# chahuja/mix-stage

Hardware: AMD Instinct MI355X
Metric: train-step clips/sec (B=32, T=64, M=8) (higher is better)
Workload: dtype f32; 1 GPU; Mix-StAGE GAN train step (reference D/G coin flip, seed 4321: 457 G + 510 D steps), B=32 clips per GPU, T=64, 128-mel, 104-dim pose, M=S=8, audio branch pinned; fp32 arithmetic (the reference trains in fp64, trainer.py:138; held to it at 1e-4 pose L1); global_batch=32, parallelism=dp1, hip_graphs=True, bn_sync=local

## Files before the change

include/mixstage.h:

```cpp
#ifndef MIXSTAGE_H_
#define MIXSTAGE_H_

#include <stddef.h>
#include <stdint.h>

#ifdef __cplusplus
extern "C" {
#endif

#define MS_ABI_VERSION 4

enum ms_block_mode {
  MS_BARE = 0,
  MS_LRELU = 1,
  MS_BN_TRAIN = 2,
  MS_BN_EVAL = 3
};

enum ms_input_mode {
  MS_IN_PLAIN = 0,
  MS_IN_BCAST = 1,
  MS_IN_UP2ADD = 2
};

enum ms_dtype { MS_F32 = 0, MS_BF16 = 1, MS_F16 = 2 };
#define MS_DT_OUT_F32 0x100
#define MS_DT_BN_FOLDED 0x200
#define MS_DT_STAT_PAIR 0x400

typedef struct ms_conv_desc {
  int32_t B;
  int32_t Cin;
  int32_t H, W;
  int32_t Cout;
  int32_t groups;
  int32_t KH, KW, SH, SW, PH, PW;
  int32_t OH, OW;
  int32_t mode;
  int32_t in_mode;
  float slope;
  float eps;
  float momentum;
  int32_t dtype;
} ms_conv_desc;

const char* ms_last_error(void);
int ms_abi_version(void);
int ms_stat_pair_ok(const ms_conv_desc* d);

size_t ms_conv_block_fwd_workspace(const ms_conv_desc* d);
size_t ms_conv_block_bwd_workspace(const ms_conv_desc* d);

int ms_conv_block_fwd(const ms_conv_desc* d, const float* x, const float* x2, const float* w,
                      const float* bias, const float* gamma, const float* beta, float* running_mean,
                      float* running_var, float* y_raw, float* y, float* save, void* workspace,
                      size_t workspace_bytes, void* stream);

typedef struct ms_fwd_options {
  const void* w_planes;
  int32_t* bn_sync;
  int32_t bn_sync_words;
} ms_fwd_options;
int ms_conv_block_fwd_ex(const ms_conv_desc* d, const float* x, const float* x2, const float* w,
                         const float* bias, const float* gamma, const float* beta, float* running_mean,
                         float* running_var, float* y_raw, float* y, float* save, void* workspace,
                         size_t workspace_bytes, void* stream, const ms_fwd_options* opt);
int ms_clip_hold(void* stream);
int ms_clip_hold_flush(void* stream);
int ms_clip_hold_discard(void* stream);
int ms_clip_grid(const ms_conv_desc* d);
int ms_clip_pair_ok(const ms_conv_desc* host, const ms_conv_desc* guest);
size_t ms_fwd_weights_bytes(const ms_conv_desc* d);
int ms_fwd_weights_prepare(int n, const ms_conv_desc* descs, const float* const* w, void* const* planes, void* stream);

int ms_conv_block_bwd(const ms_conv_desc* d, const float* x, const float* x2, const float* w,
                      const float* gamma, const float* running_mean, const float* running_var,
                      const float* y_raw, const float* y, const float* save, const float* dy, float* dyr,
                      float* dx, float* dx2, float* dw, float* dbias, float* dgamma, float* dbeta,
                      void* workspace, size_t workspace_bytes, void* stream);

typedef struct ms_bwd_options {
  void* side_stream;
  void* side_workspace;
  size_t side_workspace_bytes;
  const float* wt_prepared;
  float* wgrad_partials;
  int defer_wgrad_launch;
  const float* prev_y;
  const float* prev_y_raw;
  const float* prev_save;
  const float* prev_gamma;
  float* prev_dgamma;
  float* prev_dbeta;
  float* prev_dbias;
  float prev_slope;
  int32_t* bn_sync;
  int32_t bn_sync_words;
  int dy_is_dyr;
  const float* dx_accum;
} ms_bwd_options;
int ms_dgrad_takes_accum(const ms_conv_desc* d);
int ms_dgrad_fuses_prev_bn(const ms_conv_desc* d);
int ms_conv_block_bwd_ex(const ms_conv_desc* d, const float* x, const float* x2, const float* w,
                         const float* gamma, const float* running_mean, const float* running_var,
                         const float* y_raw, const float* y, const float* save, const float* dy, float* dyr,
                         float* dx, float* dx2, float* dw, float* dbias, float* dgamma, float* dbeta,
                         void* workspace, size_t workspace_bytes, void* stream, const ms_bwd_options* opt);

typedef struct ms_prep16_item {
  const ms_conv_desc* desc;
  const float* w;
  const float* bias;
  const float* gamma;
  const float* beta;
  const float* running_mean;
  const float* running_var;
  void* fwd;
  void* dgrad;
} ms_prep16_item;
size_t ms_weights16_bytes(const ms_conv_desc* d, int which);
int ms_weights16_prepare(int n, const ms_prep16_item* items, void* stream);

int ms_set_bn_sync_buffer(int32_t* zeroed_words, int n);

int ms_cb8_from_plain(int dtype, const float* x, void* y, int B, int C, int HW, void* stream);
int ms_cb8_to_plain(int dtype, const void* x, float* y, int B, int C, int HW, void* stream);
int ms_cb8_from_btc(int dtype, const float* x, void* y, int B, int T, int C, int velocity, void* stream);
int ms_cb8_to_btc(int dtype, const void* x, float* y, int B, int T, int C, int velocity_bwd, void* stream);

size_t ms_dgrad_weights_elems(const ms_conv_desc* d, const float* w);
int ms_set_precision(int mode);
int ms_get_precision(void);
int ms_tuning_epoch(void);
int ms_dgrad_weights_prepare(int n, const ms_conv_desc* descs, const float* const* w, float* const* wt, void* stream);

size_t ms_wgrad_partials_elems(const ms_conv_desc* d, int* splits);
int ms_set_wgrad_batched(int on, int tiles_per_workgroup);
int ms_wgrad_flush(void* stream);
int ms_wgrad_discard(void);
int ms_wgrad_reduce_multi(int n, const float* const* partials, float* const* dw, const int* elems, const int* splits,
                          void* stream);

int ms_bn_stats(const float* y_raw, float* stats, int B, int C, int HW, void* stream);
int ms_bn_train_apply(const float* stats_all, int world, int n_local, const float* gamma, const float* beta, float* running_mean,
                      float* running_var, const float* y_raw, float* y, float* save, int B, int C, int HW, float eps,
                      float momentum, float slope, void* stream);
size_t ms_bn_bwd_workspace(int B, int C);
int ms_bn_bwd_sums(const float* dy, const float* y_raw, const float* save, float* sums, int B, int C, int HW, float slope,
                   void* workspace, size_t workspace_bytes, void* stream);
int ms_bn_bwd_apply(const float* dy, const float* y_raw, const float* save, const float* gamma, const float* sums_global,
                    double n_global, float* dyr, int B, int C, int HW, float slope, void* stream);

int ms_lerp_time_fwd(const float* x, float* y, int B, int C, int Tin, int F, int Tout, void* stream);
int ms_lerp_time_bwd(const float* dy, float* dx, int B, int C, int Tin, int F, int Tout, void* stream);

int ms_softmax_mix_fwd(const float* z, const float* score, float* soft, float* out, int B, int M, int P,
                       int T, void* stream);
int ms_softmax_mix_bwd(const float* z, const float* soft, const float* dout, float* dz, float* dscore,
                       int B, int M, int P, int T, void* stream);

#define MS_CHAIN_MAX_BLOCKS 4
typedef struct ms_chain_desc {
  int32_t B, M, T, cin0, C, P, n_blocks;
  int32_t mode;
  int32_t dtype;
  int32_t sync_first_word;
  int32_t keep_all_raw;
  float slope, eps, momentum;
} ms_chain_desc;
typedef struct ms_chain_tensors {
  const void* x;
  const float* score;
  const float* w[MS_CHAIN_MAX_BLOCKS];
  const float* bias[MS_CHAIN_MAX_BLOCKS];
  const float* gamma[MS_CHAIN_MAX_BLOCKS];
  const float* beta[MS_CHAIN_MAX_BLOCKS];
  float* running_mean[MS_CHAIN_MAX_BLOCKS];
  float* running_var[MS_CHAIN_MAX_BLOCKS];
  void* y_raw[MS_CHAIN_MAX_BLOCKS];
  void* y[MS_CHAIN_MAX_BLOCKS];
  float* save[MS_CHAIN_MAX_BLOCKS];
  const float* w_logits;
  const float* bias_logits;
  float* z;
  float* soft;
  float* out;
  const void* prepared;
  int32_t* sync;
  int32_t sync_words;
} ms_chain_tensors;
int ms_decoder_chain_supported(const ms_chain_desc* d);
size_t ms_decoder_chain_prepared_bytes(const ms_chain_desc* d);
size_t ms_decoder_chain_workspace(const ms_chain_desc* d);
int ms_decoder_chain_sync_words(const ms_chain_desc* d);
int ms_decoder_chain_prepare(const ms_chain_desc* d, const float* const* w, const float* w_logits, void* prepared, void* stream);
int ms_decoder_chain_fwd(const ms_chain_desc* d, const ms_chain_tensors* t, void* workspace, size_t workspace_bytes, void* stream);

int ms_decoder_chain_eval_supported(const ms_chain_desc* d);
size_t ms_decoder_chain_eval_workspace(const ms_chain_desc* d);
int ms_decoder_chain_eval_sync_words(const ms_chain_desc* d);
int ms_decoder_chain_eval_plan(const ms_chain_desc* d, int32_t* n_tiles, int32_t* groups_per_workgroup, int32_t* tile_first,
                               int32_t* own_lo, int32_t* own_hi, int32_t cap);
int ms_decoder_chain_eval_fwd(const ms_chain_desc* d, const ms_chain_tensors* t, void* workspace, size_t workspace_bytes, void* stream);

int ms_kmeans_labels(const float* pose, const int32_t* keep, const double* centers, int64_t* labels, int B, int T, int P,
                     int PK, int M, int feats, void* stream);
int ms_znorm_select(const float* x, const int32_t* keep, const double* mean, const double* inv_std, float* y, size_t rows,
                    int P, int PK, void* stream);

int ms_step_metrics(const float* ycap, const float* gt, const int32_t* keep, const int32_t* slot_of, const double* mean,
                    const double* stdv, const float* alphas, int n_alpha, double* out, int B, int T, int P, int PK,
                    void* stream);
int ms_eval_accumulate(const float* ycap, const float* gt, const int32_t* keep, const double* mean, const double* stdv,
                       double* fid_sums, double* fid_gram, unsigned long long* w1_hist, int B, int T, int P, int PK,
                       double bin_width, int nbins, void* stream);

int ms_concat_style_fwd(const float* x, const float* emb, const int64_t* ids, int ids_stride_b, int ids_stride_t, float* out,
                        int B, int C, int D, int T, void* stream);
int ms_concat_style_bwd(const float* dout, const int64_t* ids, int ids_stride_b, int ids_stride_t, float* dx, float* demb,
                        int B, int C, int D, int T, int S, void* stream);

int ms_concat_style_soft_fwd(const float* x, const float* emb, const float* w, int w_stride_b, int w_stride_t, float* out,
                             int B, int C, int D, int T, int S, void* stream);
int ms_concat_style_soft_bwd(const float* dout, const float* emb, const float* w, int w_stride_b, int w_stride_t, float* dx,
                             float* demb, float* dw, int B, int C, int D, int T, int S, void* stream);

int ms_cross_entropy_fwd(const float* score, const int64_t* target, float* loss, float* row_scratch,
                         int n_outer, int n_inner, int C, int stride_outer, int stride_c,
                         int stride_inner, void* stream);
int ms_cross_entropy_bwd(const float* score, const int64_t* target, const float* gscale, float* dscore,
                         int n_outer, int n_inner, int C, int stride_outer, int stride_c,
                         int stride_inner, int accumulate, void* stream);

typedef struct ms_loss_scale {
  float scale;
  const float* scale_dev;
} ms_loss_scale;
int ms_cross_entropy_fwd_ex(const float* score, const int64_t* target, float* loss, int n_outer, int n_inner, int C,
                            int stride_outer, int stride_c, int stride_inner, void* stream, const ms_loss_scale* ls);
int ms_cross_entropy_bwd_ex(const float* score, const int64_t* target, const float* gscale, float* dscore, int n_outer,
                            int n_inner, int C, int stride_outer, int stride_c, int stride_inner, int accumulate, void* stream,
                            const ms_loss_scale* ls);

int ms_velocity_fwd(const float* x, float* v, int B, int T, int P, void* stream);
int ms_velocity_bwd(const float* dv, float* dx, int B, int T, int P, void* stream);

int ms_transpose_btc(const float* x, float* y, int B, int T, int C, void* stream);
int ms_transpose_bct(const float* x, float* y, int B, int C, int T, void* stream);

int ms_l1_mean_fwd(const float* a, const float* b, float target, float* loss, float* partials, size_t n,
                   void* stream);
int ms_l1_mean_bwd(const float* a, const float* b, float target, const float* gscale, float* da, size_t n,
                   void* stream);
int ms_l2_mean_fwd(const float* a, const float* b, float target, float* loss, float* partials, size_t n, void* stream);
int ms_l2_mean_bwd(const float* a, const float* b, float target, const float* gscale, float* da, size_t n, void* stream);

int ms_lp_mean_fwd_ex(int squared, const float* a, const float* b, float target, float* loss, float* partials, size_t n,
                      void* stream, const ms_loss_scale* ls);
int ms_lp_mean_bwd_ex(int squared, const float* a, const float* b, float target, const float* gscale, float* da, size_t n,
                      void* stream, const ms_loss_scale* ls);

int ms_lp_mean_pair_fwd(int squared, const float* a, const float* targets, float* loss, size_t n, void* stream, const ms_loss_scale* ls);
int ms_lp_mean_pair_bwd(int squared, const float* a, const float* targets, const float* gscale0, const float* gscale1, float* da, size_t n,
                        void* stream, const ms_loss_scale* ls);

int ms_copy_multi(int n, const void* const* src, void* const* dst, const size_t* bytes, void* stream);

int ms_write_floats(float* dst, const float* host_values, int n, void* stream);

int ms_sqnorm(const float* g, size_t n, float* norm_out, float* partials, void* stream);
int ms_adam_step(float* p, const float* g, float* m, float* v, size_t n, const float* norm, float max_norm,
                 float lr, float beta1, float beta2, float eps, int32_t* step_state, void* stream);
int ms_adam_step_segmented(float* p, const float* g, float* m, float* v, size_t n, const float* norm, float max_norm,
                           float lr, float beta1, float beta2, float eps, int32_t* step_state,
                           const int32_t* seg_of_chunk, const int32_t* seg_first_step, float* seg_scratch, int n_seg,
                           void* stream);
int ms_adam_step_segmented_scaled(float* p, const float* g, float* m, float* v, size_t n, float* norm, float max_norm,
                                  float lr, float beta1, float beta2, float eps, int32_t* step_state,
                                  const int32_t* seg_of_chunk, const int32_t* seg_first_step, float* seg_scratch, int n_seg,
                                  int32_t* loss_scale_state, int32_t growth_interval, float min_scale, float max_scale,
                                  const int32_t* const* meeting_words, int n_meeting_words, void* stream);
int ms_adam_step_segmented_lr(float* p, const float* g, float* m, float* v, size_t n, const float* norm, float max_norm,
                              const float* lr_dev, float beta1, float beta2, float eps, int32_t* step_state,
                              const int32_t* seg_of_chunk, const int32_t* seg_first_step, float* seg_scratch, int n_seg,
                              void* stream);
int ms_adam_step_segmented_scaled_lr(float* p, const float* g, float* m, float* v, size_t n, float* norm, float max_norm,
                                     const float* lr_dev, float beta1, float beta2, float eps, int32_t* step_state,
                                     const int32_t* seg_of_chunk, const int32_t* seg_first_step, float* seg_scratch, int n_seg,
                                     int32_t* loss_scale_state, int32_t growth_interval, float min_scale, float max_scale,
                                     const int32_t* const* meeting_words, int n_meeting_words, void* stream);
size_t ms_reduce_partials_count(size_t n);

#ifdef __cplusplus
}
#endif
#endif
```

include/mixstage_aux.h:

```cpp
#ifndef MIXSTAGE_AUX_H_
#define MIXSTAGE_AUX_H_

#include "mixstage.h"

#ifdef __cplusplus
extern "C" {
#endif

int ms_set_counter_buffer(int32_t* zeroed_counters, int n);

int ms_conv_block_bwd_overlap(const ms_conv_desc* d, const float* x, const float* x2, const float* w,
                              const float* gamma, const float* running_mean, const float* running_var,
                              const float* y_raw, const float* y, const float* save, const float* dy, float* dyr,
                              float* dx, float* dx2, float* dw, float* dbias, float* dgamma, float* dbeta,
                              void* workspace, size_t workspace_bytes, void* stream, void* side_stream,
                              void* side_workspace, size_t side_workspace_bytes);

int ms_timing_enable(int on);
size_t ms_timing_report(char* buf, size_t cap);

int ms_debug_set_patch_min_workgroups(int n);
int ms_debug_set_patch_tuning(int intra_split, int force_splitk);

int ms_debug_set_conv16_tile(int wm, int wn);
int ms_debug_set_conv16_ring(int nstg, int wide8);
int ms_debug_set_wgrad16_target(int workgroups);
int ms_debug_set_wgrad16_ring(int buffers);
int ms_debug_set_wgrad_target(int workgroups);
int ms_debug_set_wgrad_wave(int on);
int ms_debug_set_conv_tile(int on);
int ms_debug_set_bn_fused(int on);
int ms_debug_set_bn_fused_min_workgroups(int n);
int ms_debug_set_skip(const char* patterns);

int ms_debug_set_clip32(int on);

int ms_debug_set_clip_corun(int on);

int ms_selftest_mfma(const float* A, const float* B, float* C, int K, void* stream);
int ms_probe_peak(int kind, long iters, void* a, void* b, double* work, void* stream);

#ifdef __cplusplus
}
#endif
#endif
```

mix_stage_amd/_lib.py:

```python
import ctypes
import os

_HERE = os.path.dirname(os.path.abspath(__file__))
LIB_PATH = os.path.join(_HERE, 'libmixstage_hip.so')
_ALT_LIB = os.environ.get('MS_LIB_PATH')
if _ALT_LIB:
  LIB_PATH = _ALT_LIB

c_void_p, c_int, c_float, c_size_t = ctypes.c_void_p, ctypes.c_int, ctypes.c_float, ctypes.c_size_t


class BwdOptions(ctypes.Structure):
  _fields_ = [('side_stream', ctypes.c_void_p), ('side_workspace', ctypes.c_void_p), ('side_workspace_bytes', ctypes.c_size_t),
              ('wt_prepared', ctypes.c_void_p), ('wgrad_partials', ctypes.c_void_p), ('defer_wgrad_launch', ctypes.c_int),
              ('prev_y', ctypes.c_void_p), ('prev_y_raw', ctypes.c_void_p), ('prev_save', ctypes.c_void_p), ('prev_gamma', ctypes.c_void_p),
              ('prev_dgamma', ctypes.c_void_p), ('prev_dbeta', ctypes.c_void_p), ('prev_dbias', ctypes.c_void_p), ('prev_slope', ctypes.c_float),
              ('bn_sync', ctypes.c_void_p), ('bn_sync_words', ctypes.c_int32), ('dy_is_dyr', ctypes.c_int),
              ('dx_accum', ctypes.c_void_p)]


class LossScale(ctypes.Structure):
  _fields_ = [('scale', ctypes.c_float), ('scale_dev', ctypes.c_void_p)]


class FwdOptions(ctypes.Structure):
  _fields_ = [('w_planes', ctypes.c_void_p), ('bn_sync', ctypes.c_void_p), ('bn_sync_words', ctypes.c_int32)]


class ConvDesc(ctypes.Structure):
  _fields_ = [(n, ctypes.c_int32) for n in
              ('B', 'Cin', 'H', 'W', 'Cout', 'groups', 'KH', 'KW', 'SH', 'SW', 'PH', 'PW', 'OH', 'OW',
               'mode', 'in_mode')] + \
             [('slope', c_float), ('eps', c_float), ('momentum', c_float), ('dtype', ctypes.c_int32)]


class ChainDesc(ctypes.Structure):
  _fields_ = [(n, ctypes.c_int32) for n in ('B', 'M', 'T', 'cin0', 'C', 'P', 'n_blocks', 'mode', 'dtype', 'sync_first_word', 'keep_all_raw')] + \
             [('slope', c_float), ('eps', c_float), ('momentum', c_float)]


class ChainTensors(ctypes.Structure):
  _fields_ = [('x', ctypes.c_void_p), ('score', ctypes.c_void_p)] + \
             [(n, ctypes.c_void_p * 4) for n in ('w', 'bias', 'gamma', 'beta', 'running_mean', 'running_var', 'y_raw', 'y', 'save')] + \
             [(n, ctypes.c_void_p) for n in ('w_logits', 'bias_logits', 'z', 'soft', 'out', 'prepared', 'sync')] + \
             [('sync_words', ctypes.c_int32)]


class Prep16Item(ctypes.Structure):
  _fields_ = [('desc', ctypes.POINTER(ConvDesc))] + [(n, ctypes.c_void_p) for n in
             ('w', 'bias', 'gamma', 'beta', 'running_mean', 'running_var', 'fwd', 'dgrad')]


MS_BARE, MS_LRELU, MS_BN_TRAIN, MS_BN_EVAL = 0, 1, 2, 3
MS_IN_PLAIN, MS_IN_BCAST, MS_IN_UP2ADD = 0, 1, 2
MS_F32, MS_BF16, MS_F16, MS_DT_OUT_F32, MS_DT_BN_FOLDED = 0, 1, 2, 0x100, 0x200
MS_DT_STAT_PAIR = 0x400

_P = c_void_p
_DESC = ctypes.POINTER(ConvDesc)

SIGNATURES = {
    'ms_last_error': (ctypes.c_char_p, []),
    'ms_abi_version': (c_int, []),
    'ms_set_counter_buffer': (c_int, [_P, c_int]),
    'ms_set_bn_sync_buffer': (c_int, [_P, c_int]),
    'ms_debug_set_bn_fused': (c_int, [c_int]),
    'ms_debug_set_bn_fused_min_workgroups': (c_int, [c_int]),
    'ms_conv_block_fwd_workspace': (c_size_t, [_DESC]),
    'ms_conv_block_bwd_workspace': (c_size_t, [_DESC]),
    'ms_conv_block_fwd': (c_int, [_DESC] + [_P] * 11 + [_P, c_size_t, _P]),
    'ms_conv_block_bwd': (c_int, [_DESC] + [_P] * 17 + [_P, c_size_t, _P]),
    'ms_conv_block_bwd_overlap': (c_int, [_DESC] + [_P] * 17 + [_P, c_size_t, _P, _P, _P, c_size_t]),
    'ms_conv_block_bwd_ex': (c_int, [_DESC] + [_P] * 17 + [_P, c_size_t, _P, _P]),
    'ms_dgrad_weights_elems': (c_size_t, [_DESC, _P]),
    'ms_dgrad_weights_prepare': (c_int, [c_int, _P, _P, _P, _P]),
    'ms_tuning_epoch': (c_int, []),
    'ms_conv_block_fwd_ex': (c_int, [_DESC] + [_P] * 11 + [_P, c_size_t, _P, _P]),
    'ms_fwd_weights_bytes': (c_size_t, [_DESC]),
    'ms_fwd_weights_prepare': (c_int, [c_int, _P, _P, _P, _P]),
    'ms_set_precision': (c_int, [c_int]),
    'ms_get_precision': (c_int, []),
    'ms_wgrad_partials_elems': (c_size_t, [_DESC, _P]),
    'ms_wgrad_reduce_multi': (c_int, [c_int, _P, _P, _P, _P, _P]),
    'ms_wgrad_flush': (c_int, [_P]),
    'ms_wgrad_discard': (c_int, []),
    'ms_weights16_bytes': (c_size_t, [_DESC, c_int]),
    'ms_weights16_prepare': (c_int, [c_int, _P, _P]),
    'ms_cb8_from_plain': (c_int, [c_int, _P, _P, c_int, c_int, c_int, _P]),
    'ms_cb8_to_plain': (c_int, [c_int, _P, _P, c_int, c_int, c_int, _P]),
    'ms_cb8_from_btc': (c_int, [c_int, _P, _P, c_int, c_int, c_int, c_int, _P]),
    'ms_cb8_to_btc': (c_int, [c_int, _P, _P, c_int, c_int, c_int, c_int, _P]),
    'ms_bn_stats': (c_int, [_P, _P, c_int, c_int, c_int, _P]),
    'ms_bn_train_apply': (c_int, [_P, c_int, c_int, _P, _P, _P, _P, _P, _P, _P, c_int, c_int, c_int, c_float, c_float, c_float, _P]),
    'ms_bn_bwd_workspace': (c_size_t, [c_int, c_int]),
    'ms_bn_bwd_sums': (c_int, [_P, _P, _P, _P, c_int, c_int, c_int, c_float, _P, c_size_t, _P]),
    'ms_bn_bwd_apply': (c_int, [_P, _P, _P, _P, _P, ctypes.c_double, _P, c_int, c_int, c_int, c_float, _P]),
    'ms_lerp_time_fwd': (c_int, [_P, _P, c_int, c_int, c_int, c_int, c_int, _P]),
    'ms_lerp_time_bwd': (c_int, [_P, _P, c_int, c_int, c_int, c_int, c_int, _P]),
    'ms_softmax_mix_fwd': (c_int, [_P, _P, _P, _P, c_int, c_int, c_int, c_int, _P]),
    'ms_softmax_mix_bwd': (c_int, [_P, _P, _P, _P, _P, c_int, c_int, c_int, c_int, _P]),
    'ms_kmeans_labels': (c_int, [_P, _P, _P, _P, c_int, c_int, c_int, c_int, c_int, c_int, _P]),
    'ms_znorm_select': (c_int, [_P, _P, _P, _P, _P, c_size_t, c_int, c_int, _P]),
    'ms_step_metrics': (c_int, [_P] * 7 + [c_int, _P, c_int, c_int, c_int, c_int, _P]),
    'ms_eval_accumulate': (c_int, [_P] * 8 + [c_int, c_int, c_int, c_int, ctypes.c_double, c_int, _P]),
    'ms_concat_style_fwd': (c_int, [_P, _P, _P, c_int, c_int, _P, c_int, c_int, c_int, c_int, _P]),
    'ms_concat_style_bwd': (c_int, [_P, _P, c_int, c_int, _P, _P, c_int, c_int, c_int, c_int, c_int, _P]),
    'ms_concat_style_soft_fwd': (c_int, [_P, _P, _P, c_int, c_int, _P, c_int, c_int, c_int, c_int, c_int, _P]),
    'ms_concat_style_soft_bwd': (c_int, [_P, _P, _P, c_int, c_int, _P, _P, _P, c_int, c_int, c_int, c_int, c_int, _P]),
    'ms_cross_entropy_fwd': (c_int, [_P, _P, _P, _P] + [c_int] * 6 + [_P]),
    'ms_cross_entropy_bwd': (c_int, [_P, _P, _P, _P] + [c_int] * 7 + [_P]),
    'ms_cross_entropy_fwd_ex': (c_int, [_P, _P, _P] + [c_int] * 6 + [_P, _P]),
    'ms_cross_entropy_bwd_ex': (c_int, [_P, _P, _P, _P] + [c_int] * 7 + [_P, _P]),
    'ms_lp_mean_fwd_ex': (c_int, [c_int, _P, _P, c_float, _P, _P, c_size_t, _P, _P]),
    'ms_lp_mean_bwd_ex': (c_int, [c_int, _P, _P, c_float, _P, _P, c_size_t, _P, _P]),
    'ms_lp_mean_pair_fwd': (c_int, [c_int, _P, _P, _P, c_size_t, _P, _P]),
    'ms_lp_mean_pair_bwd': (c_int, [c_int, _P, _P, _P, _P, _P, c_size_t, _P, _P]),
    'ms_velocity_fwd': (c_int, [_P, _P, c_int, c_int, c_int, _P]),
    'ms_velocity_bwd': (c_int, [_P, _P, c_int, c_int, c_int, _P]),
    'ms_transpose_btc': (c_int, [_P, _P, c_int, c_int, c_int, _P]),
    'ms_transpose_bct': (c_int, [_P, _P, c_int, c_int, c_int, _P]),
    'ms_l1_mean_fwd': (c_int, [_P, _P, c_float, _P, _P, c_size_t, _P]),
    'ms_l1_mean_bwd': (c_int, [_P, _P, c_float, _P, _P, c_size_t, _P]),
    'ms_l2_mean_fwd': (c_int, [_P, _P, c_float, _P, _P, c_size_t, _P]),
    'ms_l2_mean_bwd': (c_int, [_P, _P, c_float, _P, _P, c_size_t, _P]),
    'ms_copy_multi': (c_int, [c_int, _P, _P, _P, _P]),
    'ms_write_floats': (c_int, [_P, _P, c_int, _P]),
    'ms_decoder_chain_supported': (c_int, [_P]),
    'ms_decoder_chain_prepared_bytes': (c_size_t, [_P]),
    'ms_decoder_chain_workspace': (c_size_t, [_P]),
    'ms_decoder_chain_sync_words': (c_int, [_P]),
    'ms_decoder_chain_prepare': (c_int, [_P, _P, _P, _P, _P]),
    'ms_decoder_chain_fwd': (c_int, [_P, _P, _P, c_size_t, _P]),
    'ms_decoder_chain_eval_supported': (c_int, [_P]),
    'ms_decoder_chain_eval_workspace': (c_size_t, [_P]),
    'ms_decoder_chain_eval_sync_words': (c_int, [_P]),
    'ms_decoder_chain_eval_plan': (c_int, [_P, _P, _P, _P, _P, _P, c_int]),
    'ms_decoder_chain_eval_fwd': (c_int, [_P, _P, _P, c_size_t, _P]),
    'ms_sqnorm': (c_int, [_P, c_size_t, _P, _P, _P]),
    'ms_adam_step': (c_int, [_P, _P, _P, _P, c_size_t, _P, c_float, c_float, c_float, c_float, c_float, _P, _P]),
    'ms_adam_step_segmented': (c_int, [_P, _P, _P, _P, c_size_t, _P, c_float, c_float, c_float, c_float, c_float, _P, _P, _P, _P,
                                       c_int, _P]),
    'ms_adam_step_segmented_scaled': (c_int, [_P, _P, _P, _P, c_size_t, _P, c_float, c_float, c_float, c_float, c_float, _P, _P, _P, _P,
                                              c_int, _P, ctypes.c_int32, c_float, c_float, _P, c_int, _P]),
    'ms_adam_step_segmented_lr': (c_int, [_P, _P, _P, _P, c_size_t, _P, c_float, _P, c_float, c_float, c_float, _P, _P, _P, _P,
                                          c_int, _P]),
    'ms_adam_step_segmented_scaled_lr': (c_int, [_P, _P, _P, _P, c_size_t, _P, c_float, _P, c_float, c_float, c_float, _P, _P, _P, _P,
                                                 c_int, _P, ctypes.c_int32, c_float, c_float, _P, c_int, _P]),
    'ms_reduce_partials_count': (c_size_t, [c_size_t]),
    'ms_timing_enable': (c_int, [c_int]),
    'ms_timing_report': (c_size_t, [ctypes.c_char_p, c_size_t]),
    'ms_debug_set_patch_min_workgroups': (c_int, [c_int]),
    'ms_debug_set_patch_tuning': (c_int, [c_int, c_int]),
    'ms_debug_set_conv16_tile': (c_int, [c_int, c_int]),
    'ms_debug_set_conv16_ring': (c_int, [c_int, c_int]),
    'ms_debug_set_skip': (c_int, [ctypes.c_char_p]),
    'ms_debug_set_clip32': (c_int, [c_int]),
    'ms_debug_set_clip_corun': (c_int, [c_int]),
    'ms_clip_hold': (c_int, [_P]),
    'ms_clip_hold_flush': (c_int, [_P]),
    'ms_clip_hold_discard': (c_int, [_P]),
    'ms_clip_grid': (c_int, [_DESC]),
    'ms_clip_pair_ok': (c_int, [_DESC, _DESC]),
    'ms_debug_set_wgrad16_target': (c_int, [c_int]),
    'ms_debug_set_wgrad16_ring': (c_int, [c_int]),
    'ms_debug_set_wgrad_target': (c_int, [c_int]),
    'ms_debug_set_wgrad_wave': (c_int, [c_int]),
    'ms_debug_set_conv_tile': (c_int, [c_int]),
    'ms_set_wgrad_batched': (c_int, [c_int, c_int]),
    'ms_dgrad_fuses_prev_bn': (c_int, [_P]),
    'ms_dgrad_takes_accum': (c_int, [_P]),
    'ms_stat_pair_ok': (c_int, [_P]),
    'ms_selftest_mfma': (c_int, [_P, _P, _P, c_int, _P]),
    'ms_probe_peak': (c_int, [c_int, ctypes.c_long, _P, _P, ctypes.POINTER(ctypes.c_double), _P]),
}

_lib = None


class MixStageLibError(RuntimeError):
  pass


def lib():
  global _lib
  if _lib is None:
    if not os.path.isfile(LIB_PATH):
      raise MixStageLibError('%s not built: run `make -C mix_stage_amd/csrc` (or __graft_entry__.build()); '
                             'there is no CPU fallback' % LIB_PATH)
    handle = ctypes.CDLL(LIB_PATH)
    for name, (res, args) in SIGNATURES.items():
      if _ALT_LIB and name.startswith('ms_debug_') and not hasattr(handle, name):
        continue
      fn = getattr(handle, name)
      fn.restype, fn.argtypes = res, args
    mode = os.environ.get('MS_PRECISION', '')
    if mode:
      if mode not in ('fp32', 'bf16x6'):
        raise MixStageLibError('MS_PRECISION=%s: expected fp32 or bf16x6' % mode)
      handle.ms_set_precision(1 if mode == 'bf16x6' else 0)
    if os.environ.get('MS_BN_FUSED'):
      handle.ms_debug_set_bn_fused(int(os.environ['MS_BN_FUSED']))
    if os.environ.get('MS_BN_FUSED_MIN_WGS'):
      handle.ms_debug_set_bn_fused_min_workgroups(int(os.environ['MS_BN_FUSED_MIN_WGS']))
    if os.environ.get('MS_CLIP32'):
      handle.ms_debug_set_clip32(int(os.environ['MS_CLIP32']))
    if os.environ.get('MS_CONV_TILE'):
      handle.ms_debug_set_conv_tile(int(os.environ['MS_CONV_TILE']))
    if os.environ.get('MS_WGRAD_WAVE'):
      handle.ms_debug_set_wgrad_wave(int(os.environ['MS_WGRAD_WAVE']))
    if os.environ.get('MS_PATCH_MIN_WGS'):
      handle.ms_debug_set_patch_min_workgroups(int(os.environ['MS_PATCH_MIN_WGS']))
    _lib = handle
  return _lib


def check(rc, what):
  if rc != 0:
    raise MixStageLibError('%s failed: %s' % (what, lib().ms_last_error().decode()))
```

mix_stage_amd/csrc/api.hip:

```cpp
#include "block_geom.h"

namespace ms {
extern int g_clip32;

static int validate(const ms_conv_desc* d, const char* who) {
  if (!d) return set_error("%s: null descriptor", who);
  if (d->B < 1 || d->Cin < 1 || d->Cout < 1 || d->groups < 1 || d->H < 1 || d->W < 1 || d->KH < 1 || d->KW < 1 ||
      d->SH < 1 || d->SW < 1 || d->PH < 0 || d->PW < 0)
    return set_error("%s: bad geometry", who);
  const int oh = (d->H + 2 * d->PH - d->KH) / d->SH + 1, ow = (d->W + 2 * d->PW - d->KW) / d->SW + 1;
  if (d->H + 2 * d->PH < d->KH || d->W + 2 * d->PW < d->KW || oh != d->OH || ow != d->OW)
    return set_error("%s: output size (%d,%d) does not match geometry (expected %d,%d)", who, d->OH, d->OW, oh, ow);
  if (d->mode < MS_BARE || d->mode > MS_BN_EVAL) return set_error("%s: bad mode %d", who, d->mode);
  if (d->in_mode < MS_IN_PLAIN || d->in_mode > MS_IN_UP2ADD) return set_error("%s: bad in_mode %d", who, d->in_mode);
  if (d->in_mode == MS_IN_UP2ADD && (d->H != 1 || d->KH != 1 || (d->W & 1)))
    return set_error("%s: UP2ADD needs a 1-D block with even W", who);
  if (dt_of(d) > DT_F16 || (d->dtype & ~(0xff | MS_DT_OUT_F32 | MS_DT_BN_FOLDED | MS_DT_STAT_PAIR))) return set_error("%s: bad dtype 0x%x", who, d->dtype);
  if (dt_of(d) == DT_F32 && (d->dtype & ~(0xff | MS_DT_STAT_PAIR))) return set_error("%s: MS_DT_OUT_F32 is a flag of the 16-bit modes", who);
  if ((d->dtype & MS_DT_STAT_PAIR) && (d->B & 1)) return set_error("%s: MS_DT_STAT_PAIR needs an even batch", who);
  const double out_elems = (double)d->B * d->groups * d->Cout * d->OH * d->OW;
  const double in_elems = (double)d->B * d->groups * d->Cin * d->H * d->W;
  const double lim = dt_of(d) == DT_F32 ? 536870912.0 : 1073741824.0;
  if (out_elems >= lim || in_elems >= lim) return set_error("%s: tensor of 2 GiB or more (%.0f elements)", who, std::max(out_elems, in_elems));
  return 0;
}

static inline bool conv_c1_of(const ms_conv_desc* d) {
  return conv_c1_ok(d->groups, d->Cin, d->Cout, d->KH, d->KW, d->SH, d->SW, d->PH, d->PW, d->H, d->in_mode == MS_IN_PLAIN);
}
static inline bool wgrad_c1_of(const ms_conv_desc* d) {
  return dt_of(d) == DT_F32 && g_precision == 0 &&
         wgrad_c1_ok(d->groups, d->Cin, d->Cout, d->KH, d->KW, d->SH, d->SW, d->PH, d->PW, d->H, d->W, d->in_mode == MS_IN_PLAIN);
}

struct FwdPlan {
  BlockGeo g;
  bool clip, c1;
  int c1_tiles;
  PatchPlan pp;
  GatherPlan pl;
  bool pair_epilogue;
  size_t w_bytes;
  struct { size_t stats, part, counts, clip_w, planes, total; } ws;
};
static FwdPlan fwd_plan(const ms_conv_desc* d) {
  FwdPlan p;
  const BlockGeo g = p.g = geo_of(d);
  const bool train = d->mode == MS_BN_TRAIN;
  p.clip = g_precision == 0 && clip32_fwd_ok(d);
  p.c1 = conv_c1_of(d);
  p.c1_tiles = p.c1 ? conv_c1_tiles(d->B, d->H, d->W) : 0;
  p.pp = plan_patch(g.nd, d->Cout, d->groups, d->Cin, d->KH, d->KW, d->SH, d->SW, d->B, d->OH, d->OW, 1, d->W);
  p.pl = plan_gather(d->Cout, g.npix, d->groups, d->Cin * g.khw);
  const PatchPlan& pp = p.pp;
  const bool patch_slab = pp.ok && (pp.splitk > 1 || pp.ksi > 1);
  p.pair_epilogue = !train || ((long)d->B / 2 * g.hw <= 4096 && !p.c1 && (pp.ok ? patch_slab : p.pl.splitk > 1));
  const size_t planes_bytes = (pp.ok && pp.p6) ? (size_t)3 * g.C * patch6_row_elems(d->Cin, d->KH, d->KW) * 2 : 0;
  p.w_bytes = p.clip ? clip32_fwd_weight_bytes(d) : planes_bytes;

  const size_t slab = (size_t)g.npix * g.C * sizeof(float);
  auto tile_stats = [&](int n_tiles) { return align_up((size_t)n_tiles * g.C * 2 * sizeof(float), 256); };
  p.ws.stats = p.ws.part = 0;
  p.ws.counts = p.c1 ? tile_stats(p.c1_tiles) : pp.ok ? tile_stats(pp.n_tiles) : 0;
  size_t front = 256;
  if (train) front = std::max(front, (size_t)p.pl.n_tiles * g.C * 2 * sizeof(float));
  if (pp.ok && train) front = std::max(front, tile_stats(pp.n_tiles) + (size_t)pp.n_tiles * sizeof(float));
  if (patch_slab) front = std::max(front, pp.splitk * slab);
  if (p.pl.splitk > 1) front = std::max(front, p.pl.splitk * slab);
  if (p.c1) front = std::max(front, tile_stats(p.c1_tiles) + (size_t)p.c1_tiles * sizeof(float));
  p.ws.total = align_up(front, 256) + 256;
  p.ws.planes = carve(p.ws.total, align_up(planes_bytes, 256));
  p.ws.clip_w = p.clip ? clip32_part_bytes(d->Cout, d->B * d->OW / 32) : 0;
  if (p.clip) p.ws.total = std::max(p.ws.total, p.ws.clip_w + align_up(p.w_bytes, 256) + 256);
  return p;
}

struct BwdPlan {
  BlockGeo g;
  DgradGeo dg;
  int nchunk;
  bool dg_clip, dg_grouped;
  PatchPlan dpp;
  GatherPlan dpl;
  size_t wt_elems;
  size_t dg_planes_bytes;
  bool wg_c1;
  WgradPatchPlan wp;
  int wg_splits;
  int wg_splits_reserved;
  struct { size_t fuse_part, bn_part, colpart, wt, wg_part, dg_part, dg_planes, total; } ws;
};
static BwdPlan bwd_plan(const ms_conv_desc* d) {
  BwdPlan p;
  const BlockGeo g = p.g = geo_of(d);
  const DgradGeo dg = p.dg = dgrad_geo_of(d);
  int bpc;
  p.nchunk = bwd_chunks(d->B, g.C, &bpc);
  p.dg_clip = g_precision == 0 && clip32_dgrad_ok(d);
  p.dg_grouped = g_precision == 0 && g_clip32 && gdgrad32_ok(d);
  p.dpp = plan_patch(g.nd, d->Cin, dg.tg, dg.tcog, dg.jh, dg.jw, 1, 1, d->B, cdiv(d->H, d->SH), cdiv(d->W, d->SW), dg.ncls, d->OW);
  p.dpl = plan_gather(d->Cin, d->B * cdiv(d->H, d->SH) * cdiv(d->W, d->SW), dg.tg * dg.ncls, dg.tcog * dg.jh * dg.jw);
  p.wt_elems = dgrad_weight_elems(d->groups, d->Cout, d->Cin, d->KH, d->KW, d->SH, d->SW);
  p.dg_planes_bytes = (p.dpp.ok && p.dpp.p6) ? (size_t)3 * dg.ncls * dg.tg * d->Cin * patch6_row_elems(dg.tcog, dg.jh, dg.jw) * 2 : 0;
  p.wg_c1 = wgrad_c1_of(d);
  p.wp = WgradPatchPlan{};
  if (p.wg_c1) {
    p.wg_splits = p.wg_splits_reserved = wgrad_c1_splits(d->B, d->H);
  } else {
    p.wp = plan_wgrad_patch(g.nd, d->Cout, d->Cin * g.khw, d->groups, d->KH, d->KW, d->SH, d->SW, d->B, d->OH, d->OW, d->W, g.up2 != 0);
    const int gather_splits = wgrad_splits(d->Cout, d->Cin * g.khw, d->groups, g.npix);
    p.wg_splits = p.wp.ok ? p.wp.splits : gather_splits;
    p.wg_splits_reserved = std::max(p.wp.ok ? p.wp.splits : 1, gather_splits);
  }

  const size_t dx_bytes = (size_t)d->B * g.cin_tot * d->H * d->W * sizeof(float);
  p.ws.total = 0;
  p.ws.fuse_part = carve(p.ws.total, clip32_dgrad_bn_part_bytes(d));
  p.ws.bn_part = carve(p.ws.total, align_up((size_t)g.C * p.nchunk * 2 * sizeof(float), 256));
  p.ws.colpart = carve(p.ws.total, align_up((size_t)g.C * p.nchunk * sizeof(float), 256));
  p.ws.wt = carve(p.ws.total, align_up(std::max(p.wt_elems, std::max(clip32_dgrad_weight_floats(d), gdgrad32_weight_floats(d))) * sizeof(float), 256));
  p.ws.wg_part = carve(p.ws.total, align_up(wsize_of(d) * sizeof(float) * (p.wg_splits_reserved > 1 ? p.wg_splits_reserved : 0), 256));
  p.ws.dg_part = carve(p.ws.total, (p.dpp.ok && p.dpp.splitk > 1) ? align_up(p.dpp.splitk * dx_bytes, 256) : 0);
  p.ws.dg_planes = carve(p.ws.total, align_up(p.dg_planes_bytes, 256));
  if (p.dpl.splitk > 1) p.ws.total += align_up(p.dpl.splitk * dx_bytes, 256);
  p.ws.total += 256;
  return p;
}

enum { DW_NONE = 0, DW_TRANSPOSED = 1, DW_CLIP = 2, DW_GROUPED = 3 };
static int dgrad_weights_of(const ms_conv_desc* d, const BwdPlan& p, const float* w) {
  if (p.dg_clip) return DW_CLIP;
  if (p.dg_grouped) return DW_GROUPED;
  const bool direct = p.dpp.ok && !p.dpp.p6 && patch_dgrad_direct_ok(w, d->Cin, d->KH, d->KW, d->SH, d->SW, p.g.bcast != 0);
  return direct ? DW_NONE : DW_TRANSPOSED;
}
static size_t dgrad_weights_elems(const ms_conv_desc* d, const BwdPlan& p, int kind) {
  return kind == DW_CLIP ? clip32_dgrad_weight_floats(d) : kind == DW_GROUPED ? gdgrad32_weight_floats(d) : p.wt_elems;
}

}

using namespace ms;

extern "C" {

size_t ms_conv_block_fwd_workspace(const ms_conv_desc* d) {
  if (!d) return 256;
  return dt_of(d) != DT_F32 ? block_fwd16_workspace(d) : fwd_plan(d).ws.total;
}

size_t ms_conv_block_bwd_workspace(const ms_conv_desc* d) {
  if (!d) return 256;
  return dt_of(d) != DT_F32 ? block_bwd16_workspace(d) : bwd_plan(d).ws.total;
}

int ms_conv_block_fwd(const ms_conv_desc* d, const float* x, const float* x2, const float* w, const float* bias,
                      const float* gamma, const float* beta, float* running_mean, float* running_var, float* y_raw, float* y,
                      float* save, void* workspace, size_t workspace_bytes, void* stream) {
  return ms_conv_block_fwd_ex(d, x, x2, w, bias, gamma, beta, running_mean, running_var, y_raw, y, save, workspace,
                              workspace_bytes, stream, nullptr);
}

static int conv_block_fwd_impl(const ms_conv_desc* d, const float* x, const float* x2, const float* w, const float* bias,
                               const float* gamma, const float* beta, float* running_mean, float* running_var, float* y_raw,
                               float* y, float* save, void* workspace, size_t workspace_bytes, void* stream,
                               const ms_fwd_options* opt);

int ms_conv_block_fwd_ex(const ms_conv_desc* d, const float* x, const float* x2, const float* w, const float* bias,
                         const float* gamma, const float* beta, float* running_mean, float* running_var, float* y_raw,
                         float* y, float* save, void* workspace, size_t workspace_bytes, void* stream,
                         const ms_fwd_options* opt) {
  const bool clip_path = d && dt_of(d) == DT_F32 && g_precision == 0 && !validate(d, "ms_conv_block_fwd") && clip32_fwd_ok(d);
  int rc = clip32_fwd_call_begin((hipStream_t)stream, clip_path, workspace, workspace_bytes);
  if (!rc) rc = conv_block_fwd_impl(d, x, x2, w, bias, gamma, beta, running_mean, running_var, y_raw, y, save, workspace, workspace_bytes, stream, opt);
  clip32_fwd_call_end((hipStream_t)stream);
  return rc;
}

static int conv_block_fwd_impl(const ms_conv_desc* d, const float* x, const float* x2, const float* w, const float* bias,
                               const float* gamma, const float* beta, float* running_mean, float* running_var, float* y_raw,
                               float* y, float* save, void* workspace, size_t workspace_bytes, void* stream,
                               const ms_fwd_options* opt) {
  const unsigned short* w_planes = opt ? (const unsigned short*)opt->w_planes : nullptr;
  int rc = validate(d, "ms_conv_block_fwd");
  if (rc) return rc;
  if (!x || !w || !y) return set_error("ms_conv_block_fwd: null tensor");
  const bool bn = d->mode == MS_BN_TRAIN || d->mode == MS_BN_EVAL;
  if (bn && (!gamma || !beta || !running_mean || !running_var)) return set_error("ms_conv_block_fwd: BN tensors missing");
  if (d->mode == MS_BN_TRAIN && (!y_raw || !save || !workspace)) return set_error("ms_conv_block_fwd: y_raw/save/workspace missing");
  if (d->in_mode == MS_IN_UP2ADD && !x2) return set_error("ms_conv_block_fwd: UP2ADD needs x2");
  if (dt_of(d) != DT_F32)
    return block_fwd16(d, x, x2, w, bias, gamma, beta, running_mean, running_var, y_raw, y, save, workspace, workspace_bytes,
                       (hipStream_t)stream, w_planes, opt ? opt->bn_sync : nullptr, opt ? opt->bn_sync_words : 0);
  const FwdPlan p = fwd_plan(d);
  if (workspace_bytes < p.ws.total) return set_error("ms_conv_block_fwd: workspace too small");
  hipStream_t s = (hipStream_t)stream;
  const BlockGeo& g = p.g;
  const int C = g.C, npix = g.npix, hw = g.hw, Kg = d->Cin * g.khw;
  float* stats = ws_at<float>(workspace, p.ws.stats);
  float* counts = ws_at<float>(workspace, p.ws.counts);
  float* part = ws_at<float>(workspace, p.ws.part);

  if (p.clip) {
    const float* wp = (const float*)w_planes;
    if (!wp) {
      float* mine = ws_at<float>(workspace, p.ws.clip_w);
      rc = clip32_prep_queue(w, mine, d->Cout, d->Cin, d->KW, 0, d->Cin, s);
      if (!rc) rc = clip32_prep_flush(s);
      if (rc) return rc;
      wp = mine;
    }
    rc = clip32_block_fwd(d, x, x2, wp, bias, gamma, beta, running_mean, running_var, y_raw, y, save, stats, opt ? opt->bn_sync : nullptr,
                          opt ? opt->bn_sync_words : 0, s);
    if (rc != -2) return rc;
    rc = clip32_hold_flush(s);
    if (rc) return rc;
  }

  float* out = d->mode == MS_BN_TRAIN ? y_raw : y;
  const int a_vec = (Kg % 4 == 0) && (((uintptr_t)w & 15) == 0);
  const int ep = d->mode == MS_BARE ? EP_BARE : d->mode == MS_LRELU ? EP_LRELU : d->mode == MS_BN_EVAL ? EP_BN_EVAL : EP_RAW_STATS;
  const int sg = d->mode == MS_BN_TRAIN ? sg_of(d) : 1;
  if (sg > 1 && !p.pair_epilogue)
    return set_error("ms_conv_block_fwd: MS_DT_STAT_PAIR is not implemented for this block's kernels (ms_stat_pair_ok)");
  if (p.c1) {
    rc = launch_conv_c1(x, w, bias, out, gamma, beta, running_mean, running_var, stats, counts, d->B, d->H, d->W, ep, d->slope,
                        d->eps, s);
    if (rc) return rc;
    if (d->mode == MS_BN_TRAIN) {
      rc = launch_bn_finalize_apply(stats, counts, p.c1_tiles, 0, npix, C, gamma, beta, running_mean, running_var, save, d->eps,
                                    d->momentum, y_raw, y, d->B, hw, d->slope, s);
    }
    return rc;
  }
  if (p.pp.ok) {
    const PatchPlan& pp = p.pp;
    PatchArgs q = {};
    q.A = w; q.src = x; q.src2 = x2; q.out = out;
    q.bias = bias; q.bn_g = gamma; q.bn_b = beta; q.bn_m = running_mean; q.bn_v = running_var;
    q.stats = stats; q.counts = counts;
    q.Mg = d->Cout; q.Kg = Kg; q.groups = d->groups; q.Kc = d->Cin; q.bcast = g.bcast; q.a_vec = a_vec; q.ep = ep;
    fill_src(q, plane_strides(g.one_d, d->B, g.cin_tot, d->H, d->W));
    fill_out(q, plane_strides(g.one_d, d->B, C, d->OH, d->OW));
    q.PH = g.one_d ? 0 : d->PH;
    q.PW = d->PW; q.tiles_x = pp.tiles_x; q.tiles_y = pp.tiles_y; q.slope = d->slope; q.eps = d->eps;
    q.o_sh = 1; q.o_sw = 1; q.o_ry = 0; q.o_rx = 0;
    q.splitk = pp.splitk; q.chunks_per_split = pp.chunks_per_split;
    q.src_elems = (size_t)d->B * g.cin_tot * d->H * d->W; q.a_elems = (size_t)C * Kg;
    const bool raw_out = pp.splitk > 1 || (pp.ksi > 1 && d->mode == MS_BN_TRAIN);
    if (raw_out) { q.part = part; q.part_stride = (size_t)npix * C; }
    const double flops = 2.0 * d->Cout * Kg * (double)npix * d->groups;
    const double bytes = 4.0 * ((double)C * Kg + (double)d->B * g.cin_tot * d->H * d->W + (double)npix * C);
    if (pp.p6) {
      const int re = patch6_row_elems(d->Cin, d->KH, d->KW);
      const unsigned short* planes = w_planes;
      if (!planes) {
        unsigned short* mine = ws_at<unsigned short>(workspace, p.ws.planes);
        rc = launch_split_weights(w, mine, C, d->Cin, d->KH, d->KW, s);
        if (rc) return rc;
        planes = mine;
      }
      q.Aplanes = planes; q.plane_stride = (unsigned)((size_t)C * re); q.a_row_elems = re;
      rc = launch_patch6(q, pp, d->KH, d->KW, d->SW, g.up2 != 0, flops, bytes, s);
    } else {
      rc = launch_patch(q, pp, d->KH, d->KW, d->SW, g.up2 != 0, flops, bytes, s);
    }
    if (rc) return rc;
    if (raw_out)
      return launch_splitk_fwd_epilogue(q.part, pp.splitk, q.part_stride, bias, gamma, beta, running_mean, running_var, y_raw,
                                        y, save, d->B, C, hw, ep, d->slope, d->eps, d->momentum, s, sg);
    if (d->mode == MS_BN_TRAIN) {
      rc = launch_bn_finalize_apply(stats, counts, pp.n_tiles, 0, npix, C, gamma, beta, running_mean, running_var, save, d->eps,
                                    d->momentum, y_raw, y, d->B, hw, d->slope, s);
    }
    return rc;
  }
  const GatherPlan& pl = p.pl;
  GatherArgs a = {};
  a.A = w; a.src = x; a.src2 = x2; a.out = out;
  a.bias = bias; a.bn_g = gamma; a.bn_b = beta; a.bn_m = running_mean; a.bn_v = running_var;
  a.stats = stats;
  a.Mg = d->Cout; a.Kg = Kg; a.groups = d->groups; a.Kc = d->Cin;
  a.bcast = g.bcast; a.src_ctotal = g.cin_tot;
  a.SRCH = d->H; a.SRCW = d->W; a.OUTH = d->OH; a.OUTW = d->OW; a.Npix = npix;
  a.KH = d->KH; a.KW = d->KW; a.SH = d->SH; a.SW = d->SW; a.PH = d->PH; a.PW = d->PW;
  a.a_vec = a_vec; a.ep = ep;
  a.slope = d->slope; a.eps = d->eps;
  if (pl.splitk > 1) {
    a.part = part;
    a.part_stride = (size_t)npix * C;
  }
  rc = launch_gather(a, false, g.up2 != 0, pl, s);
  if (rc) return rc;
  if (pl.splitk > 1) {
    return launch_splitk_fwd_epilogue(a.part, pl.splitk, a.part_stride, bias, gamma, beta, running_mean, running_var, y_raw, y,
                                      save, d->B, C, hw, ep, d->slope, d->eps, d->momentum, s, sg);
  }
  if (d->mode == MS_BN_TRAIN) {
    rc = launch_bn_finalize_apply(stats, nullptr, pl.n_tiles, 64 * pl.tn, npix, C, gamma, beta, running_mean, running_var, save,
                                  d->eps, d->momentum, y_raw, y, d->B, hw, d->slope, s);
  }
  return rc;
}

size_t ms_wgrad_partials_elems(const ms_conv_desc* d, int* splits) {
  if (validate(d, "ms_wgrad_partials_elems")) return 0;
  const int sp = dt_of(d) != DT_F32 ? wgrad16_splits(d) : bwd_plan(d).wg_splits;
  if (splits) *splits = sp;
  return sp > 1 ? (size_t)sp * wsize_of(d) : 0;
}

int ms_wgrad_reduce_multi(int n, const float* const* partials, float* const* dw, const int* elems, const int* splits,
                          void* stream) {
  if (n < 0 || (n && (!partials || !dw || !elems || !splits))) return set_error("ms_wgrad_reduce_multi: null argument");
  for (int i = 0; i < n; ++i)
    if (!partials[i] || !dw[i] || elems[i] <= 0 || splits[i] < 1) return set_error("ms_wgrad_reduce_multi: bad job %d", i);
  ReduceBatch rb;
  rb.n = 0;
  for (int i = 0; i < n; ++i) {
    ReduceJob jb = {partials[i], dw[i], elems[i], splits[i], 0, 0};
    rb.job[rb.n++] = jb;
    if (rb.n == REDUCE_BATCH_MAX) {
      const int rc = launch_reduce_splits_multi(rb, (hipStream_t)stream);
      if (rc) return rc;
      rb.n = 0;
    }
  }
  return rb.n ? launch_reduce_splits_multi(rb, (hipStream_t)stream) : 0;
}

size_t ms_dgrad_weights_elems(const ms_conv_desc* d, const float* w) {
  if (validate(d, "ms_dgrad_weights_elems")) return 0;
  if (dt_of(d) != DT_F32) return 0;
  const BwdPlan p = bwd_plan(d);
  const int kind = dgrad_weights_of(d, p, w);
  if (kind == DW_NONE) return 0;
  return align_up(dgrad_weights_elems(d, p, kind), 64) + (p.dg_planes_bytes + 3) / 4;
}

size_t ms_fwd_weights_bytes(const ms_conv_desc* d) {
  if (validate(d, "ms_fwd_weights_bytes")) return 0;
  if (dt_of(d) != DT_F32) return 0;
  return fwd_plan(d).w_bytes;
}

int ms_fwd_weights_prepare(int n, const ms_conv_desc* descs, const float* const* w, void* const* planes, void* stream) {
  if (n < 0 || (n && (!descs || !w || !planes))) return set_error("ms_fwd_weights_prepare: null argument");
  PrepQueueGuard queue_guard;
  SplitBatch sb;
  sb.n = 0;
  for (int i = 0; i < n; ++i) {
    const ms_conv_desc* d = descs + i;
    int rc = validate(d, "ms_fwd_weights_prepare");
    if (rc) return rc;
    if (dt_of(d) != DT_F32) continue;
    const FwdPlan p = fwd_plan(d);
    if (!p.w_bytes) continue;
    if (!planes[i]) return set_error("ms_fwd_weights_prepare: block %d needs a buffer of ms_fwd_weights_bytes bytes", i);
    if (p.clip) {
      rc = clip32_prep_queue(w[i], (float*)planes[i], d->Cout, d->Cin, d->KW, 0, d->Cin, (hipStream_t)stream);
      if (rc) return rc;
      continue;
    }
    SplitJob jb = {w[i], (unsigned short*)planes[i], p.g.C, d->Cin, p.g.khw, 0, 0, 0};
    sb.job[sb.n++] = jb;
    if (sb.n == SPLIT_BATCH_MAX) {
      rc = launch_split_weights_multi(sb, (hipStream_t)stream);
      if (rc) return rc;
      sb.n = 0;
    }
  }
  { const int rcq = clip32_prep_flush((hipStream_t)stream); if (rcq) return rcq; }
  return sb.n ? launch_split_weights_multi(sb, (hipStream_t)stream) : 0;
}

int ms_dgrad_weights_prepare(int n, const ms_conv_desc* descs, const float* const* w, float* const* wt, void* stream) {
  if (n < 0 || (n && (!descs || !w || !wt))) return set_error("ms_dgrad_weights_prepare: null argument");
  PrepQueueGuard queue_guard;
  TransposeBatch tb;
  tb.n = 0;
  for (int i = 0; i < n; ++i) {
    const ms_conv_desc* d = descs + i;
    int rc = validate(d, "ms_dgrad_weights_prepare");
    if (rc) return rc;
    const BwdPlan p = bwd_plan(d);
    const int kind = dgrad_weights_of(d, p, w[i]);
    if (kind == DW_NONE) continue;
    if (!wt[i]) return set_error("ms_dgrad_weights_prepare: block %d needs a buffer of ms_dgrad_weights_elems floats", i);
    if (kind == DW_CLIP) {
      rc = clip32_prep_queue(w[i], wt[i], d->Cin, d->Cout, d->KW, d->KW == 4 ? 2 : 1, d->Cin, (hipStream_t)stream);
      if (rc) return rc;
      continue;
    }
    if (kind == DW_GROUPED) {
      rc = gdgrad32_prepare(d, w[i], wt[i], (hipStream_t)stream);
      if (rc) return rc;
      continue;
    }
    TransposeJob jb = {w[i], wt[i], p.dg.tg, p.dg.tcog, d->Cin, d->KH, d->KW, d->SH, d->SW, d->PH, d->PW, p.dpp.ok ? 1 : 0, 0};
    tb.job[tb.n++] = jb;
    if (tb.n == TRANSPOSE_BATCH_MAX) {
      rc = launch_transpose_weight_multi(tb, (hipStream_t)stream);
      if (rc) return rc;
      tb.n = 0;
    }
  }
  if (tb.n) {
    const int rc = launch_transpose_weight_multi(tb, (hipStream_t)stream);
    if (rc) return rc;
  }
  { int rcq = clip32_prep_flush((hipStream_t)stream); if (!rcq) rcq = gdgrad32_prep_flush((hipStream_t)stream); if (rcq) return rcq; }
  SplitBatch sb;
  sb.n = 0;
  for (int i = 0; i < n; ++i) {
    const ms_conv_desc* d = descs + i;
    const BwdPlan p = bwd_plan(d);
    if (!p.dg_planes_bytes || dgrad_weights_of(d, p, w[i]) != DW_TRANSPOSED) continue;
    SplitJob jb = {wt[i], (unsigned short*)(wt[i] + align_up(p.wt_elems, 64)), p.dg.ncls * p.dg.tg * d->Cin, p.dg.tcog, p.dg.jh * p.dg.jw, 0, 0, 0};
    sb.job[sb.n++] = jb;
    if (sb.n == SPLIT_BATCH_MAX) {
      const int rc = launch_split_weights_multi(sb, (hipStream_t)stream);
      if (rc) return rc;
      sb.n = 0;
    }
  }
  return sb.n ? launch_split_weights_multi(sb, (hipStream_t)stream) : 0;
}

int ms_stat_pair_ok(const ms_conv_desc* d) {
  if (!d || (d->B & 1) || validate(d, "ms_stat_pair_ok")) return 0;
  if (d->mode != MS_BN_TRAIN) return 1;
  if (dt_of(d) != DT_F32) return stat_pair16_ok(d) ? 1 : 0;
  if (g_precision != 0) return 0;
  if ((long)d->B / 2 * d->OH * d->OW > BN_BWD32_FUSED_MAX) return 0;
  const FwdPlan p = fwd_plan(d);
  if (p.clip) {
    const int npx = d->SW == 2 ? 32 : 64, npw = d->B * d->OW / npx, cus = current_device_cus();
    if (npw % 2 == 0 && cus > 0 && cdiv(d->Cout, 32) * npw <= cus) return 1;
  }
  return p.pair_epilogue ? 1 : 0;
}

int ms_dgrad_fuses_prev_bn(const ms_conv_desc* d) {
  if (!d || validate(d, "ms_dgrad_fuses_prev_bn") || (d->dtype & MS_DT_STAT_PAIR)) return 0;
  return (dt_of(d) == DT_F32 && g_precision == 0 && clip32_dgrad_bn_ok(d)) ? 1 : 0;
}

int ms_dgrad_takes_accum(const ms_conv_desc* d) {
  if (!d || validate(d, "ms_dgrad_takes_accum")) return 0;
  if (dt_of(d) != DT_F32) return dgrad16_takes_accum(d) ? 1 : 0;
  return (g_precision == 0 && d->in_mode == MS_IN_PLAIN && clip32_dgrad_ok(d)) ? 1 : 0;
}

int ms_conv_block_bwd(const ms_conv_desc* d, const float* x, const float* x2, const float* w, const float* gamma,
                      const float* running_mean, const float* running_var, const float* y_raw, const float* y,
                      const float* save, const float* dy, float* dyr, float* dx, float* dx2, float* dw, float* dbias,
                      float* dgamma, float* dbeta, void* workspace, size_t workspace_bytes, void* stream) {
  ms_bwd_options o = {};
  return ms_conv_block_bwd_ex(d, x, x2, w, gamma, running_mean, running_var, y_raw, y, save, dy, dyr, dx, dx2, dw, dbias,
                              dgamma, dbeta, workspace, workspace_bytes, stream, &o);
}

static hipEvent_t fork_event() {
  static thread_local hipEvent_t ev = nullptr;
  if (!ev && hipEventCreateWithFlags(&ev, hipEventDisableTiming) != hipSuccess) ev = nullptr;
  return ev;
}

int ms_conv_block_bwd_overlap(const ms_conv_desc* d, const float* x, const float* x2, const float* w, const float* gamma,
                              const float* running_mean, const float* running_var, const float* y_raw, const float* y,
                              const float* save, const float* dy, float* dyr, float* dx, float* dx2, float* dw,
                              float* dbias, float* dgamma, float* dbeta, void* workspace, size_t workspace_bytes,
                              void* stream, void* side_stream, void* side_workspace, size_t side_workspace_bytes) {
  ms_bwd_options o = {};
  o.side_stream = side_stream; o.side_workspace = side_workspace; o.side_workspace_bytes = side_workspace_bytes;
  return ms_conv_block_bwd_ex(d, x, x2, w, gamma, running_mean, running_var, y_raw, y, save, dy, dyr, dx, dx2, dw, dbias,
                              dgamma, dbeta, workspace, workspace_bytes, stream, &o);
}

int ms_conv_block_bwd_ex(const ms_conv_desc* d, const float* x, const float* x2, const float* w, const float* gamma,
                         const float* running_mean, const float* running_var, const float* y_raw, const float* y,
                         const float* save, const float* dy, float* dyr, float* dx, float* dx2, float* dw, float* dbias,
                         float* dgamma, float* dbeta, void* workspace, size_t workspace_bytes, void* stream,
                         const ms_bwd_options* opt) {
  (void)running_mean; (void)running_var;
  ms_bwd_options none = {};
  if (!opt) opt = &none;
  void* side_stream = opt->side_stream;
  const float* wt_prepared = opt->wt_prepared;
  const bool defer_wgrad = opt->wgrad_partials != nullptr;
  int rc = validate(d, "ms_conv_block_bwd");
  if (rc) return rc;
  if (d->mode == MS_BN_EVAL) return set_error("ms_conv_block_bwd: BN_EVAL blocks are never differentiated on the path");
  if (!dy || !w || !workspace) return set_error("ms_conv_block_bwd: null tensor");
  if (d->mode == MS_BN_TRAIN && !opt->dy_is_dyr && (!y_raw || !save || !gamma || !dyr)) return set_error("ms_conv_block_bwd: BN_TRAIN needs y_raw/save/gamma/dyr");
  if ((opt->dy_is_dyr || opt->prev_y) && (dt_of(d) != DT_F32 || side_stream)) return set_error("ms_conv_block_bwd: the fused producer-BatchNorm backward is an fp32, single-stream form");
  if (d->mode == MS_LRELU && (!y || !dyr)) return set_error("ms_conv_block_bwd: LRELU needs y/dyr");
  if (dw && !x) return set_error("ms_conv_block_bwd: dw needs x");
  if (opt->dx_accum && !(dx && ms_dgrad_takes_accum(d))) return set_error("ms_conv_block_bwd: dx_accum on a block ms_dgrad_takes_accum() declines");
  if (d->in_mode == MS_IN_UP2ADD && ((dw && !x2) || (dx && !dx2))) return set_error("ms_conv_block_bwd: UP2ADD needs x2/dx2");
  if (dt_of(d) != DT_F32) {
    if (side_stream) return set_error("ms_conv_block_bwd: no side-stream form in the 16-bit modes");
    if (d->mode == MS_BARE && out_f32_of(d) && !dyr) return set_error("ms_conv_block_bwd: fp32 dy needs the dyr scratch");
    return block_bwd16(d, x, x2, w, gamma, y_raw, y, save, dy, dyr, dx, dx2, dw, dbias, dgamma, dbeta, workspace, workspace_bytes,
                       (hipStream_t)stream, wt_prepared, opt->wgrad_partials, opt->defer_wgrad_launch, opt->dx_accum);
  }
  const BwdPlan p = bwd_plan(d);
  if (workspace_bytes < p.ws.total) return set_error("ms_conv_block_bwd: workspace too small");
  hipStream_t s = (hipStream_t)stream;
  const BlockGeo& g = p.g;
  const DgradGeo& dg = p.dg;
  const int C = g.C, npix = g.npix, hw = g.hw, Kg = d->Cin * g.khw;
  const bool up2 = g.up2 != 0, bcast = g.bcast != 0;

  float* fuse_part = ws_at<float>(workspace, p.ws.fuse_part);
  float* bn_part = ws_at<float>(workspace, p.ws.bn_part);
  float* colpart = ws_at<float>(workspace, p.ws.colpart);
  float* wt = ws_at<float>(workspace, p.ws.wt);
  float* wg_part = ws_at<float>(workspace, p.ws.wg_part);
  float* dg_part = ws_at<float>(workspace, p.ws.dg_part);
  if (defer_wgrad) wg_part = opt->wgrad_partials;
  hipStream_t ws_stream = s;
  if (side_stream && side_stream != stream && dw) {
    if (defer_wgrad) return set_error("ms_conv_block_bwd_ex: wgrad_partials and side_stream are exclusive");
    if (!opt->side_workspace || opt->side_workspace_bytes < p.ws.total)
      return set_error("ms_conv_block_bwd_overlap: side workspace too small");
    ws_stream = (hipStream_t)side_stream;
    wg_part = ws_at<float>(opt->side_workspace, p.ws.wg_part);
  }

  const float* gr = dy;
  int bias_done = 0;
  const bool have_prev = opt->prev_y != nullptr;
  if (have_prev && !(dx && g_precision == 0 && clip32_dgrad_bn_ok(d)))
    return set_error("ms_conv_block_bwd: this block's data gradient cannot carry the producer's BatchNorm backward (ms_dgrad_fuses_prev_bn)");
  if (opt->dy_is_dyr) {
    if (d->mode != MS_BN_TRAIN) return set_error("ms_conv_block_bwd: dy_is_dyr is the BN_TRAIN form");
    bias_done = 1;
  } else if (d->mode == MS_BN_TRAIN) {
    rc = launch_bn_bwd(dy, y_raw, y, save, gamma, bn_part, dyr, colpart, dbias, dgamma, dbeta, d->B, C, hw, d->slope, &bias_done, s, sg_of(d));
    gr = dyr;
  } else if (d->mode == MS_LRELU) {
    rc = launch_act_bwd(dy, y, dyr, colpart, dbias, d->B, C, hw, 1, d->slope, &bias_done, s);
    gr = dyr;
  } else if (dbias) {
    rc = launch_act_bwd(dy, nullptr, nullptr, colpart, dbias, d->B, C, hw, 0, 0.f, &bias_done, s);
  }
  if (rc) return rc;
  if (dbias && !bias_done && !opt->dy_is_dyr) {
    rc = launch_colsum_finalize(colpart, dbias, d->B, C, s);
    if (rc) return rc;
  }

  if (ws_stream != s) {
    hipEvent_t ev = fork_event();
    if (!ev || hipEventRecord(ev, s) != hipSuccess || hipStreamWaitEvent(ws_stream, ev, 0) != hipSuccess)
      return set_error("ms_conv_block_bwd_overlap: stream fork failed");
  }

  bool dx_done = false;
  if (dx && p.dg_clip) {
    const float* wp = wt_prepared;
    if (!wp) {
      rc = clip32_prep_queue(w, wt, d->Cin, d->Cout, d->KW, d->KW == 4 ? 2 : 1, d->Cin, s);
      if (!rc) rc = clip32_prep_flush(s);
      if (rc) return rc;
      wp = wt;
    }
    if (have_prev) {
      const Clip32PrevBN pv = {opt->prev_y, opt->prev_y_raw, opt->prev_save, opt->prev_gamma, opt->prev_dgamma, opt->prev_dbeta, opt->prev_dbias, opt->prev_slope};
      rc = clip32_block_dgrad(d, gr, wp, dx, dx2, s, &pv, fuse_part, opt->bn_sync, opt->bn_sync_words, opt->dx_accum);
      if (rc == -2) return set_error("ms_conv_block_bwd: the fused data gradient is not resident at once on this device");
    } else {
      rc = clip32_block_dgrad(d, gr, wp, dx, dx2, s, nullptr, nullptr, nullptr, 0, opt->dx_accum);
    }
    if (rc && rc != -2) return rc;
    if (rc == -2 && opt->dx_accum) return set_error("ms_conv_block_bwd: the clip-resident data gradient declined a launch with dx_accum");
    dx_done = rc == 0;
    rc = 0;
  }
  if (dx && !dx_done && p.dg_grouped) {
    const float* wp = wt_prepared;
    if (!wp) {
      rc = gdgrad32_prepare(d, w, wt, s);
      if (!rc) rc = gdgrad32_prep_flush(s);
      if (rc) return rc;
      wp = wt;
    }
    rc = gdgrad32_launch(d, gr, wp, dx, s);
    if (rc) return rc;
    dx_done = true;
  }
  if (dx && !dx_done) {
    const PatchPlan& pp0 = p.dpp;
    const int Kg2 = dg.tcog * dg.jh * dg.jw;
    const size_t dx_elems = (size_t)d->B * g.cin_tot * d->H * d->W;
    const bool direct = pp0.ok && !pp0.p6 && patch_dgrad_direct_ok(w, d->Cin, d->KH, d->KW, d->SH, d->SW, bcast);
    if (wt_prepared) {
      wt = const_cast<float*>(wt_prepared);
    } else if (!direct) {
      rc = launch_transpose_weight(w, wt, dg.tg, dg.tcog, d->Cin, d->KH, d->KW, d->SH, d->SW, d->PH, d->PW, pp0.ok ? 1 : 0, s);
      if (rc) return rc;
    }
    if (pp0.ok) {
      PatchArgs q = {};
      q.A = wt; q.src = gr; q.out = dx; q.out2 = dx2;
      q.Mg = d->Cin; q.Kg = Kg2; q.groups = dg.tg; q.Kc = dg.tcog; q.bcast = 0; q.a_vec = (Kg2 % 4 == 0);
      if (direct) { q.A = w; q.a_vec = 2; }
      q.ep = up2 ? EP_DGRAD_UP2 : EP_BARE; q.is_dgrad = 1;
      q.cls_a_stride = (unsigned)((size_t)dg.tg * d->Cin * Kg2);
      fill_src(q, plane_strides(g.one_d, d->B, C, d->OH, d->OW));
      fill_out(q, plane_strides(g.one_d, d->B, g.cin_tot, d->H, d->W));
      const double flops = fill_parity_classes(q, d, dg, g.one_d);
      const double bytes = 4.0 * ((double)dg.ncls * dg.tg * d->Cin * Kg2 + (double)d->B * C * hw) + 4.0 * (double)dx_elems;
      q.tiles_x = pp0.tiles_x; q.tiles_y = pp0.tiles_y;
      q.splitk = pp0.splitk; q.chunks_per_split = pp0.chunks_per_split;
      q.src_elems = (size_t)d->B * C * hw; q.a_elems = (size_t)dg.ncls * dg.tg * d->Cin * Kg2;
      if (pp0.splitk > 1) {
        q.part = dg_part; q.part_stride = dx_elems;
        q.ep = EP_BARE;
      }
      if (pp0.p6) {
        const int re = patch6_row_elems(dg.tcog, dg.jh, dg.jw), rows = dg.ncls * dg.tg * d->Cin;
        const unsigned short* planes;
        if (wt_prepared) {
          planes = (const unsigned short*)(wt_prepared + align_up(p.wt_elems, 64));
        } else {
          unsigned short* mine = ws_at<unsigned short>(workspace, p.ws.dg_planes);
          rc = launch_split_weights(wt, mine, rows, dg.tcog, dg.jh, dg.jw, s);
          if (rc) return rc;
          planes = mine;
        }
        q.Aplanes = planes; q.plane_stride = (unsigned)((size_t)rows * re); q.a_row_elems = re;
        q.cls_a_stride = (unsigned)(dg.tg * d->Cin);
        rc = launch_patch6(q, pp0, dg.jh, dg.jw, 1, false, flops, bytes, s);
      } else {
        rc = launch_patch(q, pp0, dg.jh, dg.jw, 1, false, flops, bytes, s);
      }
      if (rc) return rc;
      if (pp0.splitk > 1) {
        rc = launch_splitk_dgrad_epilogue(dg_part, pp0.splitk, dx_elems, dx, dx2, dx_elems, d->W, up2 ? 1 : 0, s);
        if (rc) return rc;
      }
    } else {
      const GatherPlan& pl = p.dpl;
      GatherArgs a = {};
      a.A = wt; a.src = gr; a.out = dx; a.out2 = dx2;
      a.Mg = d->Cin; a.Kg = Kg2; a.groups = dg.tg; a.Kc = dg.tcog; a.src_ctotal = C;
      a.SRCH = d->OH; a.SRCW = d->OW; a.OUTH = d->H; a.OUTW = d->W; a.Npix = d->B * d->H * d->W; a.batch = d->B;
      a.KH = dg.jh; a.KW = dg.jw; a.SH = d->SH; a.SW = d->SW; a.PH = d->PH; a.PW = d->PW;
      a.bcast = 0;
      a.a_vec = (a.Kg % 4 == 0);
      a.ep = up2 ? EP_DGRAD_UP2 : EP_DGRAD;
      if (pl.splitk > 1) {
        a.part = dg_part;
        a.part_stride = dx_elems;
        a.ep = EP_DGRAD;
      }
      rc = launch_gather(a, true, up2, pl, s);
      if (rc) return rc;
      if (pl.splitk > 1) {
        rc = launch_splitk_dgrad_epilogue(dg_part, pl.splitk, dx_elems, dx, dx2, dx_elems, d->W, up2 ? 1 : 0, s);
        if (rc) return rc;
      }
    }
  }

  if (dw && p.wg_c1) {
    rc = launch_wgrad_c1(gr, x, wg_part, d->B, d->H, d->W, ws_stream);
    if (!rc && !defer_wgrad) rc = launch_reduce_splits(wg_part, dw, C * Kg, p.wg_splits, ws_stream);
    return rc;
  }
  if (dw && p.wp.ok) {
    const WgradPatchPlan& wp = p.wp;
    WgradPatchArgs q = {};
    q.dyr = gr; q.src = x; q.src2 = x2;
    q.out = wp.splits > 1 ? wg_part : dw;
    q.Cog = d->Cout; q.Cig = d->Cin; q.Kg = Kg; q.groups = d->groups; q.bcast = bcast;
    fill_src(q, plane_strides(g.one_d, d->B, g.cin_tot, d->H, d->W));
    fill_out(q, plane_strides(g.one_d, d->B, C, d->OH, d->OW));
    q.PH = g.one_d ? 0 : d->PH;
    q.PW = d->PW; q.tiles_x = wp.tiles_x; q.tiles_y = wp.tiles_y; q.n_tiles = wp.n_tiles;
    q.tiles_per_split = wp.tiles_per_split; q.splits = wp.splits;
    const double flops = 2.0 * d->Cout * q.Kg * (double)npix * d->groups;
    const double bytes = 4.0 * ((double)npix * C + (double)d->B * g.cin_tot * d->H * d->W + (double)C * q.Kg);
    if (wp.splits > 1 && !defer_wgrad && !wp.p6) {
      q.counters = counter_region(CNT_WGRAD, cdiv(q.Kg, 64) * cdiv(d->Cout, 64) * d->groups);
      q.final_out = dw;
    }
    if (opt->defer_wgrad_launch && !wp.p6 && ws_stream == s && (wp.splits == 1 || defer_wgrad))
      return queue_wgrad_patch(q, wp, d->KH, d->KW, d->SW, up2, flops, bytes);
    rc = wp.p6 ? launch_wgrad_patch6(q, wp, d->KH, d->KW, d->SW, up2, flops, bytes, ws_stream)
               : launch_wgrad_patch(q, wp, d->KH, d->KW, d->SW, up2, flops, bytes, ws_stream);
    if (rc) return rc;
    if (wp.splits > 1 && !q.counters && !defer_wgrad) rc = launch_reduce_splits(wg_part, dw, C * q.Kg, wp.splits, ws_stream);
  } else if (dw) {
    WgradArgs a = {};
    a.dyr = gr; a.src = x; a.src2 = x2;
    a.Cog = d->Cout; a.Cig = d->Cin; a.Kg = Kg; a.groups = d->groups;
    a.src_ctotal = g.cin_tot;
    a.H = d->H; a.W = d->W; a.OH = d->OH; a.OW = d->OW; a.Npix = npix;
    a.KH = d->KH; a.KW = d->KW; a.SH = d->SH; a.SW = d->SW; a.PH = d->PH; a.PW = d->PW;
    a.bcast = bcast;
    rc = launch_wgrad(a, up2, dw, wg_part, defer_wgrad, ws_stream, opt->defer_wgrad_launch && ws_stream == s);
  }
  return rc;
}

int ms_clip_hold(void* stream) { return clip32_hold_arm((hipStream_t)stream); }
int ms_clip_hold_flush(void* stream) { return clip32_hold_flush((hipStream_t)stream); }
int ms_clip_hold_discard(void* stream) { clip32_hold_discard((hipStream_t)stream); return 0; }
int ms_clip_grid(const ms_conv_desc* d) {
  if (validate(d, "ms_clip_grid") || dt_of(d) != DT_F32 || g_precision != 0) return 0;
  return clip32_fwd_grid(d);
}
int ms_clip_pair_ok(const ms_conv_desc* host, const ms_conv_desc* guest) {
  if (validate(host, "ms_clip_pair_ok") || validate(guest, "ms_clip_pair_ok") || dt_of(host) != DT_F32 || dt_of(guest) != DT_F32 || g_precision != 0) return 0;
  return clip32_fwd_pair_ok(host, guest) ? 1 : 0;
}
int ms_debug_set_clip_corun(int on) {
  const int prev = g_clip_corun < 0 ? 1 : g_clip_corun;
  g_clip_corun = on ? 1 : 0;
  return prev;
}

}
```

mix_stage_amd/csrc/clip32.hip:

```cpp
#include <stdio.h>
#include <stdlib.h>

#include <algorithm>
#include <map>
#include <mutex>
#include <vector>

#include "kernels.h"
#include "conv16.h"

namespace ms {

typedef unsigned int cl_u32x4 __attribute__((ext_vector_type(4)));
typedef unsigned int cl_u32x2 __attribute__((ext_vector_type(2)));
constexpr int CL_SPIN_LIMIT = 1 << 21;
constexpr int CL_MAXK8W = 9;

struct Clip32Args {
  const float* x;
  const float* x2;
  const float* wp;
  const float* bias;
  const float* gamma;
  const float* beta;
// ... 260 lines not shown
            acc[nb] = __builtin_amdgcn_mfma_f32_32x32x2f32(cl_f4e(wr[u], j), cl_f4e(bf[u & 1][nb], j), acc[nb], 0, 0, 0);
        __builtin_amdgcn_sched_barrier(0);
      }
    } else {
#pragma unroll
      for (int i = 0; i < CL_MAXK8W; ++i) {
        if (i < k8w) {
#pragma unroll
          for (int tap = 0; tap < KW; ++tap) {
            if constexpr (DG2) {
              const float4 b1 = *reinterpret_cast<const float4*>(img + ((size_t)i * 2 * pslots + bbase[0] + ((4 - tap) >> 1)) * 4);
#pragma unroll
              for (int j = 0; j < 4; ++j)
                acc[(tap + 1) & 1] = __builtin_amdgcn_mfma_f32_32x32x2f32(cl_f4e(wr[i * KW + tap], j), cl_f4e(b1, j), acc[(tap + 1) & 1], 0, 0, 0);
              continue;
            }
            float4 bf[NB];
#pragma unroll
            for (int nb = 0; nb < NB; ++nb) bf[nb] = *reinterpret_cast<const float4*>(img + ((size_t)i * 2 * pslots + bbase[nb] + cl_pos<SPLIT>(tap, half)) * 4);
#pragma unroll
            for (int j = 0; j < 4; ++j)
#pragma unroll
              for (int nb = 0; nb < NB; ++nb)
                acc[nb] = __builtin_amdgcn_mfma_f32_32x32x2f32(cl_f4e(wr[i * KW + tap], j), cl_f4e(bf[nb], j), acc[nb], 0, 0, 0);
          }
        }
      }
    }
  }
  CL_STAMP(3);
  __syncthreads();
  CL_STAMP(4);

  constexpr int RP = NPX + 4;
  float* red = cl_smem;
#pragma unroll
  for (int nb = 0; nb < NB; ++nb)
#pragma unroll
    for (int q = 0; q < 16; ++q) red[(w * 32 + 8 * (q >> 2) + 4 * h + (q & 3)) * RP + (DG2 ? 2 * n0 + nb : 32 * nb + n0)] = acc[nb][q];
  __syncthreads();

  constexpr int FPT = NPX / 8;
  float v[FPT];
  {
    const float* rp = red + chl * RP + FPT * pq;
#pragma unroll
    for (int k = 0; k < FPT; k += 4) {
      float4 s = *reinterpret_cast<const float4*>(rp + k);
#pragma unroll
      for (int ww = 1; ww < 4; ++ww) {
        const float4 u = *reinterpret_cast<const float4*>(rp + ww * 32 * RP + k);
        s.x += u.x; s.y += u.y; s.z += u.z; s.w += u.w;
      }
      v[k] = s.x + bias_c; v[k + 1] = s.y + bias_c; v[k + 2] = s.z + bias_c; v[k + 3] = s.w + bias_c;
    }
    if constexpr (!UP2) {
#pragma unroll
      for (int k = 0; k < FPT; ++k) v[k] += av[k];
    }
  }
  const int f0 = FPT * pq;
  auto store_frames = [&](float* dst, const float (&val)[FPT]) {
    if (To >= FPT) {
      const int cl = f0 / To, tt = f0 - cl * To;
      float* d = dst + ((size_t)(b0 + cl) * p.Cout + cgl) * To + tt;
#pragma unroll
      for (int k = 0; k < FPT; k += 4) *reinterpret_cast<float4*>(d + k) = float4{val[k], val[k + 1], val[k + 2], val[k + 3]};
    } else {
#pragma unroll
      for (int k = 0; k < FPT; ++k) {
        const int f = f0 + k, cl = f / To, tt = f - cl * To;
        dst[((size_t)(b0 + cl) * p.Cout + cgl) * To + tt] = val[k];
      }
    }
  };

  float sc = 1.f, sh = 0.f;
  if (p.ep == EP_RAW_STATS) {
    float s = 0.f;
#pragma unroll
    for (int k = 0; k < FPT; ++k) s += v[k];
    const float mean_w = cl_sum8(s) * (1.0f / NPX);
    float q = 0.f;
#pragma unroll
    for (int k = 0; k < FPT; ++k) { const float d = v[k] - mean_w; q = fmaf(d, d, q); }
    const float m2_w = cl_sum8(q);
    double mean = (double)mean_w, m2 = (double)m2_w;
    const int npg = p.npw / p.sg, sgi = pw / npg, pw0 = sgi * npg;
    const double n = (double)npg * NPX;
    const __amdgpu_buffer_rsrc_t rsPart = buf_rsrc(p.part);
    auto group_stats = [&](int first, double& gmean, double& gm2) {
      float2 pv[4];
      const unsigned base = 8u * (unsigned)((ct * p.npw + first) * 32 + chl);
      double ms = 0.0, qs = 0.0, dv = 0.0;
      for (int i0 = pq; i0 < npg; i0 += 32) {
#pragma unroll
        for (int u = 0; u < 4; ++u) {
          const int i = min(i0 + 8 * u, npg - 1);
          pv[u] = __builtin_bit_cast(float2, __builtin_amdgcn_raw_buffer_load_b64(rsPart, (int)(base + 8u * (unsigned)(i * 32)), 0, 16));
        }
#pragma unroll
        for (int u = 0; u < 4; ++u)
          if (i0 + 8 * u < npg) { ms += (double)pv[u].x; qs += (double)pv[u].y; }
      }
      gmean = cl_sum8_d(ms) / (double)npg;
      for (int i0 = pq; i0 < npg; i0 += 32) {
#pragma unroll
        for (int u = 0; u < 4; ++u) {
          const int i = min(i0 + 8 * u, npg - 1);
          pv[u] = __builtin_bit_cast(float2, __builtin_amdgcn_raw_buffer_load_b64(rsPart, (int)(base + 8u * (unsigned)(i * 32)), 0, 16));
        }
#pragma unroll
        for (int u = 0; u < 4; ++u)
          if (i0 + 8 * u < npg) { const double dl = (double)pv[u].x - gmean; dv += dl * dl; }
      }
      gm2 = cl_sum8_d(qs) + (double)NPX * cl_sum8_d(dv);
    };
    bool expired = false;
    if (p.npw > 1) {
      if (pq == 0)
        __builtin_amdgcn_raw_buffer_store_b64(__builtin_bit_cast(cl_u32x2, float2{mean_w, m2_w}), rsPart,
                                              (int)(8u * (unsigned)((ct * p.npw + pw) * 32 + chl)), 0, 16);
      asm volatile("s_waitcnt vmcnt(0)" ::: "memory");
      __syncthreads();
      CL_STAMP(5);
      int* lflag = reinterpret_cast<int*>(cl_smem + 4 * 32 * RP);
      if (t == 0) {
        int* counter = p.sync + p.cnt_base + 32 * ct;
        const int prior = __hip_atomic_load(p.sync, __ATOMIC_RELAXED, __HIP_MEMORY_SCOPE_AGENT);
        const unsigned old = (unsigned)__hip_atomic_fetch_add(counter, 1, __ATOMIC_RELAXED, __HIP_MEMORY_SCOPE_AGENT);
        const unsigned target = (old / (unsigned)p.npw + 1u) * (unsigned)p.npw;
        int spins = 0, bad = 0;
        while ((int)((unsigned)__hip_atomic_load(counter, __ATOMIC_RELAXED, __HIP_MEMORY_SCOPE_AGENT) - target) < 0) {
          __builtin_amdgcn_s_sleep(2);
          if (++spins > CL_SPIN_LIMIT) { __hip_atomic_store(p.sync, 20, __ATOMIC_RELAXED, __HIP_MEMORY_SCOPE_AGENT); bad = 1; break; }
        }
        lflag[0] = bad | (prior != 0);
      }
      __syncthreads();
      CL_STAMP(6);
      group_stats(pw0, mean, m2);
      expired = lflag[0] != 0;
      if (expired) { mean = __builtin_nan(""); }
    }
    const float var = (float)(m2 / n), fmean = (float)mean;
    const float invstd = 1.0f / sqrtf(var + p.eps);
    sc = gam * invstd;
    sh = bet - fmean * sc;
    if (pw == pw0 && pq == 0 && rowok && fmean == fmean && p.save) {
      float* sv = p.save + (size_t)sgi * 4 * p.Cout;
      sv[cgl] = fmean; sv[p.Cout + cgl] = invstd; sv[2 * p.Cout + cgl] = sc; sv[3 * p.Cout + cgl] = sh;
    }
    if (pw == (p.sg - 1) * npg && !expired) {
      float rmc = rmo, rvc = rvo;
      for (int gi = 0; gi + 1 < p.sg; ++gi) {
        double gmean, gm2;
        group_stats(gi * npg, gmean, gm2);
        if (pq == 0 && rowok) {
          const float ub = n > 1.0 ? (float)(gm2 / (n - 1.0)) : (float)(gm2 / n);
          running_stats_update(&p.rm[cgl], &p.rv[cgl], rmc, rvc, p.momentum, (float)gmean, ub);
          rmc = p.rm[cgl]; rvc = p.rv[cgl];
        }
      }
      if (pq == 0 && rowok && fmean == fmean) {
        const float unbiased = n > 1.0 ? (float)(m2 / (n - 1.0)) : var;
        running_stats_update(&p.rm[cgl], &p.rv[cgl], rmc, rvc, p.momentum, fmean, unbiased);
      }
    }
    if (p.y_raw && rowok && (p.raw_all || bn_inv_unsafe(fmean, invstd, sc, sh, p.slope))) store_frames(p.y_raw, v);
  } else if (p.ep == EP_BN_EVAL) {
    sc = gam * (1.0f / sqrtf(rvo + p.eps));
    sh = bet - rmo * sc;
  } else if (p.ep == EP_DGRAD_BN) {
    const int C = p.Cout;
    const float mean = p.pv_save[cgc], invstd = p.pv_save[C + cgc], scp = p.pv_save[2 * C + cgc], shp = p.pv_save[3 * C + cgc];
    const float gm = p.pv_gamma[cgc];
    const bool from_y = !bn_inv_unsafe(mean, invstd, scp, shp, p.slope);
    const float* src = from_y ? p.pv_y : p.pv_y_raw;
    float yv[FPT];
    if (To >= FPT) {
      const int cl = f0 / To, tt = f0 - cl * To;
      const float* sp = src + ((size_t)(b0 + cl) * C + cgc) * To + tt;
#pragma unroll
      for (int k = 0; k < FPT; k += 4) {
        const float4 u = *reinterpret_cast<const float4*>(sp + k);
        yv[k] = u.x; yv[k + 1] = u.y; yv[k + 2] = u.z; yv[k + 3] = u.w;
      }
    } else {
#pragma unroll
      for (int k = 0; k < FPT; ++k) {
        const int f = f0 + k, cl = f / To, tt = f - cl * To;
        yv[k] = src[((size_t)(b0 + cl) * C + cgc) * To + tt];
      }
    }
    const float beta_c = fmaf(mean, scp, shp), inv_sl = 1.0f / p.slope, inv_g = invstd / scp;
    float dz[FPT], xh[FPT];
    float s1 = 0.f, s2 = 0.f, s3 = 0.f;
#pragma unroll
    for (int k = 0; k < FPT; ++k) {
      bool pos;
      float xv;
      if (from_y) {
        pos = yv[k] > 0.f;
        xv = ((pos ? yv[k] : yv[k] * inv_sl) - beta_c) * inv_g;
      } else {
        pos = fmaf(yv[k], scp, shp) > 0.f;
        xv = (yv[k] - mean) * invstd;
      }
      dz[k] = v[k] * (pos ? 1.f : p.slope);
      xh[k] = xv;
      s1 += dz[k];
      s2 = fmaf(dz[k], xv, s2);
      s3 += xv;
    }
    s1 = cl_sum8(s1); s2 = cl_sum8(s2); s3 = cl_sum8(s3);
    double S1 = (double)s1, S2 = (double)s2, S3 = (double)s3;
    if (p.npw > 1) {
      const __amdgpu_buffer_rsrc_t rsPart = buf_rsrc(p.part);
      if (pq == 0)
        __builtin_amdgcn_raw_buffer_store_b128(__builtin_bit_cast(cl_u32x4, float4{s1, s2, s3, 0.f}), rsPart,
                                               (int)(16u * (unsigned)((ct * p.npw + pw) * 32 + chl)), 0, 16);
      asm volatile("s_waitcnt vmcnt(0)" ::: "memory");
      __syncthreads();
      int* lflag = reinterpret_cast<int*>(cl_smem + 4 * 32 * RP);
      if (t == 0) {
        int* counter = p.sync + p.cnt_base + 32 * ct;
        const int prior = __hip_atomic_load(p.sync, __ATOMIC_RELAXED, __HIP_MEMORY_SCOPE_AGENT);
        const unsigned old = (unsigned)__hip_atomic_fetch_add(counter, 1, __ATOMIC_RELAXED, __HIP_MEMORY_SCOPE_AGENT);
        const unsigned target = (old / (unsigned)p.npw + 1u) * (unsigned)p.npw;
        int spins = 0, bad = 0;
        while ((int)((unsigned)__hip_atomic_load(counter, __ATOMIC_RELAXED, __HIP_MEMORY_SCOPE_AGENT) - target) < 0) {
          __builtin_amdgcn_s_sleep(2);
          if (++spins > CL_SPIN_LIMIT) { __hip_atomic_store(p.sync, 21, __ATOMIC_RELAXED, __HIP_MEMORY_SCOPE_AGENT); bad = 1; break; }
        }
        lflag[0] = bad | (prior != 0);
      }
      __syncthreads();
      const unsigned base = 16u * (unsigned)(ct * p.npw * 32 + chl);
      double a1 = 0.0, a2 = 0.0, a3 = 0.0;
      float4 pv4[4];
      for (int i0 = pq; i0 < p.npw; i0 += 32) {
#pragma unroll
        for (int u = 0; u < 4; ++u) {
          const int i = min(i0 + 8 * u, p.npw - 1);
          pv4[u] = __builtin_bit_cast(float4, __builtin_amdgcn_raw_buffer_load_b128(rsPart, (int)(base + 16u * (unsigned)(i * 32)), 0, 16));
        }
#pragma unroll
        for (int u = 0; u < 4; ++u)
          if (i0 + 8 * u < p.npw) { a1 += (double)pv4[u].x; a2 += (double)pv4[u].y; a3 += (double)pv4[u].z; }
      }
      S1 = cl_sum8_d(a1); S2 = cl_sum8_d(a2); S3 = cl_sum8_d(a3);
      if (lflag[0]) S1 = __builtin_nan("");
    }
    const double n = (double)p.npw * NPX;
    const float m1 = (float)(S1 / n), m2 = (float)(S2 / n), gi = gm * invstd;
#pragma unroll
    for (int k = 0; k < FPT; ++k) v[k] = gi * (dz[k] - m1 - xh[k] * m2);
    if (pw == 0 && pq == 0 && rowok) {
      if (p.pv_dgamma) { p.pv_dgamma[cgl] = (float)S2; p.pv_dbeta[cgl] = (float)S1; }
      if (p.pv_dbias) p.pv_dbias[cgl] = -gi * m2 * (float)S3;
    }
    if (rowok) store_frames(p.y, v);
    return;
  }
  if (!rowok) return;
  if (p.ep == EP_DGRAD_UP2) {
    store_frames(p.y2, v);
    float hv[FPT / 2];
#pragma unroll
    for (int k = 0; k < FPT / 2; ++k) hv[k] = v[2 * k] + v[2 * k + 1];
    const int Th = To / 2, fh = f0 / 2;
    if (Th >= FPT / 2) {
      const int cl = fh / Th, tt = fh - cl * Th;
      float* d = p.y + ((size_t)(b0 + cl) * p.Cout + cgl) * Th + tt;
#pragma unroll
      for (int k = 0; k < FPT / 2; ++k) d[k] = hv[k];
    } else {
#pragma unroll
      for (int k = 0; k < FPT / 2; ++k) {
        const int f = fh + k, cl = f / Th, tt = f - cl * Th;
        p.y[((size_t)(b0 + cl) * p.Cout + cgl) * Th + tt] = hv[k];
      }
    }
    return;
  }
  if (p.ep != EP_BARE) {
#pragma unroll
    for (int k = 0; k < FPT; ++k) v[k] = lrelu(p.ep == EP_LRELU ? v[k] : fmaf(v[k], sc, sh), p.slope);
  }
  store_frames(p.y, v);
  CL_STAMP(7);
}

template <int KW, int S, int NB, bool UP2, int K8W, bool DG2 = false>
__global__ __launch_bounds__(256, 1) void clip32_kernel(const Clip32Args p) {
  prefetch_kernargs<sizeof(Clip32Args)>();
  clip32_body<KW, S, NB, UP2, K8W, DG2>(p, blockIdx.x);
}

struct ClipPairArgs {
  int nA;
  Clip32Args a, b;
};
template <int KWA, int SA, int NBA, bool UP2A, int K8WA, int KWB, int SB, int NBB, bool UP2B, int K8WB>
__global__ __launch_bounds__(256, 1) void clip32_pair_kernel(const ClipPairArgs pp) {
  const unsigned bid = blockIdx.x;
  if (bid < (unsigned)pp.nA) {
    prefetch_kernargs<sizeof(Clip32Args)>();
    clip32_body<KWA, SA, NBA, UP2A, K8WA>(pp.a, bid);
  } else {
    prefetch_kernargs<384>((int)offsetof(ClipPairArgs, b));
    clip32_body<KWB, SB, NBB, UP2B, K8WB>(pp.b, bid - (unsigned)pp.nA);
  }
}

struct ClipPrepJob {
  const float* w;
  float* out;
  int rows, red, KW, k8w, transposed, w_rows, w_cols, block_end;
};
enum { CLIP_PREP_MAX = 40 };
struct ClipPrepBatch { int n; ClipPrepJob job[CLIP_PREP_MAX]; };

constexpr int CLP_LDS = 32 * 289;
__global__ __launch_bounds__(256) void clip32_prep_kernel(const ClipPrepBatch pb) {
  __shared__ float lds[CLP_LDS];
  int j = 0;
  while (j + 1 < pb.n && (int)blockIdx.x >= pb.job[j].block_end) ++j;
  const ClipPrepJob& jb = pb.job[j];
  const int blk = blockIdx.x - (j ? pb.job[j - 1].block_end : 0);
  const int wv = blk & 3, ct = blk >> 2, t = threadIdx.x;
  const int KW = jb.KW, k8w = jb.k8w;
  const int c_lo = wv * k8w * 8, nc = min(k8w * 8, max(0, jb.red - c_lo));
  const int r_lo = 32 * ct, nr = min(32, jb.rows - r_lo);
  int pitch;
  if (!jb.transposed) {
    const int seg = nc * KW;
    pitch = (k8w * 8 * KW) | 1;
    for (int k = t; k < seg; k += 256) {
      const float* src = jb.w + ((size_t)r_lo * jb.w_cols + c_lo) * KW + k;
      const size_t rstride = (size_t)jb.w_cols * KW;
      float v[32];
#pragma unroll
      for (int rr = 0; rr < 32; ++rr) v[rr] = src[(size_t)min(rr, nr - 1) * rstride];
#pragma unroll
      for (int rr = 0; rr < 32; ++rr)
        if (rr < nr) lds[rr * pitch + k] = v[rr];
    }
  } else {
    const int seg = nr * KW;
    pitch = (32 * KW) | 1;
    const int n = nc * seg;
    for (int e0 = t; e0 < n; e0 += 8 * 256) {
      float v[8];
      int dst[8];
#pragma unroll
      for (int u = 0; u < 8; ++u) {
        const int e = min(e0 + 256 * u, n - 1);
        const int cc = e / seg, k = e - cc * seg;
        dst[u] = cc * pitch + k;
        v[u] = jb.w[((size_t)(c_lo + cc) * jb.w_cols + r_lo) * KW + k];
      }
#pragma unroll
      for (int u = 0; u < 8; ++u)
        if (e0 + 256 * u < n) lds[dst[u]] = v[u];
    }
  }
  __syncthreads();
  float4* dst = reinterpret_cast<float4*>(jb.out) + ((size_t)(ct * 4 + wv) * k8w * KW) * 64;
  const int lane = t & 63, rr = lane & 31, h = lane >> 5;
  for (int u = t >> 6; u < k8w * KW; u += 4) {
    const int k8l = u / KW, tap = u - k8l * KW;
    float vv[4];
#pragma unroll
    for (int q = 0; q < 4; ++q) {
      const int cl = 8 * k8l + 4 * h + q;
      float val = 0.f;
      if (rr < nr && cl < nc) val = jb.transposed ? lds[cl * pitch + rr * KW + (jb.transposed == 1 ? KW - 1 - tap : tap)] : lds[rr * pitch + cl * KW + tap];
      vv[q] = val;
    }
    dst[(size_t)u * 64 + lane] = float4{vv[0], vv[1], vv[2], vv[3]};
  }
}

int g_clip32 = 1;

static int clip_k8w(int red) { return (cdiv(red, 8) + 3) / 4; }

static bool clip_geom_ok(int B, int rows, int red, int To, int KW, int S, int groups, int nb) {
  if (!g_clip32 || groups != 1) return false;
  if (!((KW == 3 && S == 1) || (KW == 4 && S == 2))) return false;
  if (To < 1 || To > 32 * nb || (To & (To - 1))) return false;
  if ((B * To) % (32 * nb)) return false;
  if (red > 8 * 4 * CL_MAXK8W || rows < 1) return false;
  return true;
}

bool clip32_fwd_ok(const ms_conv_desc* d) {
  if ((d->dtype & 0xff) != 0) return false;
  if (!(d->H == 1 && d->KH == 1 && d->PW == 1 && d->in_mode != MS_IN_BCAST)) return false;
  const int nb = d->SW == 2 ? 1 : 2;
  if (d->in_mode == MS_IN_UP2ADD && !(d->KW == 3 && d->SW == 1)) return false;
  if (d->OW * d->SW != d->W) return false;
  return clip_geom_ok(d->B, d->Cout, d->Cin, d->OW, d->KW, d->SW, d->groups, nb);
}

bool clip32_dgrad_ok(const ms_conv_desc* d) {
  if ((d->dtype & 0xff) != 0) return false;
  if (!(d->H == 1 && d->KH == 1 && d->PW == 1 && d->in_mode != MS_IN_BCAST)) return false;
  if (d->KW == 4 && d->SW == 2) return d->in_mode == 0 && 2 * d->OW == d->W && clip_geom_ok(d->B, d->Cin, d->Cout, d->W, 4, 2, d->groups, 2);
  if (!(d->KW == 3 && d->SW == 1)) return false;
  return clip_geom_ok(d->B, d->Cin, d->Cout, d->W, 3, 1, d->groups, 2);
}

size_t clip32_weight_floats(int rows, int red, int KW) { return (size_t)cdiv(rows, 32) * 4 * clip_k8w(red) * KW * 256; }

size_t clip32_fwd_weight_bytes(const ms_conv_desc* d) { return clip32_fwd_ok(d) ? clip32_weight_floats(d->Cout, d->Cin, d->KW) * 4 : 0; }
size_t clip32_dgrad_weight_floats(const ms_conv_desc* d) { return clip32_dgrad_ok(d) ? clip32_weight_floats(d->Cin, d->Cout, d->KW) : 0; }

static ClipPrepBatch g_prep;
static int g_prep_blocks = 0;
int clip32_prep_queue(const float* w, float* out, int rows, int red, int KW, int transposed, int w_cols, hipStream_t s) {
  if (g_prep.n == CLIP_PREP_MAX) { const int rc = clip32_prep_flush(s); if (rc) return rc; }
  ClipPrepJob jb = {w, out, rows, red, KW, clip_k8w(red), transposed, 0, w_cols, 0};
  g_prep_blocks += cdiv(rows, 32) * 4;
  jb.block_end = g_prep_blocks;
  g_prep.job[g_prep.n++] = jb;
  return 0;
}
void clip32_prep_discard() { g_prep.n = 0; g_prep_blocks = 0; }
int clip32_prep_flush(hipStream_t s) {
  if (!g_prep.n) return 0;
  TimingScope ts(s, 0, 0, "clip32_prep_kernel|clip_prep jobs%d", g_prep.n);
  const int blocks = g_prep_blocks;
  ClipPrepBatch pb = g_prep;
  g_prep.n = 0; g_prep_blocks = 0;
  if (ts.skip()) return 0;
  hipLaunchKernelGGL(clip32_prep_kernel, dim3(blocks), dim3(256), 0, s, pb);
  return check_launch("clip32_prep_kernel");
}

size_t clip32_part_bytes(int rows, int npw) { return align_up((size_t)cdiv(rows, 32) * npw * 32 * 2 * sizeof(float), 256); }
int clip32_sync_words(int rows) { return 32 * (cdiv(rows, 32) + 1); }

template <int KW, int S, int NB, bool UP2, int K8W, bool DG2 = false>
static int clip32_launch_k(const Clip32Args& a, int nwg, int lds_bytes, hipStream_t s) {
  auto fn = clip32_kernel<KW, S, NB, UP2, K8W, DG2>;
  static unsigned long long attr_done = 0;
  if (first_time_on_device(attr_done)) {
    if (hipFuncSetAttribute(reinterpret_cast<const void*>(fn), hipFuncAttributeMaxDynamicSharedMemorySize, 160 * 1024) != hipSuccess)
      return set_error("clip32: cannot raise the dynamic LDS limit");
    done_on_device(attr_done);
  }
  hipLaunchKernelGGL(fn, dim3(nwg), dim3(256), lds_bytes, s, a);
  return check_launch("clip32_kernel");
}
template <int KW, int S, int NB, bool UP2, bool DG2 = false>
static int clip32_launch_t(const Clip32Args& a, int nwg, int lds_bytes, hipStream_t s) {
  switch (a.k8w) {
    case 2: return clip32_launch_k<KW, S, NB, UP2, 2, DG2>(a, nwg, lds_bytes, s);
    case 4: return clip32_launch_k<KW, S, NB, UP2, 4, DG2>(a, nwg, lds_bytes, s);
    case 8: return clip32_launch_k<KW, S, NB, UP2, 8, DG2>(a, nwg, lds_bytes, s);
    case 9: return clip32_launch_k<KW, S, NB, UP2, 9, DG2>(a, nwg, lds_bytes, s);
    default: return clip32_launch_k<KW, S, NB, UP2, 0, DG2>(a, nwg, lds_bytes, s);
  }
}

struct ClipJob {
  Clip32Args a;
  int KW, S, nb, nwg, lds;
  bool up2, dg2;
  const char* what;
  double flops, bytes;
};

enum { CLIP_HOST_DOWN8 = 0, CLIP_HOST_UP8 = 1, CLIP_HOSTS = 2 };
enum { CLIP_GUEST_K3_4 = 0, CLIP_GUEST_DOWN2 = 1, CLIP_GUEST_DOWN4 = 2, CLIP_GUEST_DOWN8 = 3, CLIP_GUESTS = 4 };
static int clip_host_kind(const ClipJob& j) {
  if (j.dg2 || j.a.k8w != 8) return -1;
  if (j.KW == 4 && j.S == 2 && !j.up2) return CLIP_HOST_DOWN8;
  if (j.KW == 3 && j.S == 1 && j.up2) return CLIP_HOST_UP8;
  return -1;
}
static int clip_guest_kind(const ClipJob& j) {
  if (j.dg2 || j.up2) return -1;
  if (j.KW == 3 && j.S == 1) return j.a.k8w == 4 ? CLIP_GUEST_K3_4 : -1;
  if (j.KW == 4 && j.S == 2) return j.a.k8w == 2 ? CLIP_GUEST_DOWN2 : j.a.k8w == 4 ? CLIP_GUEST_DOWN4 : j.a.k8w == 8 ? CLIP_GUEST_DOWN8 : -1;
  return -1;
}
template <int KWA, int SA, int NBA, bool UP2A, int K8WA, int KWB, int SB, int NBB, bool UP2B, int K8WB>
static int clip32_pair_launch_k(const ClipPairArgs& pp, int nwg, int lds_bytes, hipStream_t s) {
  auto fn = clip32_pair_kernel<KWA, SA, NBA, UP2A, K8WA, KWB, SB, NBB, UP2B, K8WB>;
  static unsigned long long attr_done = 0;
  if (first_time_on_device(attr_done)) {
    if (hipFuncSetAttribute(reinterpret_cast<const void*>(fn), hipFuncAttributeMaxDynamicSharedMemorySize, 160 * 1024) != hipSuccess)
      return set_error("clip32: cannot raise the dynamic LDS limit");
    done_on_device(attr_done);
  }
  hipLaunchKernelGGL(fn, dim3(nwg), dim3(256), lds_bytes, s, pp);
  return check_launch("clip32_pair_kernel");
}
template <int KWA, int SA, int NBA, bool UP2A>
static int clip32_pair_launch_g(int guest, const ClipPairArgs& pp, int nwg, int lds_bytes, hipStream_t s) {
  switch (guest) {
    case CLIP_GUEST_K3_4: return clip32_pair_launch_k<KWA, SA, NBA, UP2A, 8, 3, 1, 2, false, 4>(pp, nwg, lds_bytes, s);
    case CLIP_GUEST_DOWN2: return clip32_pair_launch_k<KWA, SA, NBA, UP2A, 8, 4, 2, 1, false, 2>(pp, nwg, lds_bytes, s);
    case CLIP_GUEST_DOWN4: return clip32_pair_launch_k<KWA, SA, NBA, UP2A, 8, 4, 2, 1, false, 4>(pp, nwg, lds_bytes, s);
    default: return clip32_pair_launch_k<KWA, SA, NBA, UP2A, 8, 4, 2, 1, false, 8>(pp, nwg, lds_bytes, s);
  }
}

static int clip32_issue(ClipJob& j, hipStream_t s) {
  Clip32Args& a = j.a;
  const int nwg = j.nwg;
  TimingScope ts(s, j.flops, j.bytes, "clip32_kernel<%d,%d,%d,%d>|conv_%s_clip k1x%d s%d rows%d red%d T%d B%d ep%d", j.KW, j.S, j.nb, j.up2 ? 1 : 0, j.what,
                 j.KW, j.S, a.rows_valid, a.Cin, a.To, a.B, a.ep);
  if (ts.skip()) return 0;
  static int dbg = -1;
  if (dbg < 0) { const char* e = getenv("MS_CLIP_DBG"); dbg = e ? atoi(e) : 0; }
  static unsigned long long* g_stamps = nullptr;
  if (dbg & 32) {
    if (!g_stamps && hipMalloc(&g_stamps, 4096 * 8 * 8) != hipSuccess) g_stamps = nullptr;
    if (g_stamps) (void)hipMemsetAsync(g_stamps, 0, 4096 * 8 * 8, s);
    a.stamps = nwg <= 4096 ? g_stamps : nullptr;
  }
  int rc;
  if (j.dg2) rc = clip32_launch_t<4, 1, 2, false, true>(a, nwg, j.lds, s);
  else if (j.KW == 3 && j.S == 1) rc = j.up2 ? clip32_launch_t<3, 1, 2, true>(a, nwg, j.lds, s) : clip32_launch_t<3, 1, 2, false>(a, nwg, j.lds, s);
  else rc = clip32_launch_t<4, 2, 1, false>(a, nwg, j.lds, s);
  if (a.stamps) {
    std::vector<unsigned long long> h((size_t)nwg * 8);
    if (hipStreamSynchronize(s) == hipSuccess && hipMemcpy(h.data(), g_stamps, h.size() * 8, hipMemcpyDeviceToHost) == hipSuccess) {
      unsigned long long t0 = ~0ull;
      for (int i = 0; i < nwg; ++i) t0 = std::min(t0, h[(size_t)i * 8]);
      fprintf(stderr, "clip32 %s k%d s%d rows%d red%d ep%d: stamps (us after the first workgroup's entry; min / median / max over %d workgroups)\n", j.what, j.KW, j.S,
              a.rows_valid, a.Cin, a.ep, nwg);
      for (int k = 0; k < 8; ++k) {
        std::vector<double> v;
        for (int i = 0; i < nwg; ++i) if (h[(size_t)i * 8 + k]) v.push_back((double)(h[(size_t)i * 8 + k] - t0) * 0.01);
        if (v.empty()) continue;
        std::sort(v.begin(), v.end());
        fprintf(stderr, "  stamp %d: %7.2f %7.2f %7.2f\n", k, v.front(), v[v.size() / 2], v.back());
      }
    }
    a.stamps = nullptr;
  }
  return rc;
}

int g_clip_corun = -1;
enum { HOLD_IDLE = 0, HOLD_ARMED = 1, HOLD_PENDING = 2 };
struct ClipHold {
  int state = HOLD_IDLE;
  ClipJob job;
  const char* ws_lo = nullptr;
  const char* ws_hi = nullptr;
};
static std::mutex g_hold_mu;
static std::map<hipStream_t, ClipHold> g_hold;
static thread_local bool t_in_fwd = false;
static thread_local const char* t_ws_lo = nullptr;
static thread_local const char* t_ws_hi = nullptr;

static bool clip_corun_on() {
  if (g_clip_corun < 0) { const char* e = getenv("MS_CLIP_CORUN"); g_clip_corun = e ? (atoi(e) != 0) : 1; }
  return g_clip_corun != 0;
}

int clip32_hold_arm(hipStream_t s) {
  std::lock_guard<std::mutex> lk(g_hold_mu);
  ClipHold& h = g_hold[s];
  if (h.state == HOLD_PENDING) return set_error("ms_clip_hold: a held block is pending on this stream (flush or discard it first)");
  h.state = HOLD_ARMED;
  return 0;
}
void clip32_hold_discard(hipStream_t s) {
  std::lock_guard<std::mutex> lk(g_hold_mu);
  auto it = g_hold.find(s);
  if (it != g_hold.end()) it->second.state = HOLD_IDLE;
}
int clip32_hold_flush(hipStream_t s) {
  ClipJob job;
  {
    std::lock_guard<std::mutex> lk(g_hold_mu);
    auto it = g_hold.find(s);
    if (it == g_hold.end()) return 0;
    const int st = it->second.state;
    it->second.state = HOLD_IDLE;
    if (st != HOLD_PENDING) return 0;
    job = it->second.job;
  }
  return clip32_issue(job, s);
}
int clip32_fwd_call_begin(hipStream_t s, bool clip_path, const void* ws, size_t ws_bytes) {
  t_in_fwd = true;
  t_ws_lo = (const char*)ws; t_ws_hi = t_ws_lo + (ws ? ws_bytes : 0);
  bool flush = false;
  {
    std::lock_guard<std::mutex> lk(g_hold_mu);
    auto it = g_hold.find(s);
    if (it != g_hold.end() && it->second.state == HOLD_PENDING)
      flush = !clip_path || (t_ws_lo < it->second.ws_hi && it->second.ws_lo < t_ws_hi);
  }
  return flush ? clip32_hold_flush(s) : 0;
}
void clip32_fwd_call_end(hipStream_t s) {
  t_in_fwd = false;
  std::lock_guard<std::mutex> lk(g_hold_mu);
  auto it = g_hold.find(s);
  if (it != g_hold.end() && it->second.state == HOLD_ARMED) it->second.state = HOLD_IDLE;
}

static bool clip_pair_fits(const ClipJob& A, const ClipJob& B) {
  if (!clip_corun_on()) return false;
  if (clip_host_kind(A) < 0 || clip_guest_kind(B) < 0) return false;
  if (A.nwg % 8) return false;
  int cus = current_device_cus();
  if (cus <= 0) cus = 256;
  return A.nwg + B.nwg <= cus;
}
static bool clip_pair_ok(const ClipJob& A, const ClipJob& B) {
  if (!clip_pair_fits(A, B)) return false;
  const bool meetA = A.a.ep == EP_RAW_STATS && A.a.npw > 1, meetB = B.a.ep == EP_RAW_STATS && B.a.npw > 1;
  if (meetA && meetB && (A.a.part == B.a.part || A.a.sync == B.a.sync)) return false;
  return true;
}
static int clip32_issue_pair(ClipJob& A, ClipJob& B, hipStream_t s) {
  char da[96], db[96];
  snprintf(da, sizeof(da), "conv_%s_clip k1x%d s%d rows%d red%d T%d B%d ep%d", A.what, A.KW, A.S, A.a.rows_valid, A.a.Cin, A.a.To, A.a.B, A.a.ep);
  snprintf(db, sizeof(db), "conv_%s_clip k1x%d s%d rows%d red%d T%d B%d ep%d", B.what, B.KW, B.S, B.a.rows_valid, B.a.Cin, B.a.To, B.a.B, B.a.ep);
  TimingScope ts(s, A.flops + B.flops, A.bytes + B.bytes, "clip32_kernel<%d,%d,%d,%d>+<%d,%d,%d,%d>|%s + %s", A.KW, A.S, A.nb, A.up2 ? 1 : 0, B.KW, B.S,
                 B.nb, B.up2 ? 1 : 0, da, db);
  if (ts.skip()) return 0;
  ClipPairArgs pp;
  pp.nA = A.nwg; pp.a = A.a; pp.b = B.a;
  pp.a.stamps = pp.b.stamps = nullptr;
  const int nwg = A.nwg + B.nwg, lds = std::max(A.lds, B.lds), guest = clip_guest_kind(B);
  return clip_host_kind(A) == CLIP_HOST_DOWN8 ? clip32_pair_launch_g<4, 2, 1, false>(guest, pp, nwg, lds, s)
                                              : clip32_pair_launch_g<3, 1, 2, true>(guest, pp, nwg, lds, s);
}

int clip32_launch(Clip32Args a, int KW, int S, bool up2, const char* what, hipStream_t s, bool dg2 = false, ClipJob* plan = nullptr) {
  const int nb = (S == 2 && !dg2) ? 1 : 2, npx = 32 * nb;
  a.k8w = clip_k8w(a.Cin);
  a.npw = a.B * a.To / npx;
  if (a.sg < 1) a.sg = 1;
  if (a.npw % a.sg) return -2;
  const int nct = cdiv(a.Cout, 32);
  a.nct = nct;
  const int ncl = npx / a.To, pslots = cl_pslots(ncl * (a.Ti + 2));
  const int img = 4 * a.k8w * 2 * pslots * 16, red = (4 * 32 * (npx + 4) + 4) * 4;
  const int lds = std::max(img, red);
  if (lds > 160 * 1024) return set_error("clip32: image of %d bytes", lds);
  const int nwg = nct * a.npw;
  static int xcd_on = -1;
  if (xcd_on < 0) { const char* e = getenv("MS_CLIP_XCD"); xcd_on = e ? atoi(e) : 1; }
  a.cx = a.px = 0;
  if (xcd_on && nwg % 8 == 0) {
    const double wct = 32.0 * a.Cin * KW, imgb = (double)a.Cin * ncl * a.Ti * (up2 ? 1.5 : 1.0);
    double best = nct % 8 == 0 ? wct * (nct / 8) + imgb * a.npw : 1e30;
    for (int cx = 4; cx >= 1; cx >>= 1) {
      const int px = 8 / cx;
      if (nct % cx || a.npw % px) continue;
      const double cost = wct * (nct / cx) + imgb * (a.npw / px);
      if (cost < best) { best = cost; a.cx = cx; a.px = px; }
    }
  }
  int cus = 256;
  cus = current_device_cus();
  if (!cus) cus = 256;
  if ((a.ep == EP_RAW_STATS || a.ep == EP_DGRAD_BN) && a.npw > 1 && nwg > cus) return -2;
  ClipJob job;
  job.a = a; job.KW = KW; job.S = S; job.nb = nb; job.nwg = nwg; job.lds = lds; job.up2 = up2; job.dg2 = dg2; job.what = what;
  job.flops = 2.0 * a.rows_valid * a.Cin * (dg2 ? 2 : KW) * (double)a.B * a.To;
  job.bytes = 4.0 * ((double)a.rows_valid * a.Cin * KW + (double)a.B * a.Cin * a.Ti + (double)a.B * a.rows_valid * a.To);
  if (plan) { *plan = job; return 0; }
  if (t_in_fwd) {
    ClipJob held;
    int st;
    {
      std::lock_guard<std::mutex> lk(g_hold_mu);
      auto it = g_hold.find(s);
      st = it == g_hold.end() ? HOLD_IDLE : it->second.state;
      if (st == HOLD_ARMED) {
        it->second.state = HOLD_PENDING;
        it->second.job = job;
        it->second.ws_lo = t_ws_lo; it->second.ws_hi = t_ws_hi;
      } else if (st == HOLD_PENDING) {
        it->second.state = HOLD_IDLE;
        held = it->second.job;
      }
    }
    if (st == HOLD_ARMED) return 0;
    if (st == HOLD_PENDING) {
      if (clip_pair_ok(job, held)) return clip32_issue_pair(job, held, s);
      const int rc = clip32_issue(held, s);
      if (rc) return rc;
    }
  }
  return clip32_issue(job, s);
}

static int clip32_fwd_plan(const ms_conv_desc* d, ClipJob* plan) {
  if (!clip32_fwd_ok(d)) return 0;
  Clip32Args a = {};
  a.B = d->B; a.Cin = d->Cin; a.Cout = d->Cout; a.rows_valid = d->Cout; a.To = d->OW; a.Ti = d->W;
  a.ep = d->mode == MS_BARE ? EP_BARE : d->mode == MS_LRELU ? EP_LRELU : d->mode == MS_BN_EVAL ? EP_BN_EVAL : EP_RAW_STATS;
  a.sg = a.ep == EP_RAW_STATS ? sg_of(d) : 1;
  plan->nwg = 0;
  if (clip32_launch(a, d->KW, d->SW, d->in_mode == MS_IN_UP2ADD, "fwd", nullptr, false, plan) != 0) return 0;
  return plan->nwg;
}
int clip32_fwd_grid(const ms_conv_desc* d) {
  ClipJob plan;
  return clip32_fwd_plan(d, &plan);
}
bool clip32_fwd_pair_ok(const ms_conv_desc* host, const ms_conv_desc* guest) {
  ClipJob A, B;
  return clip32_fwd_plan(host, &A) > 0 && clip32_fwd_plan(guest, &B) > 0 && clip_pair_fits(A, B);
}

int clip32_block_fwd(const ms_conv_desc* d, const float* x, const float* x2, const float* wp, const float* bias, const float* gamma,
                     const float* beta, float* rm, float* rv, float* y_raw, float* y, float* save, float* part, int* sync,
                     int sync_words, hipStream_t s) {
  Clip32Args a = {};
  a.x = x; a.x2 = x2; a.wp = wp; a.bias = bias; a.gamma = gamma; a.beta = beta; a.rm = rm; a.rv = rv;
  a.y_raw = d->mode == MS_BN_TRAIN ? y_raw : nullptr; a.y = y; a.save = save; a.part = part; a.sync = sync; a.cnt_base = 32;
  a.B = d->B; a.Cin = d->Cin; a.Cout = d->Cout; a.rows_valid = d->Cout; a.To = d->OW; a.Ti = d->W;
  a.ep = d->mode == MS_BARE ? EP_BARE : d->mode == MS_LRELU ? EP_LRELU : d->mode == MS_BN_EVAL ? EP_BN_EVAL : EP_RAW_STATS;
  a.slope = d->slope; a.eps = d->eps; a.momentum = d->momentum;
  if (a.ep == EP_RAW_STATS && (!sync || sync_words < 32 + clip32_sync_words(d->Cout) || !part)) return -2;
  a.sg = a.ep == EP_RAW_STATS ? sg_of(d) : 1;
  a.raw_all = (long)d->B / a.sg * d->OW > BN_BWD32_FUSED_MAX ? 1 : 0;
  return clip32_launch(a, d->KW, d->SW, d->in_mode == MS_IN_UP2ADD, "fwd", s);
}

bool clip32_dgrad_bn_ok(const ms_conv_desc* d) {
  if (!clip32_dgrad_ok(d) || d->in_mode != MS_IN_PLAIN) return false;
  const int cus = current_device_cus();
  return cus > 0 && cdiv(d->Cin, 32) * (d->B * d->W / 64) <= cus;
}
size_t clip32_dgrad_bn_part_bytes(const ms_conv_desc* d) {
  return clip32_dgrad_ok(d) && d->in_mode == MS_IN_PLAIN ? align_up((size_t)cdiv(d->Cin, 32) * (d->B * d->W / 64) * 32 * 4 * sizeof(float), 256) : 0;
}

int clip32_block_dgrad(const ms_conv_desc* d, const float* g, const float* wp, float* dx, float* dx2, hipStream_t s,
                       const Clip32PrevBN* pv, float* part, int* sync, int sync_words, const float* accum) {
  Clip32Args a = {};
  const bool up2 = d->in_mode == MS_IN_UP2ADD;
  if (accum && up2) return set_error("clip32 data gradient: dx_accum with an upsample-add input");
  a.acc = accum;
  a.x = g; a.wp = wp;
  a.y = dx; a.y2 = dx2;
  a.B = d->B; a.Cin = d->Cout; a.Cout = d->Cin; a.rows_valid = d->Cin; a.To = d->W; a.Ti = d->W;
  a.ep = up2 ? EP_DGRAD_UP2 : EP_BARE;
  if (pv) {
    if (up2 || !part || !sync || sync_words < 32 + clip32_sync_words(d->Cin) || !pv->y || !pv->y_raw || !pv->save || !pv->gamma)
      return set_error("clip32 data gradient with the producer's BatchNorm backward: missing buffer");
    a.ep = EP_DGRAD_BN;
    a.pv_y = pv->y; a.pv_y_raw = pv->y_raw; a.pv_save = pv->save; a.pv_gamma = pv->gamma;
    a.pv_dgamma = pv->dgamma; a.pv_dbeta = pv->dbeta; a.pv_dbias = pv->dbias;
    a.slope = pv->slope; a.part = part; a.sync = sync; a.cnt_base = 32;
  }
  if (d->KW == 4) {
    a.Ti = d->OW;
    return clip32_launch(a, 4, 2, false, "dgrad", s, true);
  }
  return clip32_launch(a, 3, 1, false, "dgrad", s);
}

}
```

mix_stage_amd/csrc/kernels.h:

```cpp
#pragma once
#include "common.h"

namespace ms {

enum { EP_BARE = 0, EP_LRELU = 1, EP_BN_EVAL = 2, EP_RAW_STATS = 3, EP_DGRAD = 4, EP_DGRAD_UP2 = 5, EP_BN_FUSED = 6, EP_DGRAD_BN = 7, EP_DGRAD_ACC = 8 };

struct GatherArgs {
  const float* A;
  const float* src;
  const float* src2;
  float* out;
  float* out2;
  const float* bias;
  const float* bn_g;
  const float* bn_b;
  const float* bn_m;
  const float* bn_v;
  float* stats;
  int Mg, Kg, groups, Kc, src_ctotal, SRCH, SRCW, OUTH, OUTW, Npix;
  int KH, KW, SH, SW, PH, PW;
  int bcast, a_vec, ep;
  int batch;
  int splitk, k_per_split;
  float* part;
  size_t part_stride;
  float slope, eps;
};

struct WgradArgs {
  const float* dyr;
  const float* src;
  const float* src2;
  float* out;
  int Cog, Cig, Kg, groups, src_ctotal, H, W, OH, OW, Npix;
  int KH, KW, SH, SW, PH, PW;
  int bcast, splits, r_per_split;
  int accumulate;
};
constexpr int WG_MAX_JOBS = 24;
struct WgradBatch {
  int n;
  int block_end[WG_MAX_JOBS];
  WgradArgs job[WG_MAX_JOBS];
};

struct TimingScope {
  TimingScope(hipStream_t s, double flops, double bytes, const char* fmt, ...);
  ~TimingScope();
  bool skip() const { return skip_; }
  int idx_;
  hipStream_t s_;
  bool skip_;
};

struct PatchArgs {
  const float* A;
  const float* src;
  const float* src2;
  float* out;
  const float* bias;
  const float* bn_g;
  const float* bn_b;
  const float* bn_m;
  const float* bn_v;
  float* stats;
  float* counts;
  int Mg, Kg, groups, Kc, bcast, a_vec, ep;
  int SRCH, SRCW, s_img, s_chan, s_row;
  int OUTH, OUTW, o_img, o_chan, o_row;
  int o_sh, o_sw, o_ry, o_rx;
  float* out2;
  int is_dgrad;
  int gx, gy, gz;
  int splitk, chunks_per_split;
  float* part;
  size_t part_stride;
  int PH, PW, tiles_x, tiles_y;
  float slope, eps;
  size_t src_elems, a_elems;
  int ncls, cls_PH[4], cls_PW[4], cls_OUTH[4], cls_OUTW[4], cls_ry[4], cls_rx[4];
  unsigned cls_a_stride;
  int cls_fast;
  const unsigned short* Aplanes;
  unsigned plane_stride;
  int a_row_elems;
};
struct PatchPlan { int ok, tm, tw, tiles_y, tiles_x, n_tiles, splitk, chunks_per_split, tn, wm, ksi, p6, tile; };
PatchPlan plan_patch(int nd, int Mg, int groups, int Kc, int KH, int KW, int SH, int SW, int B, int OH, int OW, int zmul = 1, int in_w = 0);
extern int g_conv_tile;
bool conv_tile_shape_ok(int KH, int KW, int S);
int launch_tile(const PatchArgs& a, const PatchPlan& pl, int KH, int KW, int S, double flops, double bytes, hipStream_t s);
int patch_chunk_channels(int KH, int KW);
bool patch_dgrad_direct_ok(const float* w, int Cin_g, int KH, int KW, int SH, int SW, bool up2_or_bcast);
int launch_patch(const PatchArgs& a, const PatchPlan& pl, int KH, int KW, int S, bool up2, double flops, double bytes,
                 hipStream_t s);

bool conv_c1_ok(int groups, int Cin, int Cout, int KH, int KW, int SH, int SW, int PH, int PW, int H, int in_plain);
int conv_c1_tiles(int B, int H, int W);
bool wgrad_c1_ok(int groups, int Cin, int Cout, int KH, int KW, int SH, int SW, int PH, int PW, int H, int W, int in_plain);
int wgrad_c1_splits(int B, int H);
int launch_wgrad_c1(const float* dyr, const float* x, float* part, int B, int H, int W, hipStream_t s);
int launch_conv_c1(const float* x, const float* w, const float* bias, float* out, const float* bn_g, const float* bn_b,
                   const float* bn_m, const float* bn_v, float* stats, float* counts, int B, int H, int W, int ep, float slope,
                   float eps, hipStream_t s);
extern int g_patch_intra;
extern int g_precision;
bool patch6_supported(int KH, int KW, int S);
int patch6_row_elems(int Kc, int KH, int KW);
int launch_split_weights(const float* w, unsigned short* planes, int rows, int Kc, int KH, int KW, hipStream_t s);
struct SplitJob {
  const float* w;
  unsigned short* planes;
  int rows, Kc, KHW, CK, row_elems, block_end;
};
enum { SPLIT_BATCH_MAX = 64 };
struct SplitBatch { int n; SplitJob job[SPLIT_BATCH_MAX]; };
int launch_split_weights_multi(SplitBatch& sb, hipStream_t s);
int launch_patch6(const PatchArgs& a, const PatchPlan& pl, int KH, int KW, int S, bool up2, double flops, double bytes,
                  hipStream_t s);
extern int g_patch_min_wgs;

struct WgradPatchArgs {
  const float* dyr;
  const float* src;
  const float* src2;
  float* out;
  int Cog, Cig, Kg, groups, bcast;
  int SRCH, SRCW, s_img, s_chan, s_row, PH, PW;
  int OUTH, OUTW, o_img, o_chan, o_row;
  int tiles_x, tiles_y, n_tiles, tiles_per_split, splits;
  int gx, gy, gz;
  int accumulate;
  int n_steps, steps_per_split;
  int wave_kind;
  int KH, KW, w4, nx4, xrp, xcp, xbuf;
  int* counters;
  float* final_out;
};
struct WgradPatchPlan { int ok, tw, tiles_y, tiles_x, n_tiles, splits, tiles_per_split, p6, wave; };
constexpr int WGP_MAX_JOBS = 48;
struct WgradPatchBatch {
  int n;
  int block_end[WGP_MAX_JOBS];
  WgradPatchArgs job[WGP_MAX_JOBS];
};
int queue_wgrad_patch(const WgradPatchArgs& a, const WgradPatchPlan& pl, int KH, int KW, int S, bool up2, double flops, double bytes);
int wgrad_patch_flush(hipStream_t s);
void wgrad_patch_discard();
bool wgrad6_supported(int KH, int KW, int S);
int launch_wgrad_patch6(const WgradPatchArgs& a, const WgradPatchPlan& pl, int KH, int KW, int S, bool up2, double flops,
                        double bytes, hipStream_t s);
WgradPatchPlan plan_wgrad_patch(int nd, int Cog, int Kg, int groups, int KH, int KW, int SH, int SW, int B, int OH, int OW, int W = 0,
                                bool up2 = false);
int launch_wgrad_patch(const WgradPatchArgs& a, const WgradPatchPlan& pl, int KH, int KW, int S, bool up2, double flops,
                       double bytes, hipStream_t s);
int launch_reduce_splits(const float* part, float* out, int n, int splits, hipStream_t s);

struct Clip32Args;
bool clip32_fwd_ok(const ms_conv_desc* d);
bool clip32_dgrad_ok(const ms_conv_desc* d);
size_t clip32_fwd_weight_bytes(const ms_conv_desc* d);
size_t clip32_dgrad_weight_floats(const ms_conv_desc* d);
size_t clip32_weight_floats(int rows, int red, int KW);
int clip32_prep_queue(const float* w, float* out, int rows, int red, int KW, int transposed, int w_cols, hipStream_t s);
int clip32_prep_flush(hipStream_t s);
void clip32_prep_discard();
void gdgrad32_prep_discard();
struct PrepQueueGuard { ~PrepQueueGuard() { clip32_prep_discard(); gdgrad32_prep_discard(); } };
size_t clip32_part_bytes(int rows, int npw);
int clip32_sync_words(int rows);
int clip32_block_fwd(const ms_conv_desc* d, const float* x, const float* x2, const float* wp, const float* bias, const float* gamma,
                     const float* beta, float* rm, float* rv, float* y_raw, float* y, float* save, float* part, int* sync,
                     int sync_words, hipStream_t s);
extern int g_clip_corun;
int clip32_hold_arm(hipStream_t s);
int clip32_hold_flush(hipStream_t s);
void clip32_hold_discard(hipStream_t s);
int clip32_fwd_call_begin(hipStream_t s, bool clip_path, const void* ws, size_t ws_bytes);
void clip32_fwd_call_end(hipStream_t s);
int clip32_fwd_grid(const ms_conv_desc* d);
bool clip32_fwd_pair_ok(const ms_conv_desc* host, const ms_conv_desc* guest);
struct Clip32PrevBN { const float* y; const float* y_raw; const float* save; const float* gamma; float* dgamma; float* dbeta; float* dbias; float slope; };
size_t clip32_dgrad_bn_part_bytes(const ms_conv_desc* d);
bool clip32_dgrad_bn_ok(const ms_conv_desc* d);
int clip32_block_dgrad(const ms_conv_desc* d, const float* g, const float* wp, float* dx, float* dx2, hipStream_t s,
                       const Clip32PrevBN* pv = nullptr, float* part = nullptr, int* sync = nullptr, int sync_words = 0,
                       const float* accum = nullptr);

bool gdgrad32_ok(const ms_conv_desc* d);
size_t gdgrad32_weight_floats(const ms_conv_desc* d);
int gdgrad32_prepare(const ms_conv_desc* d, const float* w, float* out, hipStream_t s);
int gdgrad32_prep_flush(hipStream_t s);
int gdgrad32_launch(const ms_conv_desc* d, const float* g, const float* wp, float* dx, hipStream_t s);

int chain32_supported(const ms_chain_desc* d);
size_t chain32_prepared_bytes(const ms_chain_desc* d);
size_t chain32_workspace(const ms_chain_desc* d);
int chain32_sync_words(const ms_chain_desc* d);
int chain32_prepare(const ms_chain_desc* d, const float* const* w, const float* wl, void* prepared, hipStream_t s);
int chain32_fwd(const ms_chain_desc* d, const ms_chain_tensors* tn, void* workspace, size_t workspace_bytes, hipStream_t s);
int chain16_supported(const ms_chain_desc* d);
size_t chain16_prepared_bytes(const ms_chain_desc* d);
size_t chain16_workspace(const ms_chain_desc* d);
int chain16_sync_words(const ms_chain_desc* d);
int chain16_prepare(const ms_chain_desc* d, const float* const* w, const float* wl, void* prepared, hipStream_t s);
int chain16_fwd(const ms_chain_desc* d, const ms_chain_tensors* tn, void* workspace, size_t workspace_bytes, hipStream_t s);
constexpr int CHAIN_EVAL_TILE = 64, CHAIN_EVAL_HALO = 4, CHAIN_EVAL_STEP = CHAIN_EVAL_TILE - 2 * CHAIN_EVAL_HALO, CHAIN_EVAL_FILL = 256,
              CHAIN_EVAL_MAX_PARTS = 2048;
struct ChainEvalPlan { int n_tiles, gpw, ngw; long units; };
ChainEvalPlan chain_eval_plan(const ms_chain_desc* d);
int chain_eval_shape_ok(const ms_chain_desc* d);
size_t chain_eval_workspace(const ms_chain_desc* d);
int chain_eval_sync_words(const ms_chain_desc* d);
int chain16_eval_fwd(const ms_chain_desc* d, const ms_chain_tensors* tn, void* workspace, size_t workspace_bytes, hipStream_t s);

struct GatherPlan { int tm, tn, splitk, k_per_split, n_tiles; };
GatherPlan plan_gather(int Mg, int npix, int zcount, int Kg);
int launch_gather(GatherArgs a, bool transposed, bool up2, const GatherPlan& plan, hipStream_t s);
int launch_splitk_fwd_epilogue(const float* part, int splitk, size_t part_stride, const float* bias, const float* gamma,
                               const float* beta, float* rm, float* rv, float* y_raw, float* y, float* save, int B, int C,
                               int HW, int ep, float slope, float eps, float momentum, hipStream_t s, int sg = 1);
int launch_splitk_dgrad_epilogue(const float* part, int splitk, size_t part_stride, float* dx, float* dx2, size_t n, int W,
                                 int up2, hipStream_t s);
int wgrad_splits(int Cog, int Kg, int groups, int Npix);
int launch_wgrad(WgradArgs a, bool up2, float* dw, float* partial_ws, bool defer_reduce, hipStream_t s, bool queue = false);
int wgrad_gather_flush(hipStream_t s);
void wgrad_gather_discard();
struct ReduceJob {
  const float* part;
  float* out;
  int n, splits, wave, block_end;
};
enum { REDUCE_BATCH_MAX = 96 };
struct ReduceBatch { int n; ReduceJob job[REDUCE_BATCH_MAX]; };
int launch_reduce_splits_multi(ReduceBatch& rb, hipStream_t s);
struct TransposeJob {
  const float* w;
  float* wt;
  int groups, Cog, Cig, KH, KW, SH, SW, PH, PW, flip;
  int block_end;
};
enum { TRANSPOSE_BATCH_MAX = 48 };
struct TransposeBatch { int n; TransposeJob job[TRANSPOSE_BATCH_MAX]; };
int launch_transpose_weight_multi(TransposeBatch& tb, hipStream_t s);
int launch_transpose_weight(const float* w, float* wt, int groups, int Cog, int Cig, int KH, int KW, int SH, int SW,
                            int PH, int PW, int flip, hipStream_t s);
size_t dgrad_weight_elems(int groups, int Cog, int Cig, int KH, int KW, int SH, int SW);
int launch_bn_finalize(const float* stats, const float* counts, int n_tiles, int tile_n, int N, int C, const float* gamma,
                       const float* beta, float* rm, float* rv, float* save, float eps, float momentum, hipStream_t s);
int launch_bn_apply(const float* y_raw, float* y, const float* save, int C, int HW, size_t total, float slope, hipStream_t s);
int launch_bn_finalize_apply(const float* stats, const float* counts, int n_tiles, int tile_n, int N, int C, const float* gamma,
                             const float* beta, float* rm, float* rv, float* save, float eps, float momentum, const float* y_raw,
                             float* y, int B, int HW, float slope, hipStream_t s);
int bwd_chunks(int B, int C, int* b_per_chunk);
constexpr int BN_BWD32_FUSED_MAX = 256 * 16;
int launch_bn_bwd(const float* dy, const float* y_raw, const float* y, const float* save, const float* gamma, float* partial, float* dyr,
                  float* colpart, float* dbias, float* dgamma, float* dbeta, int B, int C, int HW, float slope, int* fused,
                  hipStream_t s, int sg = 1);
int launch_act_bwd(const float* dy, const float* y, float* dyr, float* colpart, float* dbias, int B, int C, int HW, int mode, float slope, int* fused,
                   hipStream_t s);
int launch_colsum_finalize(const float* colpart, float* out, int B, int C, hipStream_t s);
int launch_adam_seg(float* p, const float* g, float* m, float* v, size_t n, const int32_t* step_state, const int32_t* seg_of_chunk,
                    const float* seg_scratch, float beta1, float beta2, float eps, hipStream_t s);

__device__ inline float adam_seg_step_size(float lr, float beta1, double t) { return (float)((double)lr / (1.0 - pow((double)beta1, t))); }
__device__ inline float adam_seg_bc2(float beta2, double t) { return (float)sqrt(1.0 - pow((double)beta2, t)); }
__device__ inline float adam_clip_coef(float max_norm, float n) {
  const float coef = max_norm / (n + 1e-6f);
  return coef > 1.f ? 1.f : coef;
}
__device__ inline bool adam_norm_finite(float n) { return fabsf(n) <= 3.0e38f; }
__device__ inline bool adam_lr_bad(float lr) { return !(lr > 0.f && lr <= 3.0e38f); }
__device__ inline void adam_flag_step(int32_t* state, bool bad) {
  state[2] = bad ? 1 : 0;
  if (bad) state[3] += 1;
}
__device__ inline int adam_meeting_raised(bool finite, const int32_t* const* __restrict__ meeting_words, int n_meeting_words) {
  int raised = 0;
  if (!finite)
    for (int i = threadIdx.x; i < n_meeting_words; i += blockDim.x)
      if (meeting_words[i] && meeting_words[i][0] != 0) raised = 1;
  return raised;
}
__device__ inline void adam_scaled_tail(int32_t* state, float* norm, float raw, bool finite, bool meeting, bool bad_lr, int step,
                                        float max_norm, int32_t* ls, int growth_interval, float min_scale, float max_scale) {
  float* lf = reinterpret_cast<float*>(ls);
  float S = lf[0];
  const float inv_S = lf[1];
  int good = ls[2];
  state[0] = step;
  const float n = raw * inv_S;
  norm[0] = n;
  reinterpret_cast<float*>(state)[1] = adam_clip_coef(max_norm, n) * inv_S;
  int skipped = 0;
  if (bad_lr) {
    state[2] = 1;
    state[3] += 1;
  } else if (finite) {
    state[2] = 0;
    if (good < 0x7fffffff) good += 1;
    if (growth_interval > 0 && good >= growth_interval && S < max_scale) { S *= 2.f; good = 0; }
  } else {
    state[2] = 1;
    good = 0;
    if (S > min_scale && !meeting) { S *= 0.5f; ls[3] += 1; skipped = 1; }
    else state[3] += 1;
  }
  lf[0] = S;
  lf[1] = 1.f / S;
  ls[2] = good;
  ls[4] = skipped;
}

}
```

mix_stage_amd/ops.py:

```python
import contextlib
import ctypes
import os

import torch

from . import _lib
from ._lib import (BwdOptions, ConvDesc, FwdOptions, MS_BARE, MS_BN_EVAL, MS_BN_TRAIN, MS_DT_STAT_PAIR, MS_IN_BCAST, MS_IN_PLAIN,
                   MS_IN_UP2ADD, MS_LRELU, check, lib)

_vp = ctypes.c_void_p


def _ptr(t):
  return None if t is None else _vp(t.data_ptr())


def _stream():
  return _vp(torch.cuda.current_stream().cuda_stream)


def _need_hip(*tensors):
  for t in tensors:
    if t is None:
      continue
    if not t.is_cuda:
      raise _lib.MixStageLibError('mix_stage_amd ops run on the MI355X only (got a %s tensor); there is no CPU '
                                  'fallback' % t.device)
    if t.is_floating_point() and t.dtype != torch.float32:
      raise TypeError('the HIP path computes in float32 (got %s); call .float() on the model and inputs' % t.dtype)


_workspaces = {}
_counters = {}
USE_IN_LAUNCH_SPLIT_REDUCTION = False


def _ensure_counters(device):
  key = (device.type, device.index)
  if key not in _counters:
    buf = torch.zeros(1 << 16, dtype=torch.int32, device=device)
    check(lib().ms_set_counter_buffer(_ptr(buf), buf.numel()), 'ms_set_counter_buffer')
    _counters[key] = buf
  return _counters[key]



_corun = {'driver': None, 'held': False, 'keep': [], 'on': os.environ.get('MS_CLIP_CORUN', '1') != '0', 'merges_offered': 0}


def workspace(nbytes, device):
  key = (device.type, device.index, torch.cuda.current_stream(device).cuda_stream)
  if _corun['held']:
    key = key + ('held',)
  if USE_IN_LAUNCH_SPLIT_REDUCTION:
    _ensure_counters(device)
  ws = _workspaces.get(key)
  if ws is None or ws.numel() < nbytes:
    size = max(int(nbytes * 1.5), 1 << 22)
    if ws is not None:
      _retired_workspaces.append(ws)
    ws = torch.empty(size, dtype=torch.uint8, device=device)
    _workspaces[key] = ws
  return ws


_retired_workspaces = []


_side_workspaces = {}


def side_workspace(nbytes, device):
  key = (device.type, device.index)
  ws = _side_workspaces.get(key)
  if ws is None or ws.numel() < nbytes:
    ws = torch.empty(max(int(nbytes * 1.5), 1 << 22), dtype=torch.uint8, device=device)
    _side_workspaces[key] = ws
  return ws


_overlap = {'stream': None, 'keep': []}


def set_backward_overlap(side_stream):
  _overlap['stream'] = side_stream
  _overlap['keep'].clear()


def join_backward_overlap():
  side = _overlap['stream']
  if side is not None:
    torch.cuda.current_stream().wait_stream(side)
  _overlap['keep'].clear()


_prepared = {'on': False, 'entries': {}, 'by_storage': {}}


def enable_prepared_weights(on):
  _prepared['on'] = bool(on)
  if not on:
    _prepared['entries'].clear()
    _prepared['by_storage'].clear()


def _prepare_entries(entries):
  entries = [e for e in entries if e['n']]
  if not entries:
    return
  L = lib()
  tune = L.ms_tuning_epoch()
  e16 = [e for e in entries if e['kind'].endswith('16')]
  if e16:
    from . import ops16
    ops16._prepare16(e16)
  for e in entries:
    if e['kind'] == 'chain32':
      wl = (ctypes.c_void_p * 4)(*[x.data_ptr() for x in e['ws'][:4]])
      check(L.ms_decoder_chain_prepare(ctypes.byref(e['d']), wl, _ptr(e['ws'][4]), _ptr(e['wt']), _stream()), 'ms_decoder_chain_prepare')
      e['version'], e['tune'] = sum(x._version for x in e['ws']), tune
  for kind, fn in (('dgrad', L.ms_dgrad_weights_prepare), ('fwd', L.ms_fwd_weights_prepare)):
    es = [e for e in entries if e['kind'] == kind]
    if not es:
      continue
    n = len(es)
    descs = (ConvDesc * n)(*[e['d'] for e in es])
    ws = (ctypes.c_void_p * n)(*[e['w'].data_ptr() for e in es])
    outs = (ctypes.c_void_p * n)(*[e['wt'].data_ptr() for e in es])
    check(fn(n, descs, ws, outs, _stream()), 'ms_%s_weights_prepare' % kind)
    for e in es:
      e['version'], e['tune'] = e['w']._version, tune


def _prepared_for(w, d, kind='dgrad'):
  if not _prepared['on']:
    return None
  L = lib()
  key = (w.data_ptr(), id(d), kind)
  tune = L.ms_tuning_epoch()
  e = _prepared['entries'].get(key)
  if e is None or e['tune'] != tune:
    if kind == 'dgrad':
      n = L.ms_dgrad_weights_elems(ctypes.byref(d), _ptr(w))
    else:
      n = (L.ms_fwd_weights_bytes(ctypes.byref(d)) + 3) // 4
    if e is None:
      e = dict(w=w, d=d, n=0, wt=None, version=-1, tune=-1, kind=kind)
      _prepared['entries'][key] = e
      _prepared['by_storage'].setdefault(w.untyped_storage().data_ptr(), []).append(e)
    if n != e['n']:
      e['n'], e['wt'] = n, (torch.empty(n, dtype=torch.float32, device=w.device) if n else None)
    e['version'] = -1
    if not n:
      e['tune'] = tune
  if not e['n']:
    return None
  if e['version'] != w._version or e['tune'] != tune:
    _prepare_entries([e])
  return e['wt']


def drop_trainer_caches(storage_ptrs):
  for sp in storage_ptrs:
    for e in _prepared['by_storage'].pop(sp, ()):
      _prepared['entries'] = {k: v for k, v in _prepared['entries'].items() if v is not e}
  _deferred['bufs'] = {k: v for k, v in _deferred['bufs'].items() if v[2] not in storage_ptrs}


def refresh_prepared_weights(flat_params, start=0):
  if _prepared['on']:
    _prepare_entries(_prepared['by_storage'].get(flat_params.untyped_storage().data_ptr(), ())[start:])


def prepared_count(flat_params):
  return len(_prepared['by_storage'].get(flat_params.untyped_storage().data_ptr(), ()))


_deferred = {'on': False, 'jobs': [], 'queued': False, 'bufs': {}, 'keep': [], 'launches': 0}
DEFER_WGRAD_LAUNCH = os.environ.get('MS_DEFER_WGRAD_LAUNCH', '1') != '0'


def enable_deferred_wgrad(on):
  _deferred['on'] = bool(on)
  lib().ms_set_wgrad_batched(1 if (on and DEFER_WGRAD_LAUNCH) else 0, int(os.environ.get('MS_WGRAD_TPS', '0')))
  reset_deferred_wgrad()
  if not on:
    _deferred['bufs'].clear()


def reset_deferred_wgrad():
  _deferred['jobs'].clear()
  _deferred['keep'].clear()
  _deferred['queued'] = False
  if _deferred['launches']:
    _deferred['launches'] = 0
    lib().ms_wgrad_discard()


def _queue_deferred_flush():
  owner = (torch.cuda.current_device(), _stream().value)
  if not _deferred['queued']:
    _deferred['queued'] = True
    _deferred['owner'] = owner
    torch.autograd.Variable._execution_engine.queue_callback(_flush_deferred_wgrad)
  elif _deferred.get('owner') != owner:
    raise _lib.MixStageLibError('deferred weight-gradient work was queued from two devices or streams in one backward pass '
                                '(%s, then %s): run concurrent trainers in separate processes or with '
                                'ops.enable_deferred_wgrad(False)' % (_deferred.get('owner'), owner))


def _wgrad_partials_for(w, d):
  info = getattr(d, '_wg_split', None)
  tune = lib().ms_tuning_epoch()
  if info is None or info[2] != tune:
    sp = ctypes.c_int(1)
    n = lib().ms_wgrad_partials_elems(ctypes.byref(d), ctypes.byref(sp))
    info = d._wg_split = (n, sp.value, tune)
  if not info[0]:
    return None, 1
  key = (w.data_ptr(), id(d))
  buf = _deferred['bufs'].get(key)
  if buf is None or buf[0].numel() != info[0]:
    buf = _deferred['bufs'][key] = (torch.empty(info[0], dtype=torch.float32, device=w.device), d,
                                    w.untyped_storage().data_ptr())
  return buf[0], info[1]


def _flush_deferred_wgrad():
  jobs = _deferred['jobs']
  _deferred['queued'] = False
  if _deferred['launches']:
    _deferred['launches'] = 0
    try:
      check(lib().ms_wgrad_flush(_stream()), 'ms_wgrad_flush')
    finally:
      _deferred['keep'].clear()
  if not jobs:
    return
  rounds, seen = [], {}
  for j in jobs:
    k = seen.get(j[1].data_ptr(), 0)
    seen[j[1].data_ptr()] = k + 1
    if k == len(rounds):
      rounds.append([])
    rounds[k].append(j)
  try:
    for rj in rounds:
      n = len(rj)
      parts = (ctypes.c_void_p * n)(*[j[0].data_ptr() for j in rj])
      outs = (ctypes.c_void_p * n)(*[j[1].data_ptr() for j in rj])
      elems = (ctypes.c_int * n)(*[j[1].numel() for j in rj])
      splits = (ctypes.c_int * n)(*[j[2] for j in rj])
      check(lib().ms_wgrad_reduce_multi(n, parts, outs, elems, splits, _stream()), 'ms_wgrad_reduce_multi')
  finally:
    jobs.clear()


class ConvGeom:
  __slots__ = ('nd', 'groups', 'KH', 'KW', 'SH', 'SW', 'PH', 'PW', 'slope', 'eps', 'momentum', '_cache')

  def __init__(self, nd, groups, kernel, stride, padding, slope=0.2, eps=1e-5, momentum=0.1):
    def two(v):
      if isinstance(v, (tuple, list)):
        return (1, int(v[0])) if len(v) == 1 else (int(v[0]), int(v[1]))
      return (int(v), int(v)) if nd == 2 else (1, int(v))
    self.nd, self.groups = nd, groups
    self.KH, self.KW = two(kernel)
    self.SH, self.SW = two(stride)
    ph, pw = two(padding)
    self.PH, self.PW = (ph, pw) if nd == 2 else (0, pw)
    if nd == 1:
      self.KH, self.SH = 1, 1
    self.slope, self.eps, self.momentum = float(slope), float(eps), float(momentum)
    self._cache = {}

  def desc(self, B, Cin_g, H, W, Cout_g, mode, in_mode, dtype=0):
    key = (B, Cin_g, H, W, Cout_g, mode, in_mode, dtype)
    d = self._cache.get(key)
    if d is None:
      OH = (H + 2 * self.PH - self.KH) // self.SH + 1
      OW = (W + 2 * self.PW - self.KW) // self.SW + 1
      if OH < 1 or OW < 1:
        raise RuntimeError('conv block: input (%d,%d) too small for kernel (%d,%d)' % (H, W, self.KH, self.KW))
      d = ConvDesc(B, Cin_g, H, W, Cout_g, self.groups, self.KH, self.KW, self.SH, self.SW, self.PH, self.PW,
                   OH, OW, mode, in_mode, self.slope, self.eps, self.momentum, dtype)
      d._tune = -1
      self._cache[key] = d
    L = lib()
    tune = L.ms_tuning_epoch()
    if d._tune != tune:
      d._fwd_ws = L.ms_conv_block_fwd_workspace(ctypes.byref(d))
      d._bwd_ws = L.ms_conv_block_bwd_workspace(ctypes.byref(d))
      d._tune = tune
    return d


_stat_pair = {'on': False}


@contextlib.contextmanager
def stat_pair():
  old = _stat_pair['on']
  _stat_pair['on'] = True
  try:
    yield
  finally:
    _stat_pair['on'] = old


def stat_pair_active():
  return _stat_pair['on']


def stat_pair_ok(geom, B2, Cin_g, W, Cout_g, mode, dtype=0):
  d = geom.desc(B2, Cin_g, 1, W, Cout_g, mode, MS_IN_PLAIN, dtype | MS_DT_STAT_PAIR)
  return bool(lib().ms_stat_pair_ok(ctypes.byref(d))), d.OW


LATE = 'late'


def _grad_slot(param, shape_like):
  slot = getattr(param, '_ms_grad_slot', None) if param is not None else None
  if slot is not None and torch.is_grad_enabled() is False:
    if getattr(param, '_ms_grad_fresh', False):
      param._ms_grad_fresh = False
      return slot, True
    if _deferred['on']:
      tmp = torch.empty_like(slot)
      _deferred['jobs'].append((tmp, slot, 1))
      _queue_deferred_flush()
      return tmp, LATE
  return torch.empty_like(shape_like), False


_link_stats = {'in_launch': 0}


class ResidualLink:
  __slots__ = ('armed', 'grad', 'taken')

  def __init__(self):
    self.armed, self.grad, self.taken = False, None, False


class _ConvBlockFn(torch.autograd.Function):
  @staticmethod
  def forward(ctx, x, x2, w, bias, gamma, beta, geom, mode, in_mode, stats, pre=None, prev=None, link=None):
    rm, rv = stats if stats is not None else (None, None)
    _need_hip(x, x2, w, bias, gamma, beta, rm, rv)
    x = x.contiguous()
    x2 = x2.contiguous() if x2 is not None else None
    nd = geom.nd
    if x.dim() != nd + 2:
      raise RuntimeError('conv block expects a %d-D input, got %s' % (nd + 2, tuple(x.shape)))
    B = x.shape[0]
    ref = x2 if in_mode == MS_IN_UP2ADD else x
    H, W = (ref.shape[2], ref.shape[3]) if nd == 2 else (1, ref.shape[2])
    ctot = w.shape[0]
    Cout_g = ctot // geom.groups
    Cin_g = w.shape[1]
    exp_c = Cin_g if in_mode == MS_IN_BCAST else Cin_g * geom.groups
    if x.shape[1] != exp_c:
      raise RuntimeError('conv block: expected %d input channels, got %d' % (exp_c, x.shape[1]))
    if in_mode == MS_IN_UP2ADD and (x.shape[2] * 2 != W or x2.shape[1] != exp_c):
      raise RuntimeError('UP2ADD: a %s and residual %s do not match' % (tuple(x.shape), tuple(x2.shape)))
    pair = MS_DT_STAT_PAIR if (_stat_pair['on'] and pre is None) else 0
    d = geom.desc(B, Cin_g, H, W, Cout_g, mode, in_mode, pair)
    oshape = (B, ctot, d.OH, d.OW) if nd == 2 else (B, ctot, d.OW)
    if pre is not None:
      y_raw, y, save = pre
      if tuple(y.shape) != oshape:
        raise RuntimeError('precomputed block output has shape %s, expected %s' % (tuple(y.shape), oshape))
    else:
      y = torch.empty(oshape, dtype=torch.float32, device=x.device)
      y_raw = save = None
      if mode == MS_BN_TRAIN:
        y_raw = torch.empty_like(y)
        save = torch.empty((8 if pair else 4) * ctot, dtype=torch.float32, device=x.device)
    ws = workspace(d._fwd_ws, x.device) if pre is None else None
    planes = _prepared_for(w, d, 'fwd') if pre is None else None
    if pre is None:
      sync = None
      if mode == MS_BN_TRAIN and nd == 1:
        from . import ops16
        sync = ops16.block_sync(x.device, d)
      opt = FwdOptions(planes.data_ptr() if planes is not None else None, sync.data_ptr() if sync is not None else None,
                       sync.numel() if sync is not None else 0)
      check(lib().ms_conv_block_fwd_ex(ctypes.byref(d), _ptr(x), _ptr(x2), _ptr(w), _ptr(bias), _ptr(gamma), _ptr(beta),
                                       _ptr(rm), _ptr(rv), _ptr(y_raw), _ptr(y), _ptr(save), _ptr(ws), ws.numel(),
                                       _stream(), ctypes.byref(opt)), 'ms_conv_block_fwd_ex')
      if _corun['held']:
        _corun['keep'].append((x, x2, w, bias, gamma, beta, rm, rv, y_raw, y, save, ws, planes, sync))
    ctx.geom_desc = d
    ctx.mode, ctx.in_mode = mode, in_mode
    ctx.prev = None
    ctx.dy_is_dyr = False
    if prev is not None and pre is None and in_mode == MS_IN_PLAIN and nd == 1 and getattr(prev, 'mode', None) == MS_BN_TRAIN \
        and not bn_sync_active() and lib().ms_dgrad_fuses_prev_bn(ctypes.byref(d)):
      from . import ops16
      py = prev.saved_tensors[5]
      watched = bool(getattr(x, '_backward_hooks', None)) or bool(getattr(x, 'retains_grad', False))
      if ops16.in_launch_meetings() and not watched and py is not None and py.data_ptr() == x.data_ptr() and tuple(py.shape) == tuple(x.shape):
        ctx.prev = prev
    ctx.link = None
    if link is not None and pre is None and nd == 1 and not bn_sync_active():
      lk, role = link
      if role == 'consumer' and in_mode == MS_IN_PLAIN and x.requires_grad and lib().ms_dgrad_takes_accum(ctypes.byref(d)) \
          and not (getattr(x, '_backward_hooks', None) or getattr(x, 'retains_grad', False)):
        lk.armed = True
        ctx.link = link
      elif role == 'residual' and in_mode == MS_IN_UP2ADD and lk.armed:
        ctx.link = link
    ctx.has_bias = bias is not None
    ctx.params = (w, bias, gamma, beta)
    ctx.save_for_backward(x, x2, w, gamma, y_raw, y if mode in (MS_LRELU, MS_BN_TRAIN) else None, save)
    return y

  @staticmethod
  def backward(ctx, dy):
    x, x2, w, gamma, y_raw, y, save = ctx.saved_tensors
    d, mode, in_mode = ctx.geom_desc, ctx.mode, ctx.in_mode
    if mode == MS_BN_EVAL:
      raise RuntimeError('backward through an eval-mode (running-stats) ConvNormRelu is not on the path')
    need_x, need_x2, need_w = ctx.needs_input_grad[0], ctx.needs_input_grad[1], ctx.needs_input_grad[2]
    need_bn = mode == MS_BN_TRAIN and ctx.needs_input_grad[4]
    dy = dy.contiguous()
    dev = dy.device
    is_dyr = bool(ctx.dy_is_dyr)
    ctx.dy_is_dyr = False
    dyr = torch.empty_like(dy) if (mode != MS_BARE and not is_dyr) else None
    up2 = in_mode == MS_IN_UP2ADD
    want_dx = need_x or (up2 and need_x2)
    dx = torch.empty_like(x) if want_dx else None
    dx2 = torch.empty_like(x2) if (want_dx and up2) else None
    pw, pbias, pgamma, pbeta = ctx.params
    dw = dbias = dgamma = dbeta = None
    direct_w = direct_b = direct_g = direct_be = False
    if need_w:
      dw, direct_w = _grad_slot(pw, w)
      if ctx.has_bias and not is_dyr:
        dbias, direct_b = _grad_slot(pbias, pbias)
    if need_bn and not is_dyr:
      dgamma, direct_g = _grad_slot(pgamma, gamma)
      dbeta, direct_be = _grad_slot(pbeta, gamma)
    if is_dyr:
      direct_b = direct_g = direct_be = True
    fuse = None
    prev = ctx.prev
    if prev is not None and want_dx and not up2 and _overlap['stream'] is None and not torch.is_grad_enabled():
      ppw, ppbias, ppgamma, ppbeta = prev.params
      p_need_w, p_need_bn = prev.needs_input_grad[2], prev.needs_input_grad[4]
      wanted = ([ppbias] if (p_need_w and prev.has_bias) else []) + ([ppgamma, ppbeta] if p_need_bn else [])
      if all(getattr(q, '_ms_grad_slot', None) is not None and (getattr(q, '_ms_grad_fresh', False) or _deferred['on']) for q in wanted):
        _, _, _, pgam_t, py_raw, py, psave = prev.saved_tensors
        if py_raw is not None and py is not None and psave is not None:
          from . import ops16
          sync = ops16.block_sync(dev, d, tag='dgrad_bn')
          if sync is not None:
            pdb = _grad_slot(ppbias, ppbias)[0] if (p_need_w and prev.has_bias) else None
            pdg = _grad_slot(ppgamma, pgam_t)[0] if p_need_bn else None
            pdbe = _grad_slot(ppbeta, pgam_t)[0] if p_need_bn else None
            fuse = (py, py_raw, psave, pgam_t, pdg, pdbe, pdb, sync, float(prev.geom_desc.slope))
    acc = None
    if ctx.link is not None and ctx.link[1] == 'consumer':
      acc, ctx.link[0].grad = ctx.link[0].grad, None
      ctx.link[0].taken = True
      if acc is not None and (not want_dx or tuple(acc.shape) != tuple(x.shape)):
        raise RuntimeError('residual link: a residual gradient of shape %s arrived for an input of shape %s (needs grad: %s)' %
                           (tuple(acc.shape), tuple(x.shape), want_dx))
    acc_in_launch = False
    ws = workspace(d._bwd_ws, dev)
    side = _overlap['stream']
    if side is not None and need_w and direct_w is not True:
      torch.cuda.current_stream().wait_stream(side)
    if side is not None and direct_w is True and (dbias is None or direct_b is True):
      ws2 = side_workspace(d._bwd_ws, dev)
      _overlap['keep'].append((x, x2, dy, dyr))
      check(lib().ms_conv_block_bwd_overlap(ctypes.byref(d), _ptr(x), _ptr(x2), _ptr(w), _ptr(gamma), None, None,
                                            _ptr(y_raw), _ptr(y), _ptr(save), _ptr(dy), _ptr(dyr), _ptr(dx), _ptr(dx2),
                                            _ptr(dw), _ptr(dbias), _ptr(dgamma), _ptr(dbeta), _ptr(ws), ws.numel(),
                                            _stream(), _vp(side.cuda_stream), _ptr(ws2), ws2.numel()),
            'ms_conv_block_bwd_overlap')
    else:
      wt = _prepared_for(w, d) if want_dx else None
      part, nsplit = (None, 1)
      if _deferred['on'] and direct_w is True:
        part, nsplit = _wgrad_partials_for(w, d)
      defer_launch = bool(_deferred['on'] and direct_w is True and dw is not None and DEFER_WGRAD_LAUNCH)
      if wt is not None or part is not None or defer_launch or fuse is not None or is_dyr or acc is not None:
        opt = BwdOptions(None, None, 0, wt.data_ptr() if wt is not None else None,
                         part.data_ptr() if part is not None else None, 1 if defer_launch else 0)
        if acc is not None:
          acc = acc.contiguous()
          opt.dx_accum = acc.data_ptr()
          acc_in_launch = True
          _link_stats['in_launch'] += 1
        if fuse is not None:
          py, py_raw, psave, pgam_t, pdg, pdbe, pdb, sync, pslope = fuse
          opt.prev_y, opt.prev_y_raw, opt.prev_save, opt.prev_gamma = py.data_ptr(), py_raw.data_ptr(), psave.data_ptr(), pgam_t.data_ptr()
          opt.prev_dgamma = pdg.data_ptr() if pdg is not None else None
          opt.prev_dbeta = pdbe.data_ptr() if pdbe is not None else None
          opt.prev_dbias = pdb.data_ptr() if pdb is not None else None
          opt.prev_slope, opt.bn_sync, opt.bn_sync_words = pslope, sync.data_ptr(), sync.numel()
          prev.dy_is_dyr = True
        opt.dy_is_dyr = 1 if is_dyr else 0
        check(lib().ms_conv_block_bwd_ex(ctypes.byref(d), _ptr(x), _ptr(x2), _ptr(w), _ptr(gamma), None, None, _ptr(y_raw),
                                         _ptr(y), _ptr(save), _ptr(dy), _ptr(dyr), _ptr(dx), _ptr(dx2), _ptr(dw),
                                         _ptr(dbias), _ptr(dgamma), _ptr(dbeta), _ptr(ws), ws.numel(), _stream(),
                                         ctypes.byref(opt)), 'ms_conv_block_bwd_ex')
        if defer_launch:
          _deferred['launches'] += 1
          _deferred['keep'].append((x, x2, dy, dyr, dw, part))
          _queue_deferred_flush()
        if part is not None:
          _deferred['jobs'].append((part, dw, nsplit))
          _queue_deferred_flush()
      else:
        check(lib().ms_conv_block_bwd(ctypes.byref(d), _ptr(x), _ptr(x2), _ptr(w), _ptr(gamma), None, None, _ptr(y_raw),
                                      _ptr(y), _ptr(save), _ptr(dy), _ptr(dyr), _ptr(dx), _ptr(dx2), _ptr(dw),
                                      _ptr(dbias), _ptr(dgamma), _ptr(dbeta), _ptr(ws), ws.numel(), _stream()),
              'ms_conv_block_bwd')
    if acc is not None and not acc_in_launch:
      dx.add_(acc)
    if ctx.link is not None and ctx.link[1] == 'residual' and dx2 is not None and ctx.needs_input_grad[1] and not ctx.link[0].taken:
      ctx.link[0].grad = dx2
      dx2 = None
    return (dx, dx2, None if direct_w else dw, None if direct_b else dbias, None if direct_g else dgamma,
            None if direct_be else dbeta, None, None, None, None, None, None, None)


def _f32(t):
  return t.float() if isinstance(t, torch.Tensor) and t.dtype == torch.float64 else t


def _bridge64(fn):
  def wrapped(*args, **kw):
    vals = list(args) + list(kw.values())
    if not any(isinstance(a, torch.Tensor) and a.dtype == torch.float64 for a in vals):
      return fn(*args, **kw)
    out = fn(*[_f32(a) for a in args], **{k: _f32(v) for k, v in kw.items()})
    back = lambda o: o.double() if isinstance(o, torch.Tensor) and o.dtype == torch.float32 else o
    return tuple(back(o) for o in out) if isinstance(out, tuple) else back(out)
  wrapped.__doc__, wrapped.__name__ = fn.__doc__, fn.__name__
  return wrapped


_chain_fusion = {'on': os.environ.get('MS_CHAIN_BN', '1') != '0'}


def enable_chain_fusion(on):
  old = _chain_fusion['on']
  _chain_fusion['on'] = bool(on)
  return old


_links16 = {'on': os.environ.get('MS_LINK16', '0') == '1'}


def enable_residual_links16(on):
  old = _links16['on']
  _links16['on'] = bool(on)
  return old


def residual_links16_active():
  return _links16['on'] and _chain_fusion['on']


def conv_block(x, w, bias, geom, mode, gamma=None, beta=None, running_mean=None, running_var=None, x2=None,
               in_mode=MS_IN_PLAIN, chain_prev=False, link=None):
  if w.dtype == torch.float64 or x.dtype == torch.float64:
    rm32, rv32 = _f32(running_mean), _f32(running_var)
    stats = (rm32, rv32) if rm32 is not None else None
    y = _ConvBlockFn.apply(_f32(x), _f32(x2), _f32(w), _f32(bias), _f32(gamma), _f32(beta), geom, mode, in_mode, stats)
    if mode == MS_BN_TRAIN and running_mean is not None and running_mean.dtype == torch.float64:
      with torch.no_grad():
        running_mean.copy_(rm32)
        running_var.copy_(rv32)
    return y.double()
  stats = (running_mean, running_var) if running_mean is not None else None
  prev = x.grad_fn if (chain_prev and _chain_fusion['on'] and x.grad_fn is not None and type(x.grad_fn).__name__ == '_ConvBlockFnBackward') else None
  link = link if (link is not None and _chain_fusion['on'] and torch.is_grad_enabled()) else None
  drv = _corun['driver']
  held = drv is not None and not drv.in_guest and geom.nd == 1 and drv.offer(x, x2, w, geom, mode, in_mode)
  if not held:
    return _ConvBlockFn.apply(x, x2, w, bias, gamma, beta, geom, mode, in_mode, stats, None, prev, link)
  try:
    y = _ConvBlockFn.apply(x, x2, w, bias, gamma, beta, geom, mode, in_mode, stats, None, prev, link)
    check(lib().ms_clip_hold_flush(_stream()), 'ms_clip_hold_flush')
  except BaseException:
    lib().ms_clip_hold_discard(_stream())
    raise
  finally:
    _corun['keep'].clear()
  return y


class _CoRun:

  def __init__(self, guest_steps, device):
    self.gen, self.in_guest, self.done, self.result = guest_steps, False, False, None
    self.cus = torch.cuda.get_device_properties(device).multi_processor_count
    self.next_desc = None
    self._resume()

  def _resume(self):
    self.in_guest = True
    try:
      self.next_desc = next(self.gen)
    except StopIteration as e:
      self.done, self.result, self.next_desc = True, e.value, None
    finally:
      self.in_guest = False

  def offer(self, x, x2, w, geom, mode, in_mode):
    if self.done or self.next_desc is None or not x.is_cuda or x.dtype != torch.float32 or w.dtype != torch.float32:
      return False
    ref = x2 if in_mode == MS_IN_UP2ADD else x
    if ref is None or ref.dim() != 3:
      return False
    L = lib()
    d = geom.desc(x.shape[0], w.shape[1], 1, ref.shape[2], w.shape[0] // geom.groups, mode, in_mode, 0)
    n_host, n_guest = L.ms_clip_grid(ctypes.byref(d)), L.ms_clip_grid(ctypes.byref(self.next_desc))
    if not n_host or not n_guest or n_host + n_guest > self.cus or not L.ms_clip_pair_ok(ctypes.byref(d), ctypes.byref(self.next_desc)):
      return False
    stream = _stream()
    check(L.ms_clip_hold(stream), 'ms_clip_hold')
    _corun['held'] = True
    try:
      self._resume()
    except BaseException:
      L.ms_clip_hold_discard(stream)
      raise
    finally:
      _corun['held'] = False
    _corun['merges_offered'] += 1
    return True

  def finish(self):
    while not self.done:
      self._resume()
    return self.result


def corun(host_fn, guest_steps, device):
  if _corun['driver'] is not None:
    raise RuntimeError('corun: a guest chain is already riding along')
  try:
    drv = _CoRun(guest_steps, device)
    _corun['driver'] = drv
    try:
      out = host_fn()
    finally:
      _corun['driver'] = None
    return out, drv.finish()
  except BaseException:
    _corun['driver'] = None
    lib().ms_clip_hold_discard(_stream())
    _corun['keep'].clear()
    raise


def corun_ok(*tensors):
  from . import ops16
  return bool(_corun['on'] and _corun['driver'] is None and not bn_sync_active() and not _stat_pair['on'] and ops16.in_launch_meetings()
              and lib().ms_get_precision() == 0 and all(t.is_cuda and t.dtype == torch.float32 for t in tensors))


def enable_corun(on):
  old = _corun['on']
  _corun['on'] = bool(on)
  return old


_marker = {'cb': None}


def set_backward_marker(callback):
  _marker['cb'] = callback


class _BackwardMarkerFn(torch.autograd.Function):
  @staticmethod
  def forward(ctx, x):
    return x.view_as(x)

  @staticmethod
  def backward(ctx, g):
    cb = _marker['cb']
    if cb is not None:
      cb()
    return g


def backward_marker(x):
  return _BackwardMarkerFn.apply(x) if (_marker['cb'] is not None and x.requires_grad) else x


_bn_sync = {'group': None, 'on': False}


def set_bn_sync(on, process_group=None):
  _bn_sync['on'], _bn_sync['group'] = bool(on), process_group


def bn_sync_active():
  import torch.distributed as dist
  return _bn_sync['on'] and dist.is_available() and dist.is_initialized() and dist.get_world_size(_bn_sync['group']) > 1


class _SyncBNActFn(torch.autograd.Function):
  @staticmethod
  def forward(ctx, y_raw, gamma, beta, rm, rv, slope, eps, momentum):
    import torch.distributed as dist
    _need_hip(y_raw, gamma, beta, rm, rv)
    y_raw = y_raw.contiguous()
    B, C = y_raw.shape[0], y_raw.shape[1]
    HW = y_raw.numel() // (B * C)
    group = _bn_sync['group']
    world = dist.get_world_size(group)
    stats = torch.empty((C, 2), dtype=torch.float32, device=y_raw.device)
    check(lib().ms_bn_stats(_ptr(y_raw), _ptr(stats), B, C, HW, _stream()), 'ms_bn_stats')
    allstats = torch.empty((world, C, 2), dtype=torch.float32, device=y_raw.device)
    dist.all_gather_into_tensor(allstats, stats, group=group) if dist.get_backend(group) == 'nccl' else \
        allstats.copy_(torch.stack(_all_gather_list(stats, world, group)))
    y = torch.empty_like(y_raw)
    save = torch.empty(4 * C, dtype=torch.float32, device=y_raw.device)
    check(lib().ms_bn_train_apply(_ptr(allstats), world, B * HW, _ptr(gamma), _ptr(beta), _ptr(rm), _ptr(rv), _ptr(y_raw),
                                  _ptr(y), _ptr(save), B, C, HW, eps, momentum, slope, _stream()), 'ms_bn_train_apply')
    ctx.save_for_backward(y_raw, gamma, save)
    ctx.meta = (B, C, HW, slope, world, group)
    ctx.params = (gamma, beta)
    return y

  @staticmethod
  def backward(ctx, dy):
    import torch.distributed as dist
    y_raw, gamma, save = ctx.saved_tensors
    B, C, HW, slope, world, group = ctx.meta
    dy = dy.contiguous()
    sums = torch.empty((C, 2), dtype=torch.float32, device=dy.device)
    ws = workspace(lib().ms_bn_bwd_workspace(B, C), dy.device)
    check(lib().ms_bn_bwd_sums(_ptr(dy), _ptr(y_raw), _ptr(save), _ptr(sums), B, C, HW, slope, _ptr(ws), ws.numel(), _stream()),
          'ms_bn_bwd_sums')
    pgamma, pbeta = ctx.params
    dgamma, direct_g = _grad_slot(pgamma, gamma)
    dbeta, direct_b = _grad_slot(pbeta, gamma)
    dgamma.copy_(sums[:, 1]); dbeta.copy_(sums[:, 0])
    gsum = sums.clone()
    dist.all_reduce(gsum, op=dist.ReduceOp.SUM, group=group)
    dyr = torch.empty_like(dy)
    check(lib().ms_bn_bwd_apply(_ptr(dy), _ptr(y_raw), _ptr(save), _ptr(gamma), _ptr(gsum), float(world) * B * HW, _ptr(dyr), B, C,
                                HW, slope, _stream()), 'ms_bn_bwd_apply')
    return dyr, None if direct_g else dgamma, None if direct_b else dbeta, None, None, None, None, None


def _all_gather_list(t, world, group):
  import torch.distributed as dist
  out = [torch.empty_like(t) for _ in range(world)]
  dist.all_gather(out, t, group=group)
  return out


def sync_bn_act(y_raw, gamma, beta, running_mean, running_var, slope, eps, momentum):
  return _SyncBNActFn.apply(y_raw, gamma, beta, running_mean, running_var, float(slope), float(eps), float(momentum))


CHAIN_SYNC_FIRST_WORD = 32
USE_DECODER_CHAIN = os.environ.get('MS_DECODER_CHAIN', '1') != '0'
USE_DECODER_CHAIN_EVAL = os.environ.get('MS_CHAIN_EVAL', '1') != '0'


def _chain_desc(B, M, T, cin0, P, mode, blk, dtype=0):
  g = blk._geometry()
  return _lib.ChainDesc(B, M, T, cin0, 256, P, 4, mode, dtype, CHAIN_SYNC_FIRST_WORD, 0, g.slope, g.eps, g.momentum)


_chain_scratch = {}


def _chain_prepared(d, ws):
  key = (ws[0].data_ptr(), d.M, d.cin0, d.P, d.dtype, 'chain32')
  if not _prepared['on']:
    n = (lib().ms_decoder_chain_prepared_bytes(ctypes.byref(d)) + 3) // 4
    buf = _chain_scratch.get(key)
    if buf is None or buf.numel() != n:
      _chain_scratch.clear()
      buf = _chain_scratch[key] = torch.empty(n, dtype=torch.float32, device=ws[0].device)
    _prepare_entries([dict(w=ws[0], ws=list(ws), d=d, n=n, wt=buf, version=-1, tune=-1, kind='chain32')])
    return buf
  e = _prepared['entries'].get(key)
  if e is None:
    n = (lib().ms_decoder_chain_prepared_bytes(ctypes.byref(d)) + 3) // 4
    e = dict(w=ws[0], ws=list(ws), d=d, n=n, wt=torch.empty(n, dtype=torch.float32, device=ws[0].device), version=-1, tune=-1,
             kind='chain32')
    _prepared['entries'][key] = e
    _prepared['by_storage'].setdefault(ws[0].untyped_storage().data_ptr(), []).append(e)
  e['ws'] = list(ws)
  if e['version'] != sum(x._version for x in ws):
    _prepare_entries([e])
  return e['wt']


_chain_eval_sync = {}


def _chain_eval_launch(d, x, score, blocks, logits, ws, P):
  if not USE_DECODER_CHAIN_EVAL or not lib().ms_decoder_chain_eval_supported(ctypes.byref(d)):
    return None
  dev = x.device
  prepared = _chain_prepared(d, ws)
  words = lib().ms_decoder_chain_eval_sync_words(ctypes.byref(d))
  sync = None
  if words:
    key = (dev.type, dev.index, torch.cuda.current_stream(dev).cuda_stream, d.B, d.M, d.T)
    sync = _chain_eval_sync.get(key)
    if sync is None or sync.numel() < CHAIN_SYNC_FIRST_WORD + words:
      sync = _chain_eval_sync[key] = torch.zeros(CHAIN_SYNC_FIRST_WORD + words, dtype=torch.int32, device=dev)
  soft = torch.empty((d.B, d.T, d.M), dtype=torch.float32, device=dev)
  out = torch.empty((d.B, d.T, P), dtype=torch.float32, device=dev)
  tn = _lib.ChainTensors()
  tn.x, tn.score = x.data_ptr(), score.data_ptr()
  for l, m in enumerate(blocks):
    tn.w[l], tn.bias[l] = m.conv.weight.data_ptr(), (m.conv.bias.data_ptr() if m.conv.bias is not None else None)
    tn.gamma[l], tn.beta[l] = m.norm.weight.data_ptr(), m.norm.bias.data_ptr()
    tn.running_mean[l], tn.running_var[l] = m.norm.running_mean.data_ptr(), m.norm.running_var.data_ptr()
  tn.w_logits, tn.bias_logits = logits.weight.data_ptr(), logits.bias.data_ptr()
  tn.soft, tn.out, tn.prepared = soft.data_ptr(), out.data_ptr(), prepared.data_ptr()
  if sync is not None:
    tn.sync, tn.sync_words = sync.data_ptr(), sync.numel()
  wsp = workspace(lib().ms_decoder_chain_eval_workspace(ctypes.byref(d)), dev)
  check(lib().ms_decoder_chain_eval_fwd(ctypes.byref(d), ctypes.byref(tn), _ptr(wsp), wsp.numel(), _stream()), 'ms_decoder_chain_eval_fwd')
  return out, soft


def decoder_chain(x, blocks, logits, score, P):
  if not USE_DECODER_CHAIN or len(blocks) != 4 or x.dim() != 3 or not x.is_cuda or x.dtype != torch.float32:
    return None
  from . import ops16
  meetings = ops16.in_launch_meetings() and not bn_sync_active()
  blk0 = blocks[0]
  M = blk0.conv.groups
  B, cin0, T = x.shape
  if any(getattr(m, '_ms_dt', 0) for m in blocks) or any(m._p and m.training for m in blocks):
    return None
  if any(m._forward_hooks or m._forward_pre_hooks for m in list(blocks) + [logits]):
    return None
  if any(m.conv.groups != M or m.conv.kernel_size != (3,) or m.conv.stride != (1,) or m.conv.padding != (1,) or
         m.conv.weight.shape[0] != 256 * M or m.conv.weight.dtype != torch.float32 or m._slope != blk0._slope for m in blocks):
    return None
  if blocks[0].conv.weight.shape[1] != cin0 or any(m.conv.weight.shape[1] != 256 for m in blocks[1:]):
    return None
  if logits.groups != M or logits.kernel_size != (1,) or logits.weight.shape[0] != M * P or logits.weight.shape[1] != 256 or logits.bias is None:
    return None
  if tuple(score.shape) != (B, M, T) or score.dtype != torch.float32:
    return None
  training = all(m.training and m.norm.track_running_stats for m in blocks)
  if not training and any(m.training for m in blocks):
    return None
  mode = MS_BN_TRAIN if training else MS_BN_EVAL
  params = [t for m in blocks for t in (m.conv.weight, m.conv.bias, m.norm.weight, m.norm.bias)] + [logits.weight, logits.bias]
  need_grad = torch.is_grad_enabled() and (x.requires_grad or score.requires_grad or any(t is not None and t.requires_grad for t in params))
  if need_grad and not training:
    return None
  d = _chain_desc(B, M, T, cin0, P, mode, blk0)
  ws = [m.conv.weight for m in blocks] + [logits.weight]
  if not lib().ms_decoder_chain_supported(ctypes.byref(d)):
    if training or need_grad:
      return None
    _need_hip(x, score, *[t for t in params if t is not None])
    return _chain_eval_launch(d, x.contiguous(), score.contiguous(), blocks, logits, ws, P)
  if not meetings:
    return None
  _need_hip(x, score, *[t for t in params if t is not None])
  x, score = x.contiguous(), score.contiguous()
  dev = x.device
  prepared = _chain_prepared(d, ws)
  sync = ops16.chain_sync(dev, B, M, CHAIN_SYNC_FIRST_WORD + lib().ms_decoder_chain_sync_words(ctypes.byref(d)))
  C = 256 * M
  keep = need_grad
  y_raw = [torch.empty((B, C, T), dtype=torch.float32, device=dev) if keep else None for _ in blocks]
  y = [torch.empty((B, C, T), dtype=torch.float32, device=dev) if keep else None for _ in blocks]
  save = [torch.empty(4 * C, dtype=torch.float32, device=dev) if keep else None for _ in blocks]
  z = torch.empty((B, M * P, T), dtype=torch.float32, device=dev) if keep else None
  soft = torch.empty((B, T, M), dtype=torch.float32, device=dev)
  out = torch.empty((B, T, P), dtype=torch.float32, device=dev)
  tn = _lib.ChainTensors()
  tn.x, tn.score = x.data_ptr(), score.data_ptr()
  for l, m in enumerate(blocks):
    tn.w[l], tn.bias[l] = m.conv.weight.data_ptr(), (m.conv.bias.data_ptr() if m.conv.bias is not None else None)
    tn.gamma[l], tn.beta[l] = m.norm.weight.data_ptr(), m.norm.bias.data_ptr()
    tn.running_mean[l], tn.running_var[l] = m.norm.running_mean.data_ptr(), m.norm.running_var.data_ptr()
    tn.y_raw[l] = y_raw[l].data_ptr() if keep else None
    tn.y[l] = y[l].data_ptr() if keep else None
    tn.save[l] = save[l].data_ptr() if keep else None
  tn.w_logits, tn.bias_logits = logits.weight.data_ptr(), logits.bias.data_ptr()
  tn.z = z.data_ptr() if keep else None
  tn.soft, tn.out, tn.prepared = soft.data_ptr(), out.data_ptr(), prepared.data_ptr()
  tn.sync, tn.sync_words = sync.data_ptr(), sync.numel()
  wsp = workspace(lib().ms_decoder_chain_workspace(ctypes.byref(d)), dev)
  check(lib().ms_decoder_chain_fwd(ctypes.byref(d), ctypes.byref(tn), _ptr(wsp), wsp.numel(), _stream()), 'ms_decoder_chain_fwd')
  if training:
    for m in blocks:
      m._note_train_pass()
  if not need_grad:
    return out, soft
  h = x
  for l, m in enumerate(blocks):
    n = m.norm
    h = _ConvBlockFn.apply(h, None, m.conv.weight, m.conv.bias, n.weight, n.bias, m._geometry(), MS_BN_TRAIN,
                           MS_IN_BCAST if l == 0 else MS_IN_PLAIN, (n.running_mean, n.running_var), (y_raw[l], y[l], save[l]))
  geom = getattr(logits, '_ms_geom', None)
  if geom is None:
    geom = logits._ms_geom = ConvGeom(1, logits.groups, logits.kernel_size, logits.stride, logits.padding, slope=0.0)
  zt = _ConvBlockFn.apply(h, None, logits.weight, logits.bias, None, None, geom, MS_BARE, MS_IN_PLAIN, None, (None, z, None))
  return _SoftmaxMixFn.apply(zt, score, int(P), (out, soft))


class _LerpTimeFn(torch.autograd.Function):
  @staticmethod
  def forward(ctx, x, t_out):
    _need_hip(x)
    x = x.contiguous()
    B, C, Tin, F = x.shape
    y = torch.empty((B, C, t_out), dtype=torch.float32, device=x.device)
    check(lib().ms_lerp_time_fwd(_ptr(x), _ptr(y), B, C, Tin, F, t_out, _stream()), 'ms_lerp_time_fwd')
    ctx.shape = (B, C, Tin, F, t_out)
    return y

  @staticmethod
  def backward(ctx, dy):
    B, C, Tin, F, t_out = ctx.shape
    dy = dy.contiguous()
    dx = torch.empty((B, C, Tin, F), dtype=torch.float32, device=dy.device)
    check(lib().ms_lerp_time_bwd(_ptr(dy), _ptr(dx), B, C, Tin, F, t_out, _stream()), 'ms_lerp_time_bwd')
    return dx, None


@_bridge64
def lerp_time(x, t_out):
  return _LerpTimeFn.apply(x, int(t_out))


class _SoftmaxMixFn(torch.autograd.Function):
  @staticmethod
  def forward(ctx, z, score, P, pre=None):
    _need_hip(z, score)
    z, score = z.contiguous(), score.contiguous()
    B, M, T = score.shape
    assert z.shape == (B, M * P, T), (z.shape, score.shape, P)
    if pre is not None:
      out, soft = pre
    else:
      soft = torch.empty((B, T, M), dtype=torch.float32, device=z.device)
      out = torch.empty((B, T, P), dtype=torch.float32, device=z.device)
      check(lib().ms_softmax_mix_fwd(_ptr(z), _ptr(score), _ptr(soft), _ptr(out), B, M, P, T, _stream()),
            'ms_softmax_mix_fwd')
    ctx.save_for_backward(z, soft)
    ctx.dims = (B, M, P, T)
    ctx.mark_non_differentiable(soft)
    return out, soft

  @staticmethod
  def backward(ctx, dout, _dsoft):
    z, soft = ctx.saved_tensors
    B, M, P, T = ctx.dims
    dout = dout.contiguous()
    dz = torch.empty_like(z)
    dscore = torch.empty((B, M, T), dtype=torch.float32, device=z.device)
    check(lib().ms_softmax_mix_bwd(_ptr(z), _ptr(soft), _ptr(dout), _ptr(dz), _ptr(dscore), B, M, P, T, _stream()),
          'ms_softmax_mix_bwd')
    return dz, dscore, None, None


# ... 395 lines not shown
```

Before: 11350 clips/s.

## Co-run clip-resident dgrad kernels in backward as paired host/guest launches

Extends the clip32 co-run mechanism from forward to backward data-gradient launches. A dgrad launch from a guest branch is held and then merged with the next host dgrad launch into a single paired kernel that splits the CUs between the two. The intent is to fill idle CUs during small backward convolutions and to cut launch count. It adds hold/flush bookkeeping in the Python autograd path, new template instantiations, and risk of ordering or hazard errors when held launches are flushed late.

```diff
diff --git a/include/mixstage.h b/include/mixstage.h
--- a/include/mixstage.h
+++ b/include/mixstage.h
@@ -70,6 +70,8 @@
 int ms_clip_hold_discard(void* stream);
 int ms_clip_grid(const ms_conv_desc* d);
 int ms_clip_pair_ok(const ms_conv_desc* host, const ms_conv_desc* guest);
+int ms_clip_dgrad_grid(const ms_conv_desc* d);
+int ms_clip_dgrad_pair_ok(const ms_conv_desc* host, const ms_conv_desc* guest);
 size_t ms_fwd_weights_bytes(const ms_conv_desc* d);
 int ms_fwd_weights_prepare(int n, const ms_conv_desc* descs, const float* const* w, void* const* planes, void* stream);
 
diff --git a/include/mixstage_aux.h b/include/mixstage_aux.h
--- a/include/mixstage_aux.h
+++ b/include/mixstage_aux.h
@@ -36,6 +36,7 @@
 int ms_debug_set_clip32(int on);
 
 int ms_debug_set_clip_corun(int on);
+int ms_debug_set_clip_corun_bwd(int on);
 
 int ms_selftest_mfma(const float* A, const float* B, float* C, int K, void* stream);
 int ms_probe_peak(int kind, long iters, void* a, void* b, double* work, void* stream);
diff --git a/mix_stage_amd/_lib.py b/mix_stage_amd/_lib.py
--- a/mix_stage_amd/_lib.py
+++ b/mix_stage_amd/_lib.py
@@ -161,6 +161,9 @@
     'ms_clip_hold_discard': (c_int, [_P]),
     'ms_clip_grid': (c_int, [_DESC]),
     'ms_clip_pair_ok': (c_int, [_DESC, _DESC]),
+    'ms_clip_dgrad_grid': (c_int, [_DESC]),
+    'ms_clip_dgrad_pair_ok': (c_int, [_DESC, _DESC]),
+    'ms_debug_set_clip_corun_bwd': (c_int, [c_int]),
     'ms_debug_set_wgrad16_target': (c_int, [c_int]),
     'ms_debug_set_wgrad16_ring': (c_int, [c_int]),
     'ms_debug_set_wgrad_target': (c_int, [c_int]),
diff --git a/mix_stage_amd/csrc/api.hip b/mix_stage_amd/csrc/api.hip
--- a/mix_stage_amd/csrc/api.hip
+++ b/mix_stage_amd/csrc/api.hip
@@ -171,9 +171,9 @@
                          float* y, float* save, void* workspace, size_t workspace_bytes, void* stream,
                          const ms_fwd_options* opt) {
   const bool clip_path = d && dt_of(d) == DT_F32 && g_precision == 0 && !validate(d, "ms_conv_block_fwd") && clip32_fwd_ok(d);
-  int rc = clip32_fwd_call_begin((hipStream_t)stream, clip_path, workspace, workspace_bytes);
+  int rc = clip32_call_begin((hipStream_t)stream, clip_path, workspace, workspace_bytes);
   if (!rc) rc = conv_block_fwd_impl(d, x, x2, w, bias, gamma, beta, running_mean, running_var, y_raw, y, save, workspace, workspace_bytes, stream, opt);
-  clip32_fwd_call_end((hipStream_t)stream);
+  clip32_call_end((hipStream_t)stream);
   return rc;
 }
 
@@ -478,19 +478,40 @@
                               dgamma, dbeta, workspace, workspace_bytes, stream, &o);
 }
 
+static int conv_block_bwd_impl(const ms_conv_desc* d, const float* x, const float* x2, const float* w, const float* gamma,
+                               const float* running_mean, const float* running_var, const float* y_raw, const float* y,
+                               const float* save, const float* dy, float* dyr, float* dx, float* dx2, float* dw, float* dbias,
+                               float* dgamma, float* dbeta, void* workspace, size_t workspace_bytes, void* stream,
+                               const ms_bwd_options* opt);
+
 int ms_conv_block_bwd_ex(const ms_conv_desc* d, const float* x, const float* x2, const float* w, const float* gamma,
                          const float* running_mean, const float* running_var, const float* y_raw, const float* y,
                          const float* save, const float* dy, float* dyr, float* dx, float* dx2, float* dw, float* dbias,
                          float* dgamma, float* dbeta, void* workspace, size_t workspace_bytes, void* stream,
                          const ms_bwd_options* opt) {
+  int rc = validate(d, "ms_conv_block_bwd");
+  if (rc) return rc;
+  const bool side = opt && opt->side_stream && opt->side_stream != stream;
+  const bool clip_path = dx && !side && dt_of(d) == DT_F32 && g_precision == 0 && clip32_dgrad_ok(d);
+  rc = clip32_call_begin((hipStream_t)stream, clip_path, workspace, workspace_bytes);
+  if (!rc) rc = conv_block_bwd_impl(d, x, x2, w, gamma, running_mean, running_var, y_raw, y, save, dy, dyr, dx, dx2, dw, dbias, dgamma, dbeta,
+                                    workspace, workspace_bytes, stream, opt);
+  clip32_call_end((hipStream_t)stream);
+  return rc;
+}
+
+static int conv_block_bwd_impl(const ms_conv_desc* d, const float* x, const float* x2, const float* w, const float* gamma,
+                               const float* running_mean, const float* running_var, const float* y_raw, const float* y,
+                               const float* save, const float* dy, float* dyr, float* dx, float* dx2, float* dw, float* dbias,
+                               float* dgamma, float* dbeta, void* workspace, size_t workspace_bytes, void* stream,
+                               const ms_bwd_options* opt) {
   (void)running_mean; (void)running_var;
   ms_bwd_options none = {};
   if (!opt) opt = &none;
   void* side_stream = opt->side_stream;
   const float* wt_prepared = opt->wt_prepared;
   const bool defer_wgrad = opt->wgrad_partials != nullptr;
-  int rc = validate(d, "ms_conv_block_bwd");
-  if (rc) return rc;
+  int rc = 0;
   if (d->mode == MS_BN_EVAL) return set_error("ms_conv_block_bwd: BN_EVAL blocks are never differentiated on the path");
   if (!dy || !w || !workspace) return set_error("ms_conv_block_bwd: null tensor");
   if (d->mode == MS_BN_TRAIN && !opt->dy_is_dyr && (!y_raw || !save || !gamma || !dyr)) return set_error("ms_conv_block_bwd: BN_TRAIN needs y_raw/save/gamma/dyr");
@@ -577,7 +598,8 @@
     if (rc && rc != -2) return rc;
     if (rc == -2 && opt->dx_accum) return set_error("ms_conv_block_bwd: the clip-resident data gradient declined a launch with dx_accum");
     dx_done = rc == 0;
-    rc = 0;
+    rc = dx_done ? 0 : clip32_hold_flush(s);
+    if (rc) return rc;
   }
   if (dx && !dx_done && p.dg_grouped) {
     const float* wp = wt_prepared;
@@ -718,10 +740,23 @@
   if (validate(host, "ms_clip_pair_ok") || validate(guest, "ms_clip_pair_ok") || dt_of(host) != DT_F32 || dt_of(guest) != DT_F32 || g_precision != 0) return 0;
   return clip32_fwd_pair_ok(host, guest) ? 1 : 0;
 }
+int ms_clip_dgrad_grid(const ms_conv_desc* d) {
+  if (validate(d, "ms_clip_dgrad_grid") || dt_of(d) != DT_F32 || g_precision != 0) return 0;
+  return clip32_dgrad_grid(d);
+}
+int ms_clip_dgrad_pair_ok(const ms_conv_desc* host, const ms_conv_desc* guest) {
+  if (validate(host, "ms_clip_dgrad_pair_ok") || validate(guest, "ms_clip_dgrad_pair_ok") || dt_of(host) != DT_F32 || dt_of(guest) != DT_F32 || g_precision != 0) return 0;
+  return clip32_dgrad_pair_ok(host, guest) ? 1 : 0;
+}
 int ms_debug_set_clip_corun(int on) {
   const int prev = g_clip_corun < 0 ? 1 : g_clip_corun;
   g_clip_corun = on ? 1 : 0;
   return prev;
 }
-
-}
+int ms_debug_set_clip_corun_bwd(int on) {
+  const int prev = g_clip_corun_bwd < 0 ? 1 : g_clip_corun_bwd;
+  g_clip_corun_bwd = on ? 1 : 0;
+  return prev;
+}
+
+}
diff --git a/mix_stage_amd/csrc/clip32.hip b/mix_stage_amd/csrc/clip32.hip
--- a/mix_stage_amd/csrc/clip32.hip
+++ b/mix_stage_amd/csrc/clip32.hip
@@ -586,15 +586,15 @@
   int nA;
   Clip32Args a, b;
 };
-template <int KWA, int SA, int NBA, bool UP2A, int K8WA, int KWB, int SB, int NBB, bool UP2B, int K8WB>
+template <int KWA, int SA, int NBA, bool UP2A, int K8WA, int KWB, int SB, int NBB, bool UP2B, int K8WB, bool DG2A = false, bool DG2B = false>
 __global__ __launch_bounds__(256, 1) void clip32_pair_kernel(const ClipPairArgs pp) {
   const unsigned bid = blockIdx.x;
   if (bid < (unsigned)pp.nA) {
     prefetch_kernargs<sizeof(Clip32Args)>();
-    clip32_body<KWA, SA, NBA, UP2A, K8WA>(pp.a, bid);
+    clip32_body<KWA, SA, NBA, UP2A, K8WA, DG2A>(pp.a, bid);
   } else {
     prefetch_kernargs<384>((int)offsetof(ClipPairArgs, b));
-    clip32_body<KWB, SB, NBB, UP2B, K8WB>(pp.b, bid - (unsigned)pp.nA);
+    clip32_body<KWB, SB, NBB, UP2B, K8WB, DG2B>(pp.b, bid - (unsigned)pp.nA);
   }
 }
 
@@ -754,27 +754,46 @@
   Clip32Args a;
   int KW, S, nb, nwg, lds;
   bool up2, dg2;
+  bool bwd;
   const char* what;
   double flops, bytes;
 };
 
 enum { CLIP_HOST_DOWN8 = 0, CLIP_HOST_UP8 = 1, CLIP_HOSTS = 2 };
 enum { CLIP_GUEST_K3_4 = 0, CLIP_GUEST_DOWN2 = 1, CLIP_GUEST_DOWN4 = 2, CLIP_GUEST_DOWN8 = 3, CLIP_GUESTS = 4 };
+enum { CLIP_BHOST_UP8 = 0, CLIP_BHOST_DOWN8 = 1 };
+enum { CLIP_BGUEST_DG0 = 0, CLIP_BGUEST_DG2 = 1, CLIP_BGUEST_DG4 = 2, CLIP_BGUEST_DG8 = 3 };
 static int clip_host_kind(const ClipJob& j) {
-  if (j.dg2 || j.a.k8w != 8) return -1;
+  if (j.a.k8w != 8) return -1;
+  if (j.bwd) {
+    if (j.up2) return -1;
+    return j.dg2 ? CLIP_BHOST_DOWN8 : (j.KW == 3 && j.S == 1) ? CLIP_BHOST_UP8 : -1;
+  }
+  if (j.dg2) return -1;
   if (j.KW == 4 && j.S == 2 && !j.up2) return CLIP_HOST_DOWN8;
   if (j.KW == 3 && j.S == 1 && j.up2) return CLIP_HOST_UP8;
   return -1;
 }
 static int clip_guest_kind(const ClipJob& j) {
-  if (j.dg2 || j.up2) return -1;
+  if (j.up2) return -1;
+  if (j.bwd) {
+    if (!j.dg2) return -1;
+    return j.a.k8w == 2 ? CLIP_BGUEST_DG2 : j.a.k8w == 4 ? CLIP_BGUEST_DG4 : j.a.k8w == 8 ? CLIP_BGUEST_DG8 : j.a.k8w == 9 ? -1 : CLIP_BGUEST_DG0;
+  }
+  if (j.dg2) return -1;
   if (j.KW == 3 && j.S == 1) return j.a.k8w == 4 ? CLIP_GUEST_K3_4 : -1;
   if (j.KW == 4 && j.S == 2) return j.a.k8w == 2 ? CLIP_GUEST_DOWN2 : j.a.k8w == 4 ? CLIP_GUEST_DOWN4 : j.a.k8w == 8 ? CLIP_GUEST_DOWN8 : -1;
   return -1;
 }
-template <int KWA, int SA, int NBA, bool UP2A, int K8WA, int KWB, int SB, int NBB, bool UP2B, int K8WB>
+static bool clip_pair_instance(const ClipJob& A, const ClipJob& B) {
+  const int h = clip_host_kind(A), g = clip_guest_kind(B);
+  if (h < 0 || g < 0 || A.bwd != B.bwd) return false;
+  if (!A.bwd) return true;
+  return h == CLIP_BHOST_UP8 ? (g == CLIP_BGUEST_DG0 || g == CLIP_BGUEST_DG8) : g != CLIP_BGUEST_DG0;
+}
+template <int KWA, int SA, int NBA, bool UP2A, int K8WA, int KWB, int SB, int NBB, bool UP2B, int K8WB, bool DG2A = false, bool DG2B = false>
 static int clip32_pair_launch_k(const ClipPairArgs& pp, int nwg, int lds_bytes, hipStream_t s) {
-  auto fn = clip32_pair_kernel<KWA, SA, NBA, UP2A, K8WA, KWB, SB, NBB, UP2B, K8WB>;
+  auto fn = clip32_pair_kernel<KWA, SA, NBA, UP2A, K8WA, KWB, SB, NBB, UP2B, K8WB, DG2A, DG2B>;
   static unsigned long long attr_done = 0;
   if (first_time_on_device(attr_done)) {
     if (hipFuncSetAttribute(reinterpret_cast<const void*>(fn), hipFuncAttributeMaxDynamicSharedMemorySize, 160 * 1024) != hipSuccess)
@@ -791,6 +810,17 @@
     case CLIP_GUEST_DOWN2: return clip32_pair_launch_k<KWA, SA, NBA, UP2A, 8, 4, 2, 1, false, 2>(pp, nwg, lds_bytes, s);
     case CLIP_GUEST_DOWN4: return clip32_pair_launch_k<KWA, SA, NBA, UP2A, 8, 4, 2, 1, false, 4>(pp, nwg, lds_bytes, s);
     default: return clip32_pair_launch_k<KWA, SA, NBA, UP2A, 8, 4, 2, 1, false, 8>(pp, nwg, lds_bytes, s);
+  }
+}
+static int clip32_pair_launch_bwd(int host, int guest, const ClipPairArgs& pp, int nwg, int lds_bytes, hipStream_t s) {
+  if (host == CLIP_BHOST_UP8) {
+    if (guest == CLIP_BGUEST_DG0) return clip32_pair_launch_k<3, 1, 2, false, 8, 4, 1, 2, false, 0, false, true>(pp, nwg, lds_bytes, s);
+    return clip32_pair_launch_k<3, 1, 2, false, 8, 4, 1, 2, false, 8, false, true>(pp, nwg, lds_bytes, s);
+  }
+  switch (guest) {
+    case CLIP_BGUEST_DG2: return clip32_pair_launch_k<4, 1, 2, false, 8, 4, 1, 2, false, 2, true, true>(pp, nwg, lds_bytes, s);
+    case CLIP_BGUEST_DG4: return clip32_pair_launch_k<4, 1, 2, false, 8, 4, 1, 2, false, 4, true, true>(pp, nwg, lds_bytes, s);
+    default: return clip32_pair_launch_k<4, 1, 2, false, 8, 4, 1, 2, false, 8, true, true>(pp, nwg, lds_bytes, s);
   }
 }
 
@@ -833,6 +863,7 @@
 }
 
 int g_clip_corun = -1;
+int g_clip_corun_bwd = -1;
 enum { HOLD_IDLE = 0, HOLD_ARMED = 1, HOLD_PENDING = 2 };
 struct ClipHold {
   int state = HOLD_IDLE;
@@ -842,13 +873,17 @@
 };
 static std::mutex g_hold_mu;
 static std::map<hipStream_t, ClipHold> g_hold;
-static thread_local bool t_in_fwd = false;
+static thread_local bool t_in_call = false;
 static thread_local const char* t_ws_lo = nullptr;
 static thread_local const char* t_ws_hi = nullptr;
 
 static bool clip_corun_on() {
   if (g_clip_corun < 0) { const char* e = getenv("MS_CLIP_CORUN"); g_clip_corun = e ? (atoi(e) != 0) : 1; }
   return g_clip_corun != 0;
+}
+static bool clip_corun_bwd_on() {
+  if (g_clip_corun_bwd < 0) { const char* e = getenv("MS_CLIP_CORUN_BWD"); g_clip_corun_bwd = e ? (atoi(e) != 0) : 1; }
+  return g_clip_corun_bwd != 0;
 }
 
 int clip32_hold_arm(hipStream_t s) {
@@ -876,8 +911,8 @@
   }
   return clip32_issue(job, s);
 }
-int clip32_fwd_call_begin(hipStream_t s, bool clip_path, const void* ws, size_t ws_bytes) {
-  t_in_fwd = true;
+int clip32_call_begin(hipStream_t s, bool clip_path, const void* ws, size_t ws_bytes) {
+  t_in_call = true;
   t_ws_lo = (const char*)ws; t_ws_hi = t_ws_lo + (ws ? ws_bytes : 0);
   bool flush = false;
   {
@@ -888,16 +923,16 @@
   }
   return flush ? clip32_hold_flush(s) : 0;
 }
-void clip32_fwd_call_end(hipStream_t s) {
-  t_in_fwd = false;
+void clip32_call_end(hipStream_t s) {
+  t_in_call = false;
   std::lock_guard<std::mutex> lk(g_hold_mu);
   auto it = g_hold.find(s);
   if (it != g_hold.end() && it->second.state == HOLD_ARMED) it->second.state = HOLD_IDLE;
 }
 
 static bool clip_pair_fits(const ClipJob& A, const ClipJob& B) {
-  if (!clip_corun_on()) return false;
-  if (clip_host_kind(A) < 0 || clip_guest_kind(B) < 0) return false;
+  if (!clip_corun_on() || (A.bwd && !clip_corun_bwd_on())) return false;
+  if (!clip_pair_instance(A, B)) return false;
   if (A.nwg % 8) return false;
   int cus = current_device_cus();
   if (cus <= 0) cus = 256;
@@ -905,7 +940,8 @@
 }
 static bool clip_pair_ok(const ClipJob& A, const ClipJob& B) {
   if (!clip_pair_fits(A, B)) return false;
-  const bool meetA = A.a.ep == EP_RAW_STATS && A.a.npw > 1, meetB = B.a.ep == EP_RAW_STATS && B.a.npw > 1;
+  auto meets = [](const ClipJob& j) { return (j.a.ep == EP_RAW_STATS || j.a.ep == EP_DGRAD_BN) && j.a.npw > 1; };
+  const bool meetA = meets(A), meetB = meets(B);
   if (meetA && meetB && (A.a.part == B.a.part || A.a.sync == B.a.sync)) return false;
   return true;
 }
@@ -920,11 +956,13 @@
   pp.nA = A.nwg; pp.a = A.a; pp.b = B.a;
   pp.a.stamps = pp.b.stamps = nullptr;
   const int nwg = A.nwg + B.nwg, lds = std::max(A.lds, B.lds), guest = clip_guest_kind(B);
+  if (A.bwd) return clip32_pair_launch_bwd(clip_host_kind(A), guest, pp, nwg, lds, s);
   return clip_host_kind(A) == CLIP_HOST_DOWN8 ? clip32_pair_launch_g<4, 2, 1, false>(guest, pp, nwg, lds, s)
                                               : clip32_pair_launch_g<3, 1, 2, true>(guest, pp, nwg, lds, s);
 }
 
-int clip32_launch(Clip32Args a, int KW, int S, bool up2, const char* what, hipStream_t s, bool dg2 = false, ClipJob* plan = nullptr) {
+int clip32_launch(Clip32Args a, int KW, int S, bool up2, const char* what, hipStream_t s, bool dg2 = false, ClipJob* plan = nullptr,
+                  bool bwd = false) {
   const int nb = (S == 2 && !dg2) ? 1 : 2, npx = 32 * nb;
   a.k8w = clip_k8w(a.Cin);
   a.npw = a.B * a.To / npx;
@@ -955,11 +993,11 @@
   if (!cus) cus = 256;
   if ((a.ep == EP_RAW_STATS || a.ep == EP_DGRAD_BN) && a.npw > 1 && nwg > cus) return -2;
   ClipJob job;
-  job.a = a; job.KW = KW; job.S = S; job.nb = nb; job.nwg = nwg; job.lds = lds; job.up2 = up2; job.dg2 = dg2; job.what = what;
+  job.a = a; job.KW = KW; job.S = S; job.nb = nb; job.nwg = nwg; job.lds = lds; job.up2 = up2; job.dg2 = dg2; job.bwd = bwd; job.what = what;
   job.flops = 2.0 * a.rows_valid * a.Cin * (dg2 ? 2 : KW) * (double)a.B * a.To;
   job.bytes = 4.0 * ((double)a.rows_valid * a.Cin * KW + (double)a.B * a.Cin * a.Ti + (double)a.B * a.rows_valid * a.To);
   if (plan) { *plan = job; return 0; }
-  if (t_in_fwd) {
+  if (t_in_call) {
     ClipJob held;
     int st;
     {
@@ -1048,9 +1086,27 @@
   }
   if (d->KW == 4) {
     a.Ti = d->OW;
-    return clip32_launch(a, 4, 2, false, "dgrad", s, true);
-  }
-  return clip32_launch(a, 3, 1, false, "dgrad", s);
-}
-
-}
+    return clip32_launch(a, 4, 2, false, "dgrad", s, true, nullptr, true);
+  }
+  return clip32_launch(a, 3, 1, false, "dgrad", s, false, nullptr, true);
+}
+
+static int clip32_dgrad_plan(const ms_conv_desc* d, ClipJob* plan) {
+  if (!clip32_dgrad_ok(d)) return 0;
+  Clip32Args a = {};
+  a.B = d->B; a.Cin = d->Cout; a.Cout = d->Cin; a.rows_valid = d->Cin; a.To = d->W; a.Ti = d->KW == 4 ? d->OW : d->W;
+  a.ep = d->in_mode == MS_IN_UP2ADD ? EP_DGRAD_UP2 : EP_BARE;
+  plan->nwg = 0;
+  if (clip32_launch(a, d->KW == 4 ? 4 : 3, d->KW == 4 ? 2 : 1, false, "dgrad", nullptr, d->KW == 4, plan, true) != 0) return 0;
+  return plan->nwg;
+}
+int clip32_dgrad_grid(const ms_conv_desc* d) {
+  ClipJob plan;
+  return clip32_dgrad_plan(d, &plan);
+}
+bool clip32_dgrad_pair_ok(const ms_conv_desc* host, const ms_conv_desc* guest) {
+  ClipJob A, B;
+  return clip32_dgrad_plan(host, &A) > 0 && clip32_dgrad_plan(guest, &B) > 0 && clip_pair_fits(A, B);
+}
+
+}
diff --git a/mix_stage_amd/csrc/kernels.h b/mix_stage_amd/csrc/kernels.h
--- a/mix_stage_amd/csrc/kernels.h
+++ b/mix_stage_amd/csrc/kernels.h
@@ -173,11 +173,14 @@
                      const float* beta, float* rm, float* rv, float* y_raw, float* y, float* save, float* part, int* sync,
                      int sync_words, hipStream_t s);
 extern int g_clip_corun;
+extern int g_clip_corun_bwd;
+int clip32_dgrad_grid(const ms_conv_desc* d);
+bool clip32_dgrad_pair_ok(const ms_conv_desc* host, const ms_conv_desc* guest);
 int clip32_hold_arm(hipStream_t s);
 int clip32_hold_flush(hipStream_t s);
 void clip32_hold_discard(hipStream_t s);
-int clip32_fwd_call_begin(hipStream_t s, bool clip_path, const void* ws, size_t ws_bytes);
-void clip32_fwd_call_end(hipStream_t s);
+int clip32_call_begin(hipStream_t s, bool clip_path, const void* ws, size_t ws_bytes);
+void clip32_call_end(hipStream_t s);
 int clip32_fwd_grid(const ms_conv_desc* d);
 bool clip32_fwd_pair_ok(const ms_conv_desc* host, const ms_conv_desc* guest);
 struct Clip32PrevBN { const float* y; const float* y_raw; const float* save; const float* gamma; float* dgamma; float* dbeta; float* dbias; float slope; };
diff --git a/mix_stage_amd/ops.py b/mix_stage_amd/ops.py
--- a/mix_stage_amd/ops.py
+++ b/mix_stage_amd/ops.py
@@ -45,7 +45,8 @@
 
 
 
-_corun = {'driver': None, 'held': False, 'keep': [], 'on': os.environ.get('MS_CLIP_CORUN', '1') != '0', 'merges_offered': 0}
+_corun = {'driver': None, 'held': False, 'keep': [], 'on': os.environ.get('MS_CLIP_CORUN', '1') != '0', 'merges_offered': 0,
+          'in_guest': False, 'bwd_on': os.environ.get('MS_CLIP_CORUN_BWD', '1') != '0', 'bwd_keep': [], 'bwd_offered': 0}
 
 
 def workspace(nbytes, device):
@@ -192,6 +193,9 @@
   _deferred['jobs'].clear()
   _deferred['keep'].clear()
   _deferred['queued'] = False
+  if _corun['bwd_keep']:
+    lib().ms_clip_hold_discard(_stream())
+    _corun['bwd_keep'].clear()
   if _deferred['launches']:
     _deferred['launches'] = 0
     lib().ms_wgrad_discard()
@@ -229,6 +233,8 @@
 def _flush_deferred_wgrad():
   jobs = _deferred['jobs']
   _deferred['queued'] = False
+  if _corun['bwd_keep']:
+    _bwd_hold_release()
   if _deferred['launches']:
     _deferred['launches'] = 0
     try:
@@ -349,6 +355,7 @@
   def forward(ctx, x, x2, w, bias, gamma, beta, geom, mode, in_mode, stats, pre=None, prev=None, link=None):
     rm, rv = stats if stats is not None else (None, None)
     _need_hip(x, x2, w, bias, gamma, beta, rm, rv)
+    xin = x
     x = x.contiguous()
     x2 = x2.contiguous() if x2 is not None else None
     nd = geom.nd
@@ -394,6 +401,9 @@
         _corun['keep'].append((x, x2, w, bias, gamma, beta, rm, rv, y_raw, y, save, ws, planes, sync))
     ctx.geom_desc = d
     ctx.mode, ctx.in_mode = mode, in_mode
+    ctx.corun_guest = bool(_corun['in_guest'] and pre is None and nd == 1 and xin is not None and xin.grad_fn is not None
+                           and type(xin.grad_fn).__name__ == '_ConvBlockFnBackward'
+                           and not (getattr(xin, '_backward_hooks', None) or getattr(xin, 'retains_grad', False)))
     ctx.prev = None
     ctx.dy_is_dyr = False
     if prev is not None and pre is None and in_mode == MS_IN_PLAIN and nd == 1 and getattr(prev, 'mode', None) == MS_BN_TRAIN \
@@ -419,6 +429,18 @@
 
   @staticmethod
   def backward(ctx, dy):
+    try:
+      return _ConvBlockFn._backward(ctx, dy)
+    except BaseException:
+      if _corun['held'] or _corun['bwd_keep']:
+        lib().ms_clip_hold_discard(_stream())
+        _corun['bwd_keep'].clear()
+      raise
+    finally:
+      _corun['held'] = False
+
+  @staticmethod
+  def _backward(ctx, dy):
     x, x2, w, gamma, y_raw, y, save = ctx.saved_tensors
     d, mode, in_mode = ctx.geom_desc, ctx.mode, ctx.in_mode
     if mode == MS_BN_EVAL:
@@ -470,8 +492,15 @@
         raise RuntimeError('residual link: a residual gradient of shape %s arrived for an input of shape %s (needs grad: %s)' %
                            (tuple(acc.shape), tuple(x.shape), want_dx))
     acc_in_launch = False
+    side = _overlap['stream']
+    guest = bool(ctx.corun_guest and want_dx and side is None and _bwd_guest_ok(d, dy))
+    if guest and _corun['bwd_keep']:
+      _bwd_hold_release()
+    if guest:
+      check(lib().ms_clip_hold(_stream()), 'ms_clip_hold')
+      _corun['held'] = True
+      _corun['bwd_offered'] += 1
     ws = workspace(d._bwd_ws, dev)
-    side = _overlap['stream']
     if side is not None and need_w and direct_w is not True:
       torch.cuda.current_stream().wait_stream(side)
     if side is not None and direct_w is True and (dbias is None or direct_b is True):
@@ -521,6 +550,11 @@
                                       _ptr(y), _ptr(save), _ptr(dy), _ptr(dyr), _ptr(dx), _ptr(dx2), _ptr(dw),
                                       _ptr(dbias), _ptr(dgamma), _ptr(dbeta), _ptr(ws), ws.numel(), _stream()),
               'ms_conv_block_bwd')
+    if guest:
+      _corun['bwd_keep'].append((x, x2, w, gamma, y_raw, y, save, dy, dyr, dx, dx2, ws, wt, acc, fuse))
+      torch.autograd.Variable._execution_engine.queue_callback(_bwd_hold_end)
+    elif _corun['bwd_keep']:
+      _bwd_hold_release()
     if acc is not None and not acc_in_launch:
       dx.add_(acc)
     if ctx.link is not None and ctx.link[1] == 'residual' and dx2 is not None and ctx.needs_input_grad[1] and not ctx.link[0].taken:
@@ -606,13 +640,13 @@
     self._resume()
 
   def _resume(self):
-    self.in_guest = True
+    self.in_guest = _corun['in_guest'] = True
     try:
       self.next_desc = next(self.gen)
     except StopIteration as e:
       self.done, self.result, self.next_desc = True, e.value, None
     finally:
-      self.in_guest = False
+      self.in_guest = _corun['in_guest'] = False
 
   def offer(self, x, x2, w, geom, mode, in_mode):
     if self.done or self.next_desc is None or not x.is_cuda or x.dtype != torch.float32 or w.dtype != torch.float32:
@@ -671,6 +705,32 @@
 def enable_corun(on):
   old = _corun['on']
   _corun['on'] = bool(on)
+  return old
+
+
+def _bwd_guest_ok(d, dy):
+  from . import ops16
+  return bool(_corun['on'] and _corun['bwd_on'] and _corun['driver'] is None and not bn_sync_active() and not _stat_pair['on']
+              and ops16.in_launch_meetings() and dy.is_cuda and dy.dtype == torch.float32 and lib().ms_get_precision() == 0
+              and lib().ms_clip_dgrad_grid(ctypes.byref(d)) > 0)
+
+
+def _bwd_hold_release():
+  try:
+    check(lib().ms_clip_hold_flush(_stream()), 'ms_clip_hold_flush')
+  finally:
+    _corun['bwd_keep'].clear()
+
+
+def _bwd_hold_end():
+  if _corun['bwd_keep']:
+    _bwd_hold_release()
+
+
+def enable_corun_bwd(on):
+  old = _corun['bwd_on']
+  _corun['bwd_on'] = bool(on)
+  lib().ms_debug_set_clip_corun_bwd(1 if on else 0)
   return old
 
 
```

New measurement: 11490 clips/s (median of 6 runs). 1.01x the previous value.
